# StarsX/FluidX12

Hardware: AMD Instinct MI355X
Metric: voxel-updates/sec (advect+40 Jacobi) at 256^3; achieved HBM GB/s vs peak (higher is better)
Workload: dtype f32

## Files before the change

### fluidx12_amd/capi.py

```python
import ctypes as C
import os

from . import build as _build

FX_OK = 0
FX_E_INVALID, FX_E_DEVICE, FX_E_NOMEM, FX_E_STATE, FX_E_COMM, FX_E_HALO = -1, -2, -3, -4, -5, -6

RAY_MARCH_DIRECT, RAY_MARCH_CUBEMAP, SEPARATE_LIGHT_PASS, OPTIMIZED = 0, 1, 2, 3
FRAME_COUNT = 3
STORAGE_FP32, STORAGE_FP16 = 0, 1
JACOBI_FIXED, JACOBI_FAITHFUL = 0, 1
ADDRESS_CLAMP, ADDRESS_MIRROR = 0, 1
FLAG_JACOBI_FUSE_MASK, FLAG_NO_OVERLAP, FLAG_RENDER_ONLY = 0xF, 0x10, 0x20
OPT_OVERLAP, OPT_JACOBI_ROUND, OPT_ADAPTIVE_HALO, OPT_COUNT_SAMPLES, OPT_RENDER_ACCEL = 1, 2, 3, 4, 5
ABI_VERSION = 7
(FIELD_VELOCITY, FIELD_VELOCITY1, FIELD_COLOR, FIELD_COLOR_PREV, FIELD_PRESSURE, FIELD_DIVERGENCE,
 FIELD_LIGHTMAP, FIELD_CUBEMAP, FIELD_TARGET, FIELD_TARGET_FLOAT, FIELD_CUBE_DEPTH) = range(11)
FIELD_TEMPERATURE = 11
DEPTH_DEVICE = 0x1
LIGHT_DIRECTIONAL, LIGHT_POINT = 0, 1
MAX_EMITTERS = 16
OBSTACLES_DEVICE = 0x1
MAX_OBSTACLE_BODIES = 16
MAX_OBSTACLE_MESHES = 16
# ... 19 lines not shown


class FrameInfo(C.Structure):
    _fields_ = [("cube_lod", C.c_uint32), ("cube_size", C.c_uint32), ("ray_samples", C.c_uint32),
                ("visibility_mask", C.c_uint32), ("frame_parity", C.c_uint32), ("edge_pixels", C.c_float),
                ("time_step", C.c_float), ("world_view_proj_i", C.c_float * 16), ("screen_to_world", C.c_float * 16)]


class Light(C.Structure):
    _fields_ = [("struct_size", C.c_uint32), ("kind", C.c_uint32), ("position", C.c_float * 3), ("color", C.c_float * 4),
                ("ambient", C.c_float * 4)]


class Emitter(C.Structure):
    _fields_ = [("struct_size", C.c_uint32), ("flags", C.c_uint32), ("center", C.c_float * 3), ("radius", C.c_float),
                ("color_rate", C.c_float * 4), ("force", C.c_float * 3), ("swirl", C.c_float)]


class ObstacleBody(C.Structure):
    _fields_ = [("struct_size", C.c_uint32), ("flags", C.c_uint32), ("box_lo", C.c_float * 3), ("box_hi", C.c_float * 3),
                ("linear", C.c_float * 3), ("angular", C.c_float * 3), ("pivot", C.c_float * 3)]


class ObstacleMesh(C.Structure):
    _fields_ = [("struct_size", C.c_uint32), ("flags", C.c_uint32), ("positions", C.c_void_p), ("indices", C.c_void_p),
                ("vertex_count", C.c_uint32), ("triangle_count", C.c_uint32), ("transform", C.c_void_p)]


class MeshReport(C.Structure):
    _fields_ = [("solid_cells", C.c_uint64), ("open_columns", C.c_uint32), ("skipped_triangles", C.c_uint32)]


class Buoyancy(C.Structure):
    _fields_ = [("struct_size", C.c_uint32), ("flags", C.c_uint32), ("ambient", C.c_float), ("density_weight", C.c_float),
                ("lift", C.c_float), ("cooling", C.c_float), ("up", C.c_float * 3)]


class HeatSource(C.Structure):
    _fields_ = [("struct_size", C.c_uint32), ("flags", C.c_uint32), ("center", C.c_float * 3), ("radius", C.c_float), ("rate", C.c_float)]


class PressureSolver(C.Structure):
    _fields_ = [("kind", C.c_uint32), ("flags", C.c_uint32), ("cycles", C.c_uint32), ("pre_sweeps", C.c_uint32), ("post_sweeps", C.c_uint32),
                ("coarse_sweeps", C.c_uint32), ("max_levels", C.c_uint32), ("omega", C.c_float)]


class ParticleParams(C.Structure):
    _fields_ = [("struct_size", C.c_uint32), ("flags", C.c_uint32), ("scheme", C.c_uint32), ("drift", C.c_float * 3), ("lifetime", C.c_float)]


class Timing(C.Structure):
    _fields_ = [("advect_ms", C.c_double), ("divergence_ms", C.c_double), ("jacobi_ms", C.c_double),
                ("project_ms", C.c_double), ("light_ms", C.c_double), ("view_ms", C.c_double),
                ("exchange_ms", C.c_double), ("steps", C.c_uint64), ("jacobi_launches", C.c_uint64),
                ("jacobi_sweeps", C.c_uint64), ("renders", C.c_uint64), ("resolve_ms", C.c_double),
                ("jacobi_main_ms", C.c_double), ("jacobi_main_launches", C.c_uint64), ("jacobi_main_sweeps", C.c_uint64),
                ("exchange_bytes", C.c_uint64), ("advect_halo_planes", C.c_uint64), ("chain_ms", C.c_double),
                ("freeze_solves", C.c_uint64), ("freeze_sweeps", C.c_uint64), ("exchange_calls", C.c_uint64),
                ("view_samples", C.c_uint64), ("light_samples", C.c_uint64), ("lightmap_fetches", C.c_uint64),
                ("freeze_strip_launches", C.c_uint64)]


_vp, _fp = C.c_void_p, C.POINTER(C.c_float)
SYMBOLS = {
    "fx_abi_version": (C.c_int, []),
    "fx_error_string": (C.c_char_p, [C.c_int]),
    "fx_create": (C.c_int, [C.POINTER(_vp), C.POINTER(Desc)]),
    "fx_destroy": (C.c_int, [_vp]),
    "fx_set_max_samples": (C.c_int, [_vp, C.c_uint32, C.c_uint32]),
    "fx_set_sh": (C.c_int, [_vp, _fp]),
    "fx_update_frame": (C.c_int, [_vp, C.c_float, C.c_uint8, _fp, _fp, _fp]),
    "fx_simulate": (C.c_int, [_vp, _vp, C.c_uint8]),
    "fx_render": (C.c_int, [_vp, _vp, C.c_uint8, C.c_uint8]),
    "fx_get_frame_info": (C.c_int, [_vp, C.POINTER(FrameInfo)]),
    "fx_synchronize": (C.c_int, [_vp]),
    "fx_last_error": (C.c_char_p, [_vp]),
    "fx_upload": (C.c_int, [_vp, C.c_int, _vp, C.c_size_t]),
    "fx_download": (C.c_int, [_vp, C.c_int, _vp, C.c_size_t]),
    "fx_field_bytes": (C.c_size_t, [_vp, C.c_int]),
    "fx_field_digest": (C.c_int, [_vp, C.c_int, C.c_uint32, C.c_uint32, C.POINTER(C.c_uint64)]),
    "fx_checkpoint_save": (C.c_int, [_vp, C.c_char_p]),
    "fx_checkpoint_load": (C.c_int, [_vp, C.c_char_p]),
    "fx_advect": (C.c_int, [_vp, _vp]),
    "fx_divergence": (C.c_int, [_vp, _vp]),
    "fx_jacobi": (C.c_int, [_vp, _vp, C.c_uint32]),
    "fx_project": (C.c_int, [_vp, _vp]),
    "fx_set_vorticity_confinement": (C.c_int, [_vp, C.c_float]),
    "fx_confine_vorticity": (C.c_int, [_vp, _vp]),
    "fx_set_emitters": (C.c_int, [_vp, C.POINTER(Emitter), C.c_uint32]),
    "fx_get_emitters": (C.c_int, [_vp, C.POINTER(Emitter), C.c_uint32, C.POINTER(C.c_uint32)]),
    "fx_set_impulse": (C.c_int, [_vp, C.c_int]),
    "fx_emit": (C.c_int, [_vp, _vp]),
    "fx_set_obstacles": (C.c_int, [_vp, _vp, _vp, C.c_size_t, C.c_uint32]),
    "fx_get_obstacles": (C.c_int, [_vp, _vp, C.c_size_t, C.POINTER(C.c_uint64)]),
    "fx_enforce_obstacles": (C.c_int, [_vp, _vp]),
    "fx_set_obstacle_bodies": (C.c_int, [_vp, C.POINTER(ObstacleBody), C.c_uint32]),
    "fx_get_obstacle_bodies": (C.c_int, [_vp, C.POINTER(ObstacleBody), C.c_uint32, C.POINTER(C.c_uint32)]),
    "fx_set_obstacle_meshes": (C.c_int, [_vp, _vp, C.POINTER(ObstacleMesh), C.c_uint32, C.POINTER(MeshReport)]),
    "fx_set_buoyancy": (C.c_int, [_vp, C.POINTER(Buoyancy)]),
    "fx_get_buoyancy": (C.c_int, [_vp, C.POINTER(Buoyancy), C.POINTER(C.c_int)]),
    "fx_set_heat_sources": (C.c_int, [_vp, C.POINTER(HeatSource), C.c_uint32]),
    "fx_get_heat_sources": (C.c_int, [_vp, C.POINTER(HeatSource), C.c_uint32, C.POINTER(C.c_uint32)]),
    "fx_heat": (C.c_int, [_vp, _vp]),
    "fx_set_particles": (C.c_int, [_vp, _vp, _fp, C.c_uint32, C.c_uint32]),
    "fx_get_particles": (C.c_int, [_vp, _fp, C.c_uint32, C.POINTER(C.c_uint32)]),
    "fx_particles_device": (C.c_int, [_vp, C.POINTER(_vp), C.POINTER(C.c_uint32)]),
    "fx_set_particle_params": (C.c_int, [_vp, C.POINTER(ParticleParams)]),
    "fx_get_particle_params": (C.c_int, [_vp, C.POINTER(ParticleParams)]),
    "fx_move_particles": (C.c_int, [_vp, _vp]),
    "fx_sample_velocity": (C.c_int, [_vp, _vp, _fp, C.c_uint32, _fp, C.c_uint32]),
    "fx_set_open_walls": (C.c_int, [_vp, C.c_uint32]),
    "fx_get_open_walls": (C.c_int, [_vp, C.POINTER(C.c_uint32)]),
    "fx_open_inflow": (C.c_int, [_vp, _vp]),
    "fx_set_advection_scheme": (C.c_int, [_vp, C.c_uint32]),
    "fx_get_advection_scheme": (C.c_int, [_vp, C.POINTER(C.c_uint32)]),
    "fx_set_pressure_solver": (C.c_int, [_vp, C.POINTER(PressureSolver)]),
    "fx_get_pressure_solver": (C.c_int, [_vp, C.POINTER(PressureSolver)]),
    "fx_pressure_solve": (C.c_int, [_vp, _vp]),
    "fx_download_pressure_level": (C.c_int, [_vp, C.c_uint32, C.c_int, _vp, C.c_size_t]),
    "fx_sh_transform": (C.c_int, [_vp, _fp, C.c_uint32, _fp]),
    "fx_set_environment": (C.c_int, [_vp, _fp, C.c_uint32]),
    "fx_render_environment": (C.c_int, [_vp, _vp, C.c_uint8]),
    "fx_clear_render_target": (C.c_int, [_vp, _vp, _fp]),
    "fx_render_cube": (C.c_int, [_vp, _vp, C.c_uint8]),
    "fx_set_scene_depth": (C.c_int, [_vp, _vp, _vp, C.c_uint32, C.c_uint32, C.c_float, C.c_float, C.c_uint32]),
    "fx_set_light": (C.c_int, [_vp, C.POINTER(Light)]),
    "fx_get_light": (C.c_int, [_vp, C.POINTER(Light)]),
    "fx_dds_cube_info": (C.c_int, [_vp, C.c_size_t, C.POINTER(C.c_uint32), C.POINTER(C.c_uint32)]),
    "fx_dds_decode_cube": (C.c_int, [_vp, _vp, C.c_size_t, C.c_uint32, _fp, C.c_size_t]),
    "fx_timing_enable": (C.c_int, [_vp, C.c_int]),
    "fx_set_option": (C.c_int, [_vp, C.c_uint32, C.c_uint32]),
    "fx_set_knob": (C.c_int, [C.c_char_p, C.c_char_p]),
    "fx_knob_name": (C.c_char_p, [C.c_uint32]),
    "fx_comm_gather_color": (C.c_int, [_vp, _vp, _vp, C.c_int, C.POINTER(C.c_uint32), C.POINTER(C.c_uint32)]),
    "fx_timing_read": (C.c_int, [_vp, C.POINTER(Timing), C.c_int]),
    "fx_comm_id_bytes": (C.c_size_t, []),
    "fx_comm_get_unique_id": (C.c_int, [_vp, C.c_size_t]),
    "fx_comm_init_rank": (C.c_int, [_vp, _vp, C.c_size_t, C.c_int, C.c_int]),
    "fx_comm_init_local": (C.c_int, [C.POINTER(_vp), C.c_int]),
    "fx_comm_init_peer": (C.c_int, [C.POINTER(_vp), C.c_int]),
}

_lib = None
LAB_KNOBS = {"ADVECT_BLOCK", "ADVECT_FAST", "ADVECT_LDS_HALF", "ADVECT_TILE_ROWS", "ADVECT_ZCHUNK", "BLOCK_REMAP", "BLOCK_SHAPE", "DEBUG_NO_COPY",
             "FREEZE_DENSE_LEVELS", "FREEZE_DENSE_ONE", "FREEZE_FAST", "FREEZE_FUSE_DIV", "FREEZE_NT", "FREEZE_SHRINK", "FREEZE_T", "FREEZE_WGS",
             "JACOBI2D_TILE", "JACOBI_BLOCK", "JACOBI_BLOCKG", "LIGHT_FILL_DIRTY", "LIGHT_RAY_NT", "LIGHT_RAY_WGS", "OBSTACLE_V4", "PROJECT_V4", "ROW_VW",
             "STRIP3H_PAIRS", "STRIP3_COOP", "STRIP3_NO512", "STRIP3_OFF", "STRIP3_ZCHUNK", "STRIP4T", "STRIP4T_256", "STRIP4T_512", "STRIP4T_FROM", "STRIP4T_GRID", "STRIP4T_NARROW", "STRIP4T_NARROW_FROM", "STRIP4T_PIECES", "STRIP4X", "STRIP4X_MINP", "STRIP4X_NT", "STRIP4X_ORDER", "STRIP4X_WGS",
             "STRIP4_OCTET", "STRIP4_ZCHUNK", "STRIP4_ZFLOOR", "STRIP_GENERIC", "STRIP_R", "STRIP_REMAP", "STRIP_WGS", "STRIP_WIDE", "STRIP_ZCHUNK", "VIEW_ORDER", "VIEW_WGS", "VORT_ZCHUNK", "WIDE_OFFSETS", "XCD_REMAP"}


def lib_path():
    return _build.LIB


def load():
    global _lib
    if _lib is not None:
        return _lib
    try:
        import torch
    except Exception:
        pass
    path = _build.ensure_built()
    if os.environ.get("FLUIDX_LIB_PATH"):
        path = os.environ["FLUIDX_LIB_PATH"]
    if not os.path.exists(path):
# ... 48 lines not shown
```

### fluidx12_amd/csrc/fx_advect_lds.hip

```cpp
#include "fx_internal.h"
#include <algorithm>
#include <cstdlib>
#include <cstdio>

namespace fx {

namespace {

constexpr int TX = kAdvectTileX;
constexpr int HX = TX + 2;
constexpr int NSLOT = 4;
template <bool HALF, int TY> struct Lay {
	static constexpr int NCELL = HX * (TY + 2);
	static constexpr int VEL_BYTES = NCELL * 4;
	static constexpr int COL_BYTES = HALF ? 2 * NCELL * 4 : NCELL * 16;
	static constexpr int SLOT_BYTES = COL_BYTES + 3 * VEL_BYTES;
};
typedef _Float16 h16;
typedef _Float16 h16x4 __attribute__((ext_vector_type(4)));
__device__ __forceinline__ h16 to_h16(float v) { asm("" : "+v"(v)); return (h16)v; }
__device__ __forceinline__ float lo_half(uint32_t d) { return (float)__builtin_bit_cast(h16, (uint16_t)(d & 0xffffu)); }
__device__ __forceinline__ float hi_half(uint32_t d) { return (float)__builtin_bit_cast(h16, (uint16_t)(d >> 16)); }

__device__ __forceinline__ float lerpf(float a, float b, float f) { return fmaf(f, b - a, a); }
__device__ __forceinline__ float saturatef(float x) { return fminf(fmaxf(x, 0.0f), 1.0f); }

__device__ __forceinline__ int addr_tap(int i, int n, int mode)
{
	if (mode == FX_ADDRESS_MIRROR) {
		const int period = 2 * n;
		int m = i % period;
		if (m < 0) m += period;
		return m < n ? m : period - 1 - m;
	}
	return min(max(i, 0), n - 1);
}

typedef __attribute__((address_space(3))) void lds_void;
typedef const __attribute__((address_space(1))) void glb_void;

template <int VEL_BYTES>
__device__ __forceinline__ void stage64(const void* col, const void* v0, const void* v1, const void* v2, uint32_t off_col, uint32_t off_vel, uint32_t lds_col, uint32_t lds_vel)
{
	uint32_t keep;
	lds_col = __builtin_amdgcn_readfirstlane(lds_col);
	lds_vel = __builtin_amdgcn_readfirstlane(lds_vel);
	asm volatile(
		"s_mov_b32 %0, m0\n\t"
		"s_mov_b32 m0, %7\n\t"
		"s_nop 0\n\t"
		"global_load_lds_dwordx4 %5, %1\n\t"
		"s_mov_b32 m0, %8\n\t"
		"s_nop 0\n\t"
		"global_load_lds_dword %6, %2\n\t"
		"s_add_u32 m0, m0, %9\n\t"
		"s_nop 0\n\t"
		"global_load_lds_dword %6, %3\n\t"
		"s_add_u32 m0, m0, %9\n\t"
		"s_nop 0\n\t"
		"global_load_lds_dword %6, %4\n\t"
		"s_mov_b32 m0, %0"
		: "=&s"(keep)
		: "s"(col), "s"(v0), "s"(v1), "s"(v2), "v"(off_col), "v"(off_vel), "s"(lds_col), "s"(lds_vel), "n"(VEL_BYTES)
		: "scc");
}

template <int VEL_BYTES>
__device__ __forceinline__ void stage64h(const void* col, const void* v0, const void* v1, const void* v2, uint32_t off_col, uint32_t off_vel, uint32_t lds_col, uint32_t lds_vel)
{
	uint32_t keep;
	lds_col = __builtin_amdgcn_readfirstlane(lds_col);
	lds_vel = __builtin_amdgcn_readfirstlane(lds_vel);
	const uint32_t off_col_hi = off_col + 4u;
	asm volatile(
		"s_mov_b32 %0, m0\n\t"
		"s_mov_b32 m0, %8\n\t"
		"s_nop 0\n\t"
		"global_load_lds_dword %5, %1\n\t"
		"s_add_u32 m0, m0, %10\n\t"
		"s_nop 0\n\t"
		"global_load_lds_dword %6, %1\n\t"
		"s_mov_b32 m0, %9\n\t"
		"s_nop 0\n\t"
		"global_load_lds_ushort %7, %2\n\t"
		"s_add_u32 m0, m0, %10\n\t"
		"s_nop 0\n\t"
		"global_load_lds_ushort %7, %3\n\t"
		"s_add_u32 m0, m0, %10\n\t"
		"s_nop 0\n\t"
		"global_load_lds_ushort %7, %4\n\t"
		"s_mov_b32 m0, %0"
		: "=&s"(keep)
		: "s"(col), "s"(v0), "s"(v1), "s"(v2), "v"(off_col), "v"(off_col_hi), "v"(off_vel), "s"(lds_col), "s"(lds_vel), "n"(VEL_BYTES)
		: "scc");
}

template <typename T>
__device__ __forceinline__ T ldg32(const void* base, uint32_t byte_off)
{
	return *reinterpret_cast<const T*>(static_cast<const char*>(base) + byte_off);
}


template <bool P2> __device__ __forceinline__ uint32_t rows(uint32_t y, int lgX, const Geom& g) { return P2 ? y << lgX : y * (uint32_t)g.X; }
template <bool P2> __device__ __forceinline__ uint32_t planes(uint32_t z, int lgP, const Geom& g) { return P2 ? z << lgP : z * ((uint32_t)g.X * (uint32_t)g.Y); }

template <bool HALF, bool P2>
__device__ __forceinline__ void advect_gather(const Geom& g, const SimParams& sp, int ix, int iy, int z0, int z1, bool z_present, float fx, float fy, float fz,
	const char* v0, const char* v1, const char* v2, const void* __restrict__ col_in, int lgX, int lgP, unsigned* halo_overflow, float (&u)[3], float (&c)[4])
{
	const int xa0 = addr_tap(ix, g.X, sp.address), xa1 = addr_tap(ix + 1, g.X, sp.address);
	const int ya0 = addr_tap(iy, g.Y, sp.address), ya1 = addr_tap(iy + 1, g.Y, sp.address);
	if (!z_present) {
		atomicOr(halo_overflow, 1u);
		z0 = min(max(z0, g.zlo), g.zhi);
		z1 = min(max(z1, g.zlo), g.zhi);
	}
	const uint32_t p0 = planes<P2>((uint32_t)g.lz(z0), lgP, g), p1 = planes<P2>((uint32_t)g.lz(z1), lgP, g);
	const uint32_t ry0 = rows<P2>((uint32_t)ya0, lgX, g), ry1 = rows<P2>((uint32_t)ya1, lgX, g);
	const uint32_t c000 = p0 + ry0 + (uint32_t)xa0, c100 = p0 + ry0 + (uint32_t)xa1;
	const uint32_t c010 = p0 + ry1 + (uint32_t)xa0, c110 = p0 + ry1 + (uint32_t)xa1;
	const uint32_t c001 = p1 + ry0 + (uint32_t)xa0, c101 = p1 + ry0 + (uint32_t)xa1;
	const uint32_t c011 = p1 + ry1 + (uint32_t)xa0, c111 = p1 + ry1 + (uint32_t)xa1;
	const char* vb[3] = { v0, v1, v2 };
	auto gv = [](const char* b, uint32_t cell) -> float { return HALF ? (float)ldg32<h16>(b, cell * 2u) : ldg32<float>(b, cell * 4u); };
	auto gc = [&](uint32_t cell) -> float4 {
		if (HALF) { const h16x4 h = ldg32<h16x4>(col_in, cell * 8u); return make_float4((float)h.x, (float)h.y, (float)h.z, (float)h.w); }
		return ldg32<float4>(col_in, cell * 16u);
	};
#pragma unroll
	for (int a = 0; a < 3; ++a) {
		const float c00 = lerpf(gv(vb[a], c000), gv(vb[a], c100), fx);
		const float c10 = lerpf(gv(vb[a], c010), gv(vb[a], c110), fx);
		const float c01 = lerpf(gv(vb[a], c001), gv(vb[a], c101), fx);
		const float c11 = lerpf(gv(vb[a], c011), gv(vb[a], c111), fx);
		u[a] = lerpf(lerpf(c00, c10, fy), lerpf(c01, c11, fy), fz);
	}
	const float4 t000 = gc(c000), t100 = gc(c100), t010 = gc(c010), t110 = gc(c110);
	const float4 t001 = gc(c001), t101 = gc(c101), t011 = gc(c011), t111 = gc(c111);
#define FX_TRI(m) lerpf(lerpf(lerpf(t000.m, t100.m, fx), lerpf(t010.m, t110.m, fx), fy), \
	lerpf(lerpf(t001.m, t101.m, fx), lerpf(t011.m, t111.m, fx), fy), fz)
	c[0] = FX_TRI(x); c[1] = FX_TRI(y); c[2] = FX_TRI(z); c[3] = FX_TRI(w);
#undef FX_TRI
}

template <bool HALF, bool ALPHA>
__device__ __forceinline__ void advect_finish(const SimParams& sp, float (&u)[3], float (&c)[4], float ex, float dx, float dz, float dt, float atten,
	uint32_t id, uint32_t stride, void* __restrict__ vel_out, void* __restrict__ col_out, float* __restrict__ alpha_out)
{
	if (__builtin_amdgcn_ballot_w64(sp.impulse && ex > -6.5f) != 0) {
		const float basis = exp2f(ex);
		if (basis >= 0.0183156393f) {
			float Fx, Fy, Fz;
			if (sp.is3d) {
				Fx = fmaf(basis, 0.0f, dz * -200.0f);
				Fy = fmaf(basis, 192.0f, 0.0f);
				Fz = fmaf(basis, 0.0f, dx * 200.0f);
			} else {
				Fx = 0.0f; Fy = basis * 48.0f; Fz = 0.0f;
			}
			u[0] = fmaf(Fx, dt, u[0]); u[1] = fmaf(Fy, dt, u[1]); u[2] = fmaf(Fz, dt, u[2]);
			const float bdt = basis * dt;
			c[0] = saturatef(fmaf(bdt, 8.0f, c[0]));
			c[1] = saturatef(fmaf(bdt, 16.0f, c[1]));
			c[2] = saturatef(fmaf(bdt, 40.0f, c[2]));
			c[3] = saturatef(fmaf(bdt, 40.0f, c[3]));
		}
	}
	char* vo = static_cast<char*>(vel_out);
	char* co = static_cast<char*>(col_out);
	if (HALF) {
		*reinterpret_cast<h16*>(vo + id * 2u) = to_h16(u[0] * atten);
		*reinterpret_cast<h16*>(vo + (stride + id) * 2u) = to_h16(u[1] * atten);
		*reinterpret_cast<h16*>(vo + (2u * stride + id) * 2u) = to_h16(u[2] * atten);
		h16x4 hc;
		hc.x = to_h16(c[0] * atten); hc.y = to_h16(c[1] * atten); hc.z = to_h16(c[2] * atten); hc.w = to_h16(c[3] * atten);
		*reinterpret_cast<h16x4*>(co + id * 8u) = hc;
		if (ALPHA) *reinterpret_cast<float*>(reinterpret_cast<char*>(alpha_out) + id * 4u) = (float)hc.w;
	} else {
		*reinterpret_cast<float*>(vo + id * 4u) = u[0] * atten;
		*reinterpret_cast<float*>(vo + (stride + id) * 4u) = u[1] * atten;
		*reinterpret_cast<float*>(vo + (2u * stride + id) * 4u) = u[2] * atten;
		*reinterpret_cast<float4*>(co + id * 16u) = make_float4(c[0] * atten, c[1] * atten, c[2] * atten, c[3] * atten);
		if (ALPHA) *reinterpret_cast<float*>(reinterpret_cast<char*>(alpha_out) + id * 4u) = c[3] * atten;
	}
}

}

template <bool HALF, int TY, bool DEFER, bool P2, bool ALPHA>
__global__ __launch_bounds__(64 * TY) __attribute__((amdgpu_waves_per_eu(4, 4))) void k_advect_lds(const Geom g, const SimParams sp,
	const void* __restrict__ vel_in, const void* __restrict__ col_in, void* __restrict__ vel_out, void* __restrict__ col_out, float* __restrict__ alpha_out,
	int z_begin, int nzp, int zchunk, int nchunks, unsigned* halo_overflow, float rX, float rY, float rZ, float inv_rr,
	int lgX, int lgY, int lg_gx, int lg_gy, uint32_t* __restrict__ far_list, uint32_t* __restrict__ far_flat, uint32_t* __restrict__ far_total, uint32_t far_cap)
{
	__shared__ uint32_t far_n, far_base;
	extern __shared__ __attribute__((aligned(16))) char lds[];

	const int tid = (int)threadIdx.x, lane = tid & 63, wave = __builtin_amdgcn_readfirstlane(tid >> 6);
	const int ntx = P2 ? 1 << lg_gx : lg_gx, nty = P2 ? 1 << lg_gy : lg_gy;
	const int ntiles = ntx * nty * nchunks;
	int tl = (int)blockIdx.x;
	{
		const int q = ntiles >> 3, r = ntiles & 7, xcd = tl & 7, j = tl >> 3;
		tl = xcd * q + min(xcd, r) + j;
	}
	const int tx = P2 ? tl & (ntx - 1) : tl % ntx, ty = P2 ? (tl >> lg_gx) & (nty - 1) : (tl / ntx) % nty, chunk = P2 ? tl >> (lg_gx + lg_gy) : tl / (ntx * nty);
	const int x0t = tx << 6, y0t = ty * TY;
	const int zb = z_begin + chunk * zchunk, ze = min(zb + zchunk, z_begin + nzp);
	if (zb >= ze) return;

	const int lgP = lgX + lgY;
	constexpr int COL_BYTES = Lay<HALF, TY>::COL_BYTES, SLOT_BYTES = Lay<HALF, TY>::SLOT_BYTES;
	constexpr int NCELL = Lay<HALF, TY>::NCELL, VEL_BYTES = Lay<HALF, TY>::VEL_BYTES, NT = 64 * TY;
	constexpr uint32_t ES = HALF ? 2 : 4, CS = HALF ? 8 : 16;
	const uint32_t stride = planes<P2>((uint32_t)g.nzl(), lgP, g);
	const char* v0 = reinterpret_cast<const char*>(vel_in);
	const char* v1 = v0 + (size_t)stride * ES;
	const char* v2 = v1 + (size_t)stride * ES;

	uint32_t src_a, src_b = 0;
	{
		const int c = tid, r = c / HX, cc = c - r * HX;
		src_a = rows<P2>((uint32_t)addr_tap(y0t - 1 + r, g.Y, sp.address), lgX, g) + (uint32_t)addr_tap(x0t - 1 + cc, g.X, sp.address);
	}
	const bool has_b = NT + tid < NCELL;
	if (has_b) {
		const int c = NT + tid, r = c / HX, cc = c - r * HX;
		src_b = rows<P2>((uint32_t)addr_tap(y0t - 1 + r, g.Y, sp.address), lgX, g) + (uint32_t)addr_tap(x0t - 1 + cc, g.X, sp.address);
	}
	const bool wave_has_b = NT + wave * 64 < NCELL;

	const uint32_t lds0 = (uint32_t)(size_t)(__attribute__((address_space(3))) char*)lds;
	auto fill = [&](int zq) {
		const int za = min(max(addr_tap(zq, g.Zg, sp.address), g.zlo), g.zhi);
		const size_t pz = planes<P2>((uint32_t)g.lz(za), lgP, g);
		const uint32_t slot = __builtin_amdgcn_readfirstlane(lds0 + (uint32_t)(((zq + 4) & 3) * SLOT_BYTES));
		const char* bc = reinterpret_cast<const char*>(col_in) + pz * CS;
		const char *b0 = v0 + pz * ES, *b1 = v1 + pz * ES, *b2 = v2 + pz * ES;
		if (HALF) stage64h<VEL_BYTES>(bc, b0, b1, b2, src_a * CS, src_a * ES, slot + (uint32_t)wave * (64 * 4), slot + COL_BYTES + (uint32_t)wave * (64 * 4));
		else stage64<VEL_BYTES>(bc, b0, b1, b2, src_a * CS, src_a * ES, slot + (uint32_t)wave * (64 * 16), slot + COL_BYTES + (uint32_t)wave * (64 * 4));
		if (wave_has_b) {
			if (has_b) {
				if (HALF) stage64h<VEL_BYTES>(bc, b0, b1, b2, src_b * CS, src_b * ES, slot + (NT + (uint32_t)wave * 64) * 4, slot + COL_BYTES + (NT + (uint32_t)wave * 64) * 4);
				else stage64<VEL_BYTES>(bc, b0, b1, b2, src_b * CS, src_b * ES, slot + (NT + (uint32_t)wave * 64) * 16, slot + COL_BYTES + (NT + (uint32_t)wave * 64) * 4);
			}
		}
	};

	if (DEFER && tid == 0) far_n = 0u;
	fill(zb - 1);
	fill(zb);
	fill(zb + 1);
	asm volatile("s_waitcnt vmcnt(0)" ::: "memory");
	__syncthreads();

	const int x = x0t + lane, y = y0t + wave;
	const bool has_voxel = P2 || (x < g.X && y < g.Y);
	const float dt = sp.dt;
	const float px = P2 ? ((float)x + 0.5f) * rX : ((float)x + 0.5f) / (float)g.X;
	const float py = P2 ? ((float)y + 0.5f) * rY : ((float)y + 0.5f) / (float)g.Y;
	const float dx = px + -0.5f, dy = py + -0.100000001f;
	const float dxy2 = fmaf(dy, dy, dx * dx);
	const uint32_t own = (uint32_t)((wave + 1) * HX + lane + 1);
	const float atten = fmaxf(fmaf(-dt, 0.200000003f, 1.0f), 0.0f);

	auto compute = [&](int z) {
		if (!has_voxel) return;
		const float pz = P2 ? ((float)z + 0.5f) * rZ : ((float)z + 0.5f) / (float)g.Zg;
		const float dz = pz + -0.5f;
		const float d2 = fmaf(dz, dz, dxy2);
		const float ex = ((d2 * -4.0f) * inv_rr) * 1.44269502f;

		const char* sc = lds + ((z + 4) & 3) * SLOT_BYTES;
		const uint32_t* vs = reinterpret_cast<const uint32_t*>(sc + COL_BYTES);
		auto vval = [](uint32_t d) -> float { return HALF ? lo_half(d) : __uint_as_float(d); };
		const float u0x = vval(vs[own]), u0y = vval(vs[NCELL + own]), u0z = vval(vs[2 * NCELL + own]);
		const float ax = fmaf(-u0x, dt, px), ay = fmaf(-u0y, dt, py), az = fmaf(-u0z, dt, pz);
		const float tx_ = ax * (float)g.X - 0.5f, ty_ = ay * (float)g.Y - 0.5f, tz_ = az * (float)g.Zg - 0.5f;
		const float flx = floorf(tx_), fly = floorf(ty_), flz = floorf(tz_);
		const float fx = tx_ - flx, fy = ty_ - fly, fz = tz_ - flz;
		const int ix = (int)flx, iy = (int)fly, iz = (int)flz;
		const int jx = ix - x, jy = iy - y, jz = iz - z;
		int z0 = addr_tap(iz, g.Zg, sp.address), z1 = addr_tap(iz + 1, g.Zg, sp.address);
		const bool z_present = z0 >= g.zlo && z0 <= g.zhi && z1 >= g.zlo && z1 <= g.zhi;
		const bool inwin = (unsigned)(jx + 1) <= 1u && (unsigned)(jy + 1) <= 1u && (unsigned)(jz + 1) <= 1u && z_present;

		float u[3], c[4];
		if (DEFER && !inwin) {
			const uint32_t slot = atomicAdd(&far_n, 1u);
			far_list[(size_t)blockIdx.x * far_cap + slot] = P2 ? (uint32_t)x | (uint32_t)y << lgX | (uint32_t)z << lgP
				: ((uint32_t)z * (uint32_t)g.Y + (uint32_t)y) * (uint32_t)g.X + (uint32_t)x;
		}
		if (DEFER || inwin) {
			const int kx = DEFER && !inwin ? 0 : jx, ky = DEFER && !inwin ? 0 : jy, kz = DEFER && !inwin ? z : iz;
			const uint32_t c0 = (uint32_t)((int)own + ky * HX + kx);
			const char* s0 = lds + ((kz + 4) & 3) * SLOT_BYTES;
			const char* s1 = lds + ((kz + 5) & 3) * SLOT_BYTES;
#pragma unroll
			for (int a = 0; a < 3; ++a) {
				const uint32_t* p0 = reinterpret_cast<const uint32_t*>(s0 + COL_BYTES + a * VEL_BYTES) + c0;
				const uint32_t* p1 = reinterpret_cast<const uint32_t*>(s1 + COL_BYTES + a * VEL_BYTES) + c0;
				const float c00 = lerpf(vval(p0[0]), vval(p0[1]), fx);
				const float c10 = lerpf(vval(p0[HX]), vval(p0[HX + 1]), fx);
				const float c01 = lerpf(vval(p1[0]), vval(p1[1]), fx);
				const float c11 = lerpf(vval(p1[HX]), vval(p1[HX + 1]), fx);
				u[a] = lerpf(lerpf(c00, c10, fy), lerpf(c01, c11, fy), fz);
			}
			float4 t000, t100, t010, t110, t001, t101, t011, t111;
			if (HALF) {
				auto tex = [](const char* slot, uint32_t c) -> float4 {
					const uint32_t rg = reinterpret_cast<const uint32_t*>(slot)[c], ba = reinterpret_cast<const uint32_t*>(slot)[NCELL + c];
					return make_float4(lo_half(rg), hi_half(rg), lo_half(ba), hi_half(ba));
				};
				t000 = tex(s0, c0); t100 = tex(s0, c0 + 1); t010 = tex(s0, c0 + HX); t110 = tex(s0, c0 + HX + 1);
				t001 = tex(s1, c0); t101 = tex(s1, c0 + 1); t011 = tex(s1, c0 + HX); t111 = tex(s1, c0 + HX + 1);
			} else {
				const float4* q0 = reinterpret_cast<const float4*>(s0) + c0;
				const float4* q1 = reinterpret_cast<const float4*>(s1) + c0;
				t000 = q0[0]; t100 = q0[1]; t010 = q0[HX]; t110 = q0[HX + 1];
				t001 = q1[0]; t101 = q1[1]; t011 = q1[HX]; t111 = q1[HX + 1];
			}
#define FX_TRI(m) lerpf(lerpf(lerpf(t000.m, t100.m, fx), lerpf(t010.m, t110.m, fx), fy), \
	lerpf(lerpf(t001.m, t101.m, fx), lerpf(t011.m, t111.m, fx), fy), fz)
			c[0] = FX_TRI(x); c[1] = FX_TRI(y); c[2] = FX_TRI(z); c[3] = FX_TRI(w);
#undef FX_TRI
		} else {
			advect_gather<HALF, P2>(g, sp, ix, iy, z0, z1, z_present, fx, fy, fz, v0, v1, v2, col_in, lgX, lgP, halo_overflow, u, c);
		}

		const uint32_t id = planes<P2>((uint32_t)g.lz(z), lgP, g) + rows<P2>((uint32_t)y, lgX, g) + (uint32_t)x;
		advect_finish<HALF, ALPHA>(sp, u, c, ex, dx, dz, dt, atten, id, stride, vel_out, col_out, alpha_out);
	};

	for (int z = zb; z < ze; ++z) {
		if (z + 2 <= ze) fill(z + 2);
		compute(z);
		if (!(P2 || y < g.Y)) asm volatile("s_waitcnt vmcnt(0)" ::: "memory");
		else if (ALPHA) asm volatile("s_waitcnt vmcnt(5)" ::: "memory");
		else asm volatile("s_waitcnt vmcnt(4)" ::: "memory");
		__syncthreads();
	}
	if (DEFER) {
		const uint32_t n = far_n;
		if (n != 0u) {
			if (tid == 0) far_base = atomicAdd(far_total, n);
			__syncthreads();
			const uint32_t base = far_base;
			const uint32_t* seg = far_list + (size_t)blockIdx.x * far_cap;
			for (uint32_t i = (uint32_t)tid; i < n; i += (uint32_t)NT) far_flat[base + i] = seg[i];
		}
	}
}

template <bool HALF, bool P2, bool ALPHA>
__global__ __launch_bounds__(256) void k_advect_far(const Geom g, const SimParams sp,
	const void* __restrict__ vel_in, const void* __restrict__ col_in, void* __restrict__ vel_out, void* __restrict__ col_out, float* __restrict__ alpha_out,
	const uint32_t* __restrict__ far_flat, const uint32_t* __restrict__ far_total, uint32_t* __restrict__ far_total_next, unsigned* halo_overflow,
	float rX, float rY, float rZ, float inv_rr, int lgX, int lgY)
{
	const uint32_t n = *far_total;
	if (blockIdx.x == 0 && threadIdx.x == 0) *far_total_next = 0u;
	const int lgP = lgX + lgY;
	constexpr uint32_t ES = HALF ? 2 : 4;
	const uint32_t stride = planes<P2>((uint32_t)g.nzl(), lgP, g);
	const char* v0 = reinterpret_cast<const char*>(vel_in);
	const char* v1 = v0 + (size_t)stride * ES;
	const char* v2 = v1 + (size_t)stride * ES;
	const float dt = sp.dt;
	const float atten = fmaxf(fmaf(-dt, 0.200000003f, 1.0f), 0.0f);
	for (uint32_t i = blockIdx.x * 256u + threadIdx.x; i < n; i += gridDim.x * 256u) {
		const uint32_t code = far_flat[i];
		int x, y, z;
		if (P2) { x = (int)(code & (uint32_t)(g.X - 1)); y = (int)((code >> lgX) & (uint32_t)(g.Y - 1)); z = (int)(code >> lgP); }
		else { const uint32_t XY = (uint32_t)g.X * (uint32_t)g.Y, rem = code % XY; z = (int)(code / XY); y = (int)(rem / (uint32_t)g.X); x = (int)(rem % (uint32_t)g.X); }
		const float px = P2 ? ((float)x + 0.5f) * rX : ((float)x + 0.5f) / (float)g.X;
		const float py = P2 ? ((float)y + 0.5f) * rY : ((float)y + 0.5f) / (float)g.Y;
		const float pz = P2 ? ((float)z + 0.5f) * rZ : ((float)z + 0.5f) / (float)g.Zg;
		const float dx = px + -0.5f, dy = py + -0.100000001f, dz = pz + -0.5f;
		const float dxy2 = fmaf(dy, dy, dx * dx);
		const float d2 = fmaf(dz, dz, dxy2);
		const float ex = ((d2 * -4.0f) * inv_rr) * 1.44269502f;
		const uint32_t id = planes<P2>((uint32_t)g.lz(z), lgP, g) + rows<P2>((uint32_t)y, lgX, g) + (uint32_t)x;
		auto gv = [](const char* b, uint32_t cell) -> float { return HALF ? (float)ldg32<h16>(b, cell * 2u) : ldg32<float>(b, cell * 4u); };
		const float u0x = gv(v0, id), u0y = gv(v1, id), u0z = gv(v2, id);
		const float ax = fmaf(-u0x, dt, px), ay = fmaf(-u0y, dt, py), az = fmaf(-u0z, dt, pz);
		const float tx_ = ax * (float)g.X - 0.5f, ty_ = ay * (float)g.Y - 0.5f, tz_ = az * (float)g.Zg - 0.5f;
		const float flx = floorf(tx_), fly = floorf(ty_), flz = floorf(tz_);
		const float fx = tx_ - flx, fy = ty_ - fly, fz = tz_ - flz;
		const int ix = (int)flx, iy = (int)fly, iz = (int)flz;
		const int z0 = addr_tap(iz, g.Zg, sp.address), z1 = addr_tap(iz + 1, g.Zg, sp.address);
		const bool z_present = z0 >= g.zlo && z0 <= g.zhi && z1 >= g.zlo && z1 <= g.zhi;
		float u[3], c[4];
		advect_gather<HALF, P2>(g, sp, ix, iy, z0, z1, z_present, fx, fy, fz, v0, v1, v2, col_in, lgX, lgP, halo_overflow, u, c);
		advect_finish<HALF, ALPHA>(sp, u, c, ex, dx, dz, dt, atten, id, stride, vel_out, col_out, alpha_out);
	}
}


hipError_t launch_advect_lds(const Geom& g, const SimParams& sp, int half_store, const void* vel_in, const void* col_in,
	void* vel_out, void* col_out, int z_begin, int z_end, unsigned* halo_overflow, uint32_t* far_scratch, size_t far_words, int far_parity, bool* far_used, hipStream_t s, bool force,
	AdvectAlpha* alpha)
{
	if (far_used) *far_used = false;
	if (alpha) alpha->written = false;
	const int nzp = z_end - z_begin;
	AdvectLdsKnobs kn;
	kn.tile_rows = FX_KNOB_INT("ADVECT_TILE_ROWS", 8);
	kn.lds_half = FX_KNOB_INT("ADVECT_LDS_HALF", 1);
	kn.defer = FX_KNOB_INT("ADVECT_DEFER", 1);
	kn.zchunk = FX_KNOB("ADVECT_ZCHUNK");
	const AdvectLdsPlan pl = advect_lds_plan(g, half_store, z_begin, z_end, force, far_scratch != nullptr, far_words, alpha && alpha->out, kn);
	if (!pl.staged) return hipErrorNotSupported;
	const bool p2 = pl.p2, defer = pl.defer;
	const int TY = pl.tile_rows, ntx = pl.tiles_x, nty = pl.tiles_y, zchunk = pl.zchunk, nchunks = pl.nchunks;
	auto lg = [](int v) { int k = 0; while ((1 << k) < v) ++k; return k; };
	const int lgX = lg(g.X), lgY = lg(g.Y), lg_gx = p2 ? lg(ntx) : ntx, lg_gy = p2 ? lg(nty) : nty;
	const int tiles_xy = ntx * nty;
	const float rX = 1.0f / (float)g.X, rY = 1.0f / (float)g.Y, rZ = 1.0f / (float)g.Zg, inv_rr = sp.is3d ? 256.0f : 1024.0f;
	const uint32_t far_cap = (uint32_t)(TX * TY * zchunk);
	const size_t flat_words = (size_t)g.X * g.Y * (size_t)nzp;
	if (far_used) *far_used = defer;
	uint32_t* far_total = far_scratch ? far_scratch + (far_parity & 1) : nullptr;
	uint32_t* far_total_next = far_scratch ? far_scratch + ((far_parity & 1) ^ 1) : nullptr;
	uint32_t* far_flat = far_scratch ? far_scratch + 2 : nullptr;
	uint32_t* far_list = far_scratch ? far_scratch + 2 + flat_words : nullptr;
#define FX_ADV(H_, TY_, D_, P_, A_) do { \
		static bool attr_set = false; \
		if (!attr_set) { (void)hipFuncSetAttribute(reinterpret_cast<const void*>(k_advect_lds<H_, TY_, D_, P_, A_>), hipFuncAttributeMaxDynamicSharedMemorySize, NSLOT * Lay<H_, TY_>::SLOT_BYTES); attr_set = true; } \
		hipLaunchKernelGGL((k_advect_lds<H_, TY_, D_, P_, A_>), dim3(tiles_xy * nchunks), dim3(64 * TY_), (NSLOT * Lay<H_, TY_>::SLOT_BYTES), s, g, sp, vel_in, col_in, vel_out, col_out, alpha_out, \
			z_begin, nzp, zchunk, nchunks, halo_overflow, rX, rY, rZ, inv_rr, lgX, lgY, lg_gx, lg_gy, far_list, far_flat, far_total, far_cap); } while (0)
#define FX_FAR(H_, P_, A_) hipLaunchKernelGGL((k_advect_far<H_, P_, A_>), dim3(far_wgs), dim3(256), 0, s, g, sp, vel_in, col_in, vel_out, col_out, alpha_out, far_flat, far_total, far_total_next, halo_overflow, rX, rY, rZ, inv_rr, lgX, lgY)
	const int far_wgs = 1024;
	float* alpha_out = pl.alpha ? alpha->out : nullptr;
	if (alpha_out) {
		if (half_store) { if (p2) { FX_ADV(true, 8, true, true, true); FX_FAR(true, true, true); } else { FX_ADV(true, 8, true, false, true); FX_FAR(true, false, true); } }
		else { if (p2) { FX_ADV(false, 8, true, true, true); FX_FAR(false, true, true); } else { FX_ADV(false, 8, true, false, true); FX_FAR(false, false, true); } }
		alpha->written = true;
	} else if (!p2) {
		if (defer) {
			if (half_store) { FX_ADV(true, 8, true, false, false); FX_FAR(true, false, false); } else { FX_ADV(false, 8, true, false, false); FX_FAR(false, false, false); }
		} else { if (half_store) FX_ADV(true, 8, false, false, false); else FX_ADV(false, 8, false, false, false); }
	} else if (defer) {
		if (TY == 16) { if (half_store) FX_ADV(true, 16, true, true, false); else FX_ADV(false, 16, true, true, false); }
		else { if (half_store) FX_ADV(true, 8, true, true, false); else FX_ADV(false, 8, true, true, false); }
		if (half_store) FX_FAR(true, true, false); else FX_FAR(false, true, false);
	} else {
		if (TY == 16) { if (half_store) FX_ADV(true, 16, false, true, false); else FX_ADV(false, 16, false, true, false); }
		else { if (half_store) FX_ADV(true, 8, false, true, false); else FX_ADV(false, 8, false, true, false); }
	}
#undef FX_FAR
#undef FX_ADV
	return hipGetLastError();
}

}
```

### fluidx12_amd/csrc/fx_api.cpp

```cpp
#include "fx_host.h"
#include <cstring>
#include "fx_hostmath.h"
#include "fx_mesh_args.h"

using namespace fx;
using namespace fxh;

extern "C" {

int fx_abi_version(void) { return FX_ABI_VERSION; }

int fx_set_max_samples(fx_ctx* ctx, uint32_t max_ray, uint32_t max_light)
{
	if (!ctx || !max_ray || !max_light) return FX_E_INVALID;
	ctx->max_ray_samples = max_ray;
	ctx->max_light_samples = max_light;
	return FX_OK;
}

int fx_set_sh(fx_ctx* ctx, const float* coeffs27)
{
	if (!ctx) return FX_E_INVALID;
	if (!ctx->sh_dev) return FX_E_STATE;
	if (!coeffs27) { ctx->has_sh = false; return FX_OK; }
// ... 254 lines not shown
		ctx->depth = depth;
	} else {
		const size_t bytes = (size_t)width * height * sizeof(float);
		if (!ctx->depth_own) FX_HIP(hipMalloc((void**)&ctx->depth_own, bytes));
		hipStream_t s = pick_stream(ctx, stream);
		FX_HIP(hipMemcpyAsync(ctx->depth_own, depth, bytes, hipMemcpyHostToDevice, s));
		FX_HIP(hipStreamSynchronize(s));
		ctx->depth = ctx->depth_own;
	}
	ctx->depth_zn = z_near;
	ctx->depth_zf = z_far;
	return FX_OK;
}

int fx_set_light(fx_ctx* ctx, const fx_light* light)
{
	if (!ctx) return FX_E_INVALID;
	if (ctx->g.Zg <= 1 || ctx->g.nz != ctx->g.Zg) return FX_E_INVALID;
	if (!light) { default_light(ctx); return FX_OK; }
	if (light->struct_size != sizeof(fx_light)) return FX_E_INVALID;
	if (light->kind != FX_LIGHT_DIRECTIONAL && light->kind != FX_LIGHT_POINT) return FX_E_INVALID;
	for (int a = 0; a < 3; ++a) if (!std::isfinite(light->position[a])) return FX_E_INVALID;
	for (int a = 0; a < 4; ++a)
		if (!std::isfinite(light->color[a]) || !std::isfinite(light->ambient[a]) || light->color[a] < 0.0f || light->ambient[a] < 0.0f) return FX_E_INVALID;
	if (light->kind == FX_LIGHT_DIRECTIONAL && light->position[0] == 0.0f && light->position[1] == 0.0f && light->position[2] == 0.0f) return FX_E_INVALID;
	std::memcpy(ctx->fc.light_pt, light->position, sizeof ctx->fc.light_pt);
	std::memcpy(ctx->fc.light_color, light->color, sizeof ctx->fc.light_color);
	std::memcpy(ctx->fc.ambient, light->ambient, sizeof ctx->fc.ambient);
	ctx->light_kind = light->kind;
	return FX_OK;
}

int fx_get_light(fx_ctx* ctx, fx_light* out)
{
	if (!ctx || !out) return FX_E_INVALID;
	out->struct_size = sizeof(fx_light);
	out->kind = ctx->light_kind;
	std::memcpy(out->position, ctx->fc.light_pt, sizeof out->position);
	std::memcpy(out->color, ctx->fc.light_color, sizeof out->color);
	std::memcpy(out->ambient, ctx->fc.ambient, sizeof out->ambient);
	return FX_OK;
}

int fx_set_environment(fx_ctx* ctx, const float* cube, uint32_t n)
{
	if (!ctx || (cube && (!n || n > 8192))) return FX_E_INVALID;
	DeviceGuard dg(ctx->device);
	FX_HIP(hipDeviceSynchronize());
	if (ctx->env) { FX_HIP(hipFree(ctx->env)); ctx->env = nullptr; ctx->env_n = 0; }
	if (!cube) return FX_OK;
	const size_t bytes = (size_t)6 * n * n * 3 * sizeof(float);
	FX_HIP(hipMalloc((void**)&ctx->env, bytes));
	FX_HIP(hipMemcpy(ctx->env, cube, bytes, hipMemcpyHostToDevice));
	ctx->env_n = n;
	return FX_OK;
}

int fx_render_environment(fx_ctx* ctx, void* stream, uint8_t frame_index)
{
	if (!ctx || frame_index >= FX_FRAME_COUNT) return FX_E_INVALID;
	if (!ctx->env || !ctx->view_valid) return FX_E_STATE;
	DeviceGuard dg(ctx->device);
	hipStream_t s = pick_stream(ctx, stream);
	int rc = ensure_target(ctx, s);
	if (rc) return rc;
	ScopedMark mk(ctx, s, MK_RESOLVE);
	FX_HIP(launch_environment(ctx->env, (int)ctx->env_n, ctx->fc, (int)ctx->desc.viewport_w, (int)ctx->desc.viewport_h,
		ctx->target, ctx->target_float, s));
	return FX_OK;
}

int fx_get_frame_info(fx_ctx* ctx, fx_frame_info* out)
{
	if (!ctx || !out) return FX_E_INVALID;
	out->cube_lod = ctx->cube_lod;
	out->cube_size = (uint32_t)ctx->g.X >> ctx->cube_lod;
	out->ray_samples = ctx->ray_samples;
	out->visibility_mask = ctx->visibility_mask;
	out->frame_parity = ctx->frame_parity;
	out->edge_pixels = ctx->edge_pixels;
	out->time_step = ctx->time_step;
	std::memcpy(out->world_view_proj_i, ctx->fc.wvp_i, sizeof out->world_view_proj_i);
	std::memcpy(out->screen_to_world, ctx->fc.s2w, sizeof out->screen_to_world);
	return FX_OK;
}

int fx_advect(fx_ctx* ctx, void* stream)
{
	if (!ctx) return FX_E_INVALID;
	if (ctx->desc.flags & FX_FLAG_RENDER_ONLY) return FX_E_STATE;
	if (!ctx->frame_valid) return FX_E_STATE;
	if (ctx->nranks > 1) return FX_E_INVALID;
	hipStream_t s = pick_stream(ctx, stream);
	ScopedMark mk(ctx, s, MK_ADVECT);
	return advect_range(ctx, s, owned(ctx), false);
}

static int sim_guard(const fx_ctx* ctx, bool whole = true)
{
	if (!ctx) return FX_E_INVALID;
	if (ctx->desc.flags & FX_FLAG_RENDER_ONLY) return FX_E_STATE;
	if (whole && (ctx->g.nz != ctx->g.Zg || ctx->nranks > 1)) return FX_E_INVALID;
	return FX_OK;
}

static int run_stage(fx_ctx* ctx, void* stream, int (*phase)(fx_ctx*, hipStream_t))
{
	const int rc = sim_guard(ctx);
	return rc ? rc : phase(ctx, pick_stream(ctx, stream));
}

int fx_set_vorticity_confinement(fx_ctx* ctx, float epsilon)
{
	if (!std::isfinite(epsilon) || epsilon < 0.0f) return FX_E_INVALID;
	if (const int rc = sim_guard(ctx)) return rc;
	ctx->vort_eps = epsilon;
	return FX_OK;
}

int fx_confine_vorticity(fx_ctx* ctx, void* stream) { return run_stage(ctx, stream, confine_phase); }

int fx_set_emitters(fx_ctx* ctx, const fx_emitter* list, uint32_t count)
{
	if (const int rc = sim_guard(ctx)) return rc;
	if (count > FX_MAX_EMITTERS || (count && !list)) return FX_E_INVALID;
	for (uint32_t k = 0; k < count; ++k) {
		const fx_emitter& e = list[k];
		if (e.struct_size != sizeof(fx_emitter) || e.flags != 0) return FX_E_INVALID;
		if (!std::isfinite(e.radius) || !(e.radius > 0.0f) || !std::isfinite(e.swirl)) return FX_E_INVALID;
		for (int a = 0; a < 3; ++a) if (!std::isfinite(e.center[a]) || !std::isfinite(e.force[a])) return FX_E_INVALID;
		for (int a = 0; a < 4; ++a) if (!std::isfinite(e.color_rate[a]) || e.color_rate[a] < 0.0f) return FX_E_INVALID;
	}
	ctx->emitters.assign(list, list + count);
	return FX_OK;
}

int fx_get_emitters(fx_ctx* ctx, fx_emitter* out, uint32_t capacity, uint32_t* count)
{
	if (const int rc = sim_guard(ctx, false)) return rc;
	if (!count || (capacity && !out)) return FX_E_INVALID;
	*count = (uint32_t)ctx->emitters.size();
	for (uint32_t k = 0; k < capacity && k < *count; ++k) out[k] = ctx->emitters[k];
	return FX_OK;
}

int fx_set_impulse(fx_ctx* ctx, int enabled)
{
	if (const int rc = sim_guard(ctx, !enabled)) return rc;
	ctx->impulse_on = enabled != 0;
	return FX_OK;
}

int fx_emit(fx_ctx* ctx, void* stream) { return run_stage(ctx, stream, emit_phase); }

static int install_obstacle_mask(fx_ctx* ctx, const uint8_t* src, hipStream_t s)
{
	FX_HIP(launch_obstacle_codes(ctx->g, src, ctx->obst_spare, ctx->obst_stats, s));
	unsigned st[8];
	FX_HIP(hipMemcpyAsync(st, ctx->obst_stats, sizeof st, hipMemcpyDeviceToHost, s));
	FX_HIP(hipStreamSynchronize(s));
	std::swap(ctx->obst_code, ctx->obst_spare);
	ctx->obst_cells = (uint64_t)st[0] | ((uint64_t)st[1] << 32);
	for (int a = 0; a < 3; ++a) {
		ctx->obst_lo[a] = ctx->obst_cells ? (int)st[2 + a] : 0;
		ctx->obst_hi[a] = ctx->obst_cells ? (int)st[5 + a] + 1 : 0;
	}
// ... 563 lines not shown
	FX_HIP(hipHostMalloc((void**)&ctx->rec_host, 4 * sizeof(int) * (size_t)nrec, hipHostMallocDefault));
	std::memset(ctx->rec_host, 0, 4 * sizeof(int) * (size_t)nrec);
	FX_HIP(hipEventCreateWithFlags(&ctx->rec_ev, hipEventDisableTiming));
	return FX_OK;
}

int fx_comm_init_rank(fx_ctx* ctx, const void* id, size_t bytes, int rank, int nranks)
{
	if (!ctx || !id) return FX_E_INVALID;
	int rc = check_slab_chain(ctx, rank, nranks);
	if (rc) return rc;
	Transport* t = make_rccl_transport(id, bytes, rank, nranks, ctx->device, &ctx->last_error);
	if (!t) { std::fprintf(stderr, "fluidx: %s\n", ctx->last_error.c_str()); return FX_E_COMM; }
	fx_comm_group* g = new fx_comm_group();
	g->members.push_back(ctx);
	g->transport = t;
	g->refs = 1;
	g->per_member = false; g->shared_stream = nullptr; g->broken = false;
	if ((rc = make_lane(g, ctx->device, nullptr))) { destroy_lanes(g); delete t; delete g; return rc; }
	if ((rc = t->min_over_ranks(ctx->g.nz, ctx->stream, &g->min_nz))) { destroy_lanes(g); delete t; delete g; return rc; }
	{
		const fx_desc& d = ctx->desc;
		uint32_t h = 2166136261u;
		for (uint32_t v : { d.grid_x, d.grid_y, d.grid_z, d.halo_advect, d.halo_jacobi, d.jacobi_iters, d.jacobi_mode, d.storage, d.advect_address, (uint32_t)nranks,
				d.flags & (FX_FLAG_NO_OVERLAP | FX_FLAG_JACOBI_FUSE_MASK), (uint32_t)ctx->opt_overlap, (uint32_t)ctx->opt_round, (uint32_t)ctx->opt_adaptive })
			h = (h ^ v) * 16777619u;
		const int digest = (int)(h & 0x3FFFFFFFu);
		int lo = 0, hi = 0;
		if ((rc = t->min_over_ranks(digest, ctx->stream, &lo)) || (rc = t->min_over_ranks(-digest, ctx->stream, &hi))) { destroy_lanes(g); delete t; delete g; return rc; }
		if (lo != digest || -hi != digest) {
			ctx->last_error = "fx_comm_init_rank: the ranks were created with different descriptors";
			std::fprintf(stderr, "fluidx: %s\n", ctx->last_error.c_str());
			destroy_lanes(g); delete t; delete g;
			return FX_E_INVALID;
		}
	}
	if (!ctx->step_rec && (rc = make_step_record(ctx, nranks, true))) { destroy_lanes(g); delete t; delete g; return rc; }
	{
		DeviceGuard dg(ctx->device);
		const int mine[4] = { ctx->g.z0, ctx->g.nz, 0, 0 };
		bool ok = hipMemcpy(ctx->step_rec, mine, sizeof mine, hipMemcpyHostToDevice) == hipSuccess &&
			t->allgather(ctx->step_rec, 4, ctx->gath_dev, ctx->stream) == FX_OK &&
			hipMemcpyAsync(ctx->rec_host, ctx->gath_dev, 4 * sizeof(int) * (size_t)nranks, hipMemcpyDeviceToHost, ctx->stream) == hipSuccess &&
			hipStreamSynchronize(ctx->stream) == hipSuccess;
		bool tiles = ok;
		for (int r = 0; ok && r + 1 < nranks; ++r) tiles = tiles && ctx->rec_host[4 * r] + ctx->rec_host[4 * r + 1] == ctx->rec_host[4 * (r + 1)];
		if (ok) ok = hipMemset(ctx->step_rec, 0, 4 * sizeof(int)) == hipSuccess;
		if (!ok || !tiles) {
			ctx->last_error = ok ? "fx_comm_init_rank: the slabs of the ranks do not tile the grid in rank order" : "fx_comm_init_rank: exchanging the slab ranges failed";
			std::fprintf(stderr, "fluidx: %s\n", ctx->last_error.c_str());
			destroy_lanes(g); delete t; delete g;
			return ok ? FX_E_INVALID : FX_E_COMM;
		}
	}
	ctx->group = g; ctx->rank = rank; ctx->nranks = nranks;
	return FX_OK;
}

int fx_comm_gather_color(fx_ctx* ctx, void* stream, fx_ctx* full, int root, const uint32_t* slab_z0, const uint32_t* slab_nz)
{
	if (!ctx || !ctx->group || root < 0 || root >= ctx->nranks) return FX_E_INVALID;
	if (group_broken(ctx)) return FX_E_STATE;
	if (!is_driver(ctx)) return FX_OK;
	const bool local = ctx->group->transport->is_local();
	const bool am_root = local || ctx->rank == root;
	if (am_root) {
		if (!full || full->g.X != ctx->g.X || full->g.Y != ctx->g.Y || full->g.Zg != ctx->g.Zg || full->g.nz != full->g.Zg ||
			full->half != ctx->half) return FX_E_INVALID;
		if (!local && full->device != ctx->device) return FX_E_INVALID;
		if (local && full->device != ctx->group->members[(size_t)root]->device) return FX_E_INVALID;
	}
	if (!local && (!slab_z0 || !slab_nz)) return FX_E_INVALID;
	const size_t plane_bytes = ctx->g.plane() * 4 * elem_size(ctx);
	std::vector<GatherPart> parts((size_t)ctx->nranks);
	for (int r = 0; r < ctx->nranks; ++r) {
		const fx_ctx* m = local ? ctx->group->members[r] : (r == ctx->rank ? ctx : nullptr);
		const uint32_t z0 = local ? (uint32_t)m->g.z0 : slab_z0[r], nz = local ? (uint32_t)m->g.nz : slab_nz[r];
		if (z0 > (uint32_t)ctx->g.Zg || nz > (uint32_t)ctx->g.Zg - z0) return FX_E_INVALID;
		if (!local && r == ctx->rank && (z0 != (uint32_t)ctx->g.z0 || nz != (uint32_t)ctx->g.nz)) return FX_E_INVALID;
		parts[r].rank = r;
		parts[r].bytes = (size_t)nz * plane_bytes;
		parts[r].src = m ? (const char*)m->col[m->frame_parity] + (size_t)m->g.H * plane_bytes : nullptr;
		parts[r].dst = am_root ? (char*)full->col[full->frame_parity] + (size_t)z0 * plane_bytes : nullptr;
		if (am_root) full->accel_alpha_of = nullptr;
	}
	DeviceGuard dg(ctx->device);
	hipStream_t s = pick_stream(ctx, stream);
	if (ctx->halo_fault) return FX_E_HALO;
	std::vector<hipStream_t> streams;
	if (ctx->group->per_member) for (fx_ctx* m : ctx->group->members) streams.push_back(m->stream);
	else streams.push_back(s);
	hipStream_t done_on = ctx->group->per_member ? streams[(size_t)root] : s;
	ScopedMark mk(ctx, s, MK_EXCH);
	int rc = ctx->group->transport->gather(ctx->group, parts, root, streams);
	if (rc) return rc;
	if (am_root && full->stream != done_on) {
		fx_lane& L = ctx->group->per_member ? ctx->group->lanes[(size_t)root] : ctx->group->lanes[0];
		DeviceGuard dgr(L.device);
		FX_HIP(hipEventRecord(L.ev_done, done_on));
		DeviceGuard dgf(full->device);
		FX_HIP(hipStreamWaitEvent(full->stream, L.ev_done, 0));
	}
	return FX_OK;
}

static int check_local_members(fx_ctx** ctxs, int nranks, bool one_device)
{
	if (!ctxs || nranks < 1) return FX_E_INVALID;
	int zexp = 0;
	for (int r = 0; r < nranks; ++r) {
		if (!ctxs[r]) return FX_E_INVALID;
		int rc = check_slab_chain(ctxs[r], r, nranks);
		if (rc) return rc;
		if (ctxs[r]->g.z0 != zexp || (one_device && ctxs[r]->device != ctxs[0]->device)) return FX_E_INVALID;
		const fx_desc &a = ctxs[r]->desc, &b = ctxs[0]->desc;
		if (a.grid_x != b.grid_x || a.grid_y != b.grid_y || a.grid_z != b.grid_z || a.halo_advect != b.halo_advect ||
			a.halo_jacobi != b.halo_jacobi || a.jacobi_iters != b.jacobi_iters || a.jacobi_mode != b.jacobi_mode ||
			a.storage != b.storage || a.advect_address != b.advect_address)
			return FX_E_INVALID;
		for (int q = 0; q < r; ++q) if (ctxs[q] == ctxs[r]) return FX_E_INVALID;
		zexp += ctxs[r]->g.nz;
	}
	return FX_OK;
}

static int init_in_process_group(fx_ctx** ctxs, int nranks, bool peer)
{
	int rc = check_local_members(ctxs, nranks, !peer);
	if (rc) return rc;
	if (peer) {
		for (int r = 0; r + 1 < nranks; ++r) {
			const int a = ctxs[r]->device, b = ctxs[r + 1]->device;
			if (a == b) continue;
			int ab = 0, ba = 0;
			if (hipDeviceCanAccessPeer(&ab, a, b) != hipSuccess || hipDeviceCanAccessPeer(&ba, b, a) != hipSuccess || !ab || !ba) {
				ctxs[0]->last_error = "fx_comm_init_peer: two neighbouring slabs live on devices without peer access";
				return FX_E_DEVICE;
			}
			for (int k = 0; k < 2; ++k) {
				DeviceGuard dg(k ? b : a);
				const hipError_t e = hipDeviceEnablePeerAccess(k ? a : b, 0);
				if (e != hipSuccess && e != hipErrorPeerAccessAlreadyEnabled) { (void)hipGetLastError(); return FX_E_DEVICE; }
				(void)hipGetLastError();
			}
		}
	}
	for (int r = 0; r < nranks; ++r)
		if (!ctxs[r]->step_rec) { if ((rc = make_step_record(ctxs[r], 1, false))) return rc; }
	fx_comm_group* g = new fx_comm_group();
	g->transport = make_local_transport();
	g->refs = nranks;
	g->per_member = peer; g->shared_stream = nullptr; g->broken = false;
	for (int r = 0; r < (peer ? nranks : 1); ++r)
		if ((rc = make_lane(g, ctxs[r]->device, peer ? ctxs[r]->stream : nullptr))) { destroy_lanes(g); delete g->transport; delete g; return rc; }
	g->min_nz = ctxs[0]->g.nz;
	for (int r = 1; r < nranks; ++r) g->min_nz = std::min(g->min_nz, ctxs[r]->g.nz);
	for (int r = 0; r < nranks; ++r) {
		g->members.push_back(ctxs[r]);
		ctxs[r]->group = g; ctxs[r]->rank = r; ctxs[r]->nranks = nranks;
		if (peer) continue;
		if (r > 0) {
			if (ctxs[r]->owns_stream) (void)hipStreamDestroy(ctxs[r]->stream);
			ctxs[r]->stream = ctxs[0]->stream;
		}
		ctxs[r]->owns_stream = false;
		g->shared_stream = ctxs[0]->stream;
	}
// ... 9 lines not shown
```

### fluidx12_amd/csrc/fx_comm.cpp

```cpp
#include "fx_context.h"
#include <dlfcn.h>
#include <rccl/rccl.h>
#include <cstdio>
#include <cstdlib>
#include <cstring>

namespace fx {

int exchange_items(fx_ctx* c, int which_set, int k, int pidx, ExchItem out[4])
{
	const size_t plane = c->g.plane();
	const size_t es = c->half ? 2 : 4;
	switch (which_set) {
	case EX_ADVECT_IN:
		out[0] = ExchItem{ (char*)c->vel[0], plane * es, 3, k, nullptr, c->adv_w_lo, c->adv_w_hi };
		out[1] = ExchItem{ (char*)c->col[1 - c->frame_parity], plane * es * 4, 1, k, nullptr, c->adv_w_lo, c->adv_w_hi };
		return 2;
	case EX_UZ1:
		out[0] = ExchItem{ (char*)c->vel[1] + 2 * (size_t)c->g.nzl() * plane * es, plane * es, 1, k, nullptr };
		return 1;
	case EX_DIV:
		out[0] = ExchItem{ (char*)c->b, plane * 4, 1, k, nullptr };
		return 1;
	case EX_PRESSURE:
		(void)pidx;
		out[0] = ExchItem{ (char*)c->p[c->p_cur & 1], plane * 4, 1, k, nullptr };
		if (!c->frozen) return 1;
		out[1] = ExchItem{ (char*)c->frozen, plane, 1, k, nullptr };
		return 2;
	case EX_ADVECT_VEL:
		out[0] = ExchItem{ (char*)c->vel[0], plane * es, 3, k, nullptr, c->adv_w_lo, c->adv_w_hi };
		return 1;
	case EX_COLOR_CUR:
		out[0] = ExchItem{ (char*)c->col[c->frame_parity], plane * es * 4, 1, k, nullptr };
		return 1;
	case EX_FREEZE:
		out[0] = ExchItem{ (char*)c->fz_x_p, plane * 4, 1, k, nullptr };
		out[1] = ExchItem{ (char*)c->fz_x_m, (size_t)((c->g.X + 3) / 4) * c->g.Y, 1, k, nullptr };
		return 2;
	case EX_PRESSURE_FACE:
		out[0] = ExchItem{ (char*)c->p_face[(pidx >> 1) & 1], plane * 4, 1, k, (char*)c->p[(c->p_cur ^ pidx) & 1] };
		return 1;
	}
	return 0;
}

void halo_segments(const fx_ctx* c, const ExchItem* items, int n, std::vector<Seg>& out)
{
	const Geom& g = c->g;
	for (int i = 0; i < n; ++i) {
		const ExchItem& it = items[i];
		if (it.k <= 0) continue;
		const size_t pb = it.plane_bytes;
		const int klo = it.k_lo >= 0 ? it.k_lo : it.k, khi = it.k_hi >= 0 ? it.k_hi : it.k;
		for (int cpt = 0; cpt < it.ncomp; ++cpt) {
			char* base = it.base + (size_t)cpt * g.nzl() * pb;
			char* rbase = (it.recv_base ? it.recv_base : it.base) + (size_t)cpt * g.nzl() * pb;
			if (c->rank > 0 && klo > 0)
				out.push_back(Seg{ base + (size_t)g.H * pb, rbase + (size_t)(g.H - klo) * pb, (size_t)klo * pb, -1 });
			if (c->rank + 1 < c->nranks && khi > 0)
				out.push_back(Seg{ base + (size_t)(g.H + g.nz - khi) * pb, rbase + (size_t)(g.H + g.nz) * pb, (size_t)khi * pb, +1 });
		}
	}
}

struct LocalTransport : Transport {
	bool is_local() const override { return true; }
	int min_over_ranks(int v, hipStream_t, int* out) override { *out = v; return FX_OK; }
	int allgather(const int*, int, int*, hipStream_t) override { return FX_OK; }
	int exchange(fx_comm_group* grp, const std::vector<std::vector<Seg>>& segs, const std::vector<hipStream_t>& streams, int channel) override
	{
		(void)channel;
		const int n = (int)grp->members.size();
		if ((int)segs.size() != n || streams.empty()) return FX_E_STATE;
		const bool peer = streams.size() > 1;
		if (peer && ((int)streams.size() != n || (int)grp->lanes.size() != n)) return FX_E_STATE;
#ifdef FX_LAB
		const bool no_copy = [] { const char* e = FX_KNOB("DEBUG_NO_COPY"); return e && e[0] == '1'; }();
		if (no_copy) return FX_OK;
#endif
		int home = -1;
		(void)hipGetDevice(&home);
		int rc = FX_OK;
		if (peer) {
			for (int r = 0; r < n && rc == FX_OK; ++r)
				if (hipSetDevice(grp->lanes[r].device) != hipSuccess || hipEventRecord(grp->lanes[r].x_ready, streams[r]) != hipSuccess) rc = FX_E_DEVICE;
			for (int r = 0; r < n && rc == FX_OK; ++r)
				for (int d = -1; d <= 1; d += 2) {
					const int q = r + d;
					if (q < 0 || q >= n) continue;
					if (hipSetDevice(grp->lanes[r].device) != hipSuccess || hipStreamWaitEvent(streams[r], grp->lanes[q].x_ready, 0) != hipSuccess) rc = FX_E_DEVICE;
				}
		}
		for (int r = 0; r < n && rc == FX_OK; ++r) {
			hipStream_t s = peer ? streams[r] : streams[0];
			if (peer && hipSetDevice(grp->lanes[r].device) != hipSuccess) { rc = FX_E_DEVICE; break; }
			for (int d = -1; d <= 1 && rc == FX_OK; d += 2) {
				const int q = r + d;
				if (q < 0 || q >= n) continue;
				size_t jp = 0;
				for (const Seg& mine : segs[r]) {
					if (mine.dir != d) continue;
					while (jp < segs[q].size() && segs[q][jp].dir != -d) ++jp;
					if (jp == segs[q].size() || segs[q][jp].bytes != mine.bytes) { rc = FX_E_STATE; break; }
					hipError_t e;
					if (peer && grp->lanes[r].device != grp->lanes[q].device)
						e = hipMemcpyPeerAsync(mine.recv, grp->lanes[r].device, segs[q][jp].send, grp->lanes[q].device, mine.bytes, s);
					else e = launch_copy_bytes(mine.recv, segs[q][jp].send, mine.bytes, s);
					if (e != hipSuccess) { rc = FX_E_DEVICE; break; }
					++jp;
				}
			}
		}
		if (peer) {
			for (int r = 0; r < n && rc == FX_OK; ++r)
				if (hipSetDevice(grp->lanes[r].device) != hipSuccess || hipEventRecord(grp->lanes[r].x_done, streams[r]) != hipSuccess) rc = FX_E_DEVICE;
			for (int r = 0; r < n && rc == FX_OK; ++r)
// ... 234 lines not shown
```

### fluidx12_amd/csrc/fx_context.cpp

```cpp
#include "fx_host.h"
#include <time.h>

using namespace fx;
using namespace fxh;

namespace fx {
bool digest_range_ok(const Geom& g, uint32_t z_begin, uint32_t z_count)
{
	if (!z_count) return true;
	if (g.nz < 0 || z_count > (uint32_t)g.nz) return false;
	const int64_t first = (int64_t)z_begin, end = first + (int64_t)z_count;
	return first >= (int64_t)g.z0 && end <= (int64_t)g.z0 + (int64_t)g.nz;
}
}

namespace fxh {

size_t ev_record(fx_ctx* c, hipStream_t s)
{
	if (c->ev_used == c->ev.size()) {
		hipEvent_t e;
		if (hipEventCreate(&e) != hipSuccess) return (size_t)-1;
		c->ev.push_back(e);
	}
	(void)hipEventRecord(c->ev[c->ev_used], s);
	return c->ev_used++;
}

int drain_timing(fx_ctx* c)
{
	for (const auto& m : c->marks) {
		float ms = 0.0f;
		if (hipEventSynchronize(c->ev[m.e1]) != hipSuccess) return FX_E_DEVICE;
		if (hipEventElapsedTime(&ms, c->ev[m.e0], c->ev[m.e1]) != hipSuccess) return FX_E_DEVICE;
		switch (m.kind) {
		case MK_ADVECT: c->acc.advect_ms += ms; break;
		case MK_DIV: c->acc.divergence_ms += ms; break;
		case MK_JACOBI: c->acc.jacobi_ms += ms; c->acc.jacobi_launches += m.launches; c->acc.jacobi_sweeps += m.sweeps;
			c->acc.jacobi_main_ms += ms; c->acc.jacobi_main_launches += m.launches; c->acc.jacobi_main_sweeps += m.sweeps; break;
		case MK_JACOBI_TAIL: c->acc.jacobi_ms += ms; c->acc.jacobi_launches += m.launches; c->acc.jacobi_sweeps += m.sweeps; break;
		case MK_PROJECT: c->acc.project_ms += ms; break;
		case MK_LIGHT: c->acc.light_ms += ms; break;
		case MK_VIEW: c->acc.view_ms += ms; break;
		case MK_EXCH: c->acc.exchange_ms += ms; break;
		case MK_RESOLVE: c->acc.resolve_ms += ms; break;
		case MK_CHAIN: c->acc.chain_ms += ms; break;
		}
	}
	c->marks.clear();
	c->ev_used = 0;
	return FX_OK;
}

int ensure_stage(fx_ctx* ctx, size_t bytes)
{
	if (ctx->stage_bytes >= bytes) return FX_OK;
	if (ctx->stage) { FX_HIP(hipFree(ctx->stage)); ctx->stage = nullptr; ctx->stage_bytes = 0; }
	FX_HIP(hipMalloc((void**)&ctx->stage, bytes));
	ctx->stage_bytes = bytes;
	return FX_OK;
}

void destroy_lanes(fx_comm_group* g)
{
	for (fx_lane& l : g->lanes) {
		DeviceGuard dg(l.device);
		if (l.comm) (void)hipStreamDestroy(l.comm);
		if (l.face) (void)hipStreamDestroy(l.face);
		for (hipEvent_t e : { l.ev_ready, l.ev_done, l.ev_col_ready, l.ev_col_done, l.ev_int, l.ev_face1, l.x_ready, l.x_done }) if (e) (void)hipEventDestroy(e);
	}
	g->lanes.clear();
}

void group_release(fx_comm_group* g)
{
	{
		DeviceGuard dg(g->lanes.empty() ? 0 : g->lanes[0].device);
		if (g->shared_stream) (void)hipStreamDestroy(g->shared_stream);
	}
	destroy_lanes(g);
	delete g->transport;
	delete g;
}

void free_all(fx_ctx* c)
{
	for (int i = 0; i < 2; ++i) {
		if (c->vel[i]) (void)hipFree(c->vel[i]);
		if (c->col[i]) (void)hipFree(c->col[i]);
		if (c->p[i]) (void)hipFree(c->p[i]);
	}
	void* others[] = { c->env, c->cube_depth, c->depth_own, c->accel.occ, c->accel.alpha, c->accel.bits, c->accel.list, c->accel.cells, c->accel.gi, c->accel.ctr, c->target, c->target_float, c->p_face[0], c->p_face[1], c->b, c->frozen, c->frozen_alt, c->lightmap, c->cube, c->sh_dev, c->halo_overflow, c->stage,
		c->sh_scratch[0], c->sh_scratch[1], c->sh_scratch[2], c->sh_scratch[3], c->p_aux, c->fz_mask[0], c->fz_mask[1], c->fz_mask[2], c->fz_tile_next, c->fz_stat, c->fz_list[0], c->fz_list[1], c->fz_counts, c->sample_counters, c->adv_far, c->obst_code, c->obst_spare, c->obst_stats, c->vox_bits, c->vox_report, c->vox_work, c->temp[0], c->temp[1], c->mc_vel, c->mc_col, c->mg_mem, c->part };
	for (void* q : others) if (q) (void)hipFree(q);
	for (hipEvent_t e : c->ev) (void)hipEventDestroy(e);
	if (c->step_rec) (void)hipFree(c->step_rec);
	if (c->gath_dev) (void)hipFree(c->gath_dev);
	if (c->rec_host) (void)hipHostFree(c->rec_host);
	if (c->fz_active_host) (void)hipHostFree(c->fz_active_host);
	if (c->fz_active_ev) (void)hipEventDestroy(c->fz_active_ev);
	if (c->rec_ev) (void)hipEventDestroy(c->rec_ev);
	if (c->owns_stream && c->stream) (void)hipStreamDestroy(c->stream);
}

}

extern "C" {

const char* fx_error_string(int status)
{
	switch (status) {
	case FX_OK: return "ok";
	case FX_E_INVALID: return "invalid argument";
	case FX_E_DEVICE: return "HIP device/runtime error";
	case FX_E_NOMEM: return "out of memory";
	case FX_E_STATE: return "invalid call order";
	case FX_E_COMM: return "RCCL communication error";
	case FX_E_HALO: return "advection back-trace left the exchanged halo";
	default: return "unknown status";
	}
}

int fx_create(fx_ctx** out, const fx_desc* d)
{
	if (!out || !d || d->struct_size != sizeof(fx_desc)) return FX_E_INVALID;
	*out = nullptr;
	if (!d->grid_x || !d->grid_y || !d->grid_z) return FX_E_INVALID;
	if (d->grid_x != d->grid_y) return FX_E_INVALID;
	if (d->grid_x > 65535 || d->grid_z > 65535) return FX_E_INVALID;
	if (d->storage > FX_STORAGE_FP16 || d->jacobi_mode > FX_JACOBI_FAITHFUL || d->advect_address > FX_ADDRESS_MIRROR) return FX_E_INVALID;
	if (!d->jacobi_iters) return FX_E_INVALID;
	uint32_t z0 = d->slab_z0, nz = d->slab_nz ? d->slab_nz : d->grid_z;
	if (z0 + nz > d->grid_z) return FX_E_INVALID;
	const bool slab = nz != d->grid_z;

	int ndev = 0;
	if (hipGetDeviceCount(&ndev) != hipSuccess || ndev <= 0) return FX_E_DEVICE;
	int dev = d->device;
	if (dev < 0 && hipGetDevice(&dev) != hipSuccess) return FX_E_DEVICE;
	if (dev >= ndev) return FX_E_INVALID;

	fx_ctx* ctx = new (std::nothrow) fx_ctx();
	if (!ctx) return FX_E_NOMEM;
	ctx->desc = *d;
	ctx->desc.slab_z0 = z0; ctx->desc.slab_nz = nz;
	default_light(ctx);
	if (!ctx->desc.halo_advect) ctx->desc.halo_advect = kDefaultAdvectHalo;
	if (!ctx->desc.halo_jacobi) ctx->desc.halo_jacobi = kDefaultJacobiHalo;
	if (!slab) { ctx->desc.halo_advect = 0; }
	const int H = slab ? (int)std::max(ctx->desc.halo_advect, ctx->desc.halo_jacobi) : 0;
	if (slab && (int)nz < H) { delete ctx; return FX_E_INVALID; }
	if (slab && (d->flags & FX_FLAG_RENDER_ONLY)) { delete ctx; return FX_E_INVALID; }
	ctx->g = Geom{ (int)d->grid_x, (int)d->grid_y, (int)d->grid_z, (int)z0, (int)nz, H,
		std::max((int)z0 - H, 0), std::min((int)(z0 + nz) + H, (int)d->grid_z) - 1 };
	ctx->half = d->storage == FX_STORAGE_FP16;
	ctx->device = dev;
	ctx->max_ray_samples = 192; ctx->max_light_samples = 64;
	ctx->rank = 0; ctx->nranks = 1;
	ctx->opt_overlap = (d->flags & FX_FLAG_NO_OVERLAP) ? 0 : 2;
	ctx->opt_round = (int)ctx->desc.halo_jacobi;

	DeviceGuard dg(dev);
	if (!dg.ok) { delete ctx; return FX_E_DEVICE; }
	int rc = [&]() -> int {
		FX_HIP(hipStreamCreateWithFlags(&ctx->stream, hipStreamNonBlocking));
		ctx->owns_stream = true;
		const size_t cells = ctx->g.cells_local();
		const size_t es = elem_size(ctx);
		if (d->flags & FX_FLAG_RENDER_ONLY) {
			FX_HIP(hipMalloc(&ctx->col[0], 4 * cells * es));
			FX_HIP(hipMemsetAsync(ctx->col[0], 0, 4 * cells * es, ctx->stream));
		}
		for (int i = 0; i < 2 && !(d->flags & FX_FLAG_RENDER_ONLY); ++i) {
			FX_HIP(hipMalloc(&ctx->vel[i], 3 * cells * es));
			FX_HIP(hipMalloc(&ctx->col[i], 4 * cells * es));
			FX_HIP(hipMalloc((void**)&ctx->p[i], cells * 4));
			FX_HIP(hipMemsetAsync(ctx->vel[i], 0, 3 * cells * es, ctx->stream));
			FX_HIP(hipMemsetAsync(ctx->col[i], 0, 4 * cells * es, ctx->stream));
			FX_HIP(hipMemsetAsync(ctx->p[i], 0, cells * 4, ctx->stream));
		}
		if (slab && !(d->flags & FX_FLAG_RENDER_ONLY))
			for (int i = 0; i < 2; ++i) {
				FX_HIP(hipMalloc((void**)&ctx->p_face[i], cells * 4));
				FX_HIP(hipMemsetAsync(ctx->p_face[i], 0, cells * 4, ctx->stream));
			}
		if (!(d->flags & FX_FLAG_RENDER_ONLY)) {
			FX_HIP(hipMalloc((void**)&ctx->b, cells * 4));
			FX_HIP(hipMemsetAsync(ctx->b, 0, cells * 4, ctx->stream));
		}
		if (d->jacobi_mode == FX_JACOBI_FAITHFUL && !(d->flags & FX_FLAG_RENDER_ONLY)) {
			FX_HIP(hipMalloc((void**)&ctx->frozen, cells));
			FX_HIP(hipMemsetAsync(ctx->frozen, 0, cells, ctx->stream));
			if (ctx->g.Zg == 1) {
				FX_HIP(hipMalloc((void**)&ctx->frozen_alt, cells));
				FX_HIP(hipMemsetAsync(ctx->frozen_alt, 0, cells, ctx->stream));
			}
			if (jacobi_freeze_supported(ctx->g)) {
				const size_t mb = jacobi_freeze_mask_bytes(ctx->g), nt = (size_t)jacobi_freeze_tiles(ctx->g);
				FX_HIP(hipMalloc((void**)&ctx->p_aux, cells * 4));
				FX_HIP(hipMemsetAsync(ctx->p_aux, 0, cells * 4, ctx->stream));
				for (int i = 0; i < 3; ++i) {
					FX_HIP(hipMalloc((void**)&ctx->fz_mask[i], mb));
					FX_HIP(hipMemsetAsync(ctx->fz_mask[i], 0, mb, ctx->stream));
				}
				FX_HIP(hipMalloc((void**)&ctx->fz_tile_next, nt * sizeof(uint32_t)));
				FX_HIP(hipMemsetAsync(ctx->fz_tile_next, 0, nt * sizeof(uint32_t), ctx->stream));
				for (int i = 0; i < 2; ++i) FX_HIP(hipMalloc(&ctx->fz_list[i], jacobi_freeze_list_bytes(ctx->g)));
				FX_HIP(hipMalloc((void**)&ctx->fz_counts, 2 * jacobi_freeze_count_words() * sizeof(uint32_t)));
				FX_HIP(hipMemsetAsync(ctx->fz_counts, 0, 2 * jacobi_freeze_count_words() * sizeof(uint32_t), ctx->stream));
				FX_HIP(hipMalloc((void**)&ctx->fz_stat, kFreezeStatRing * sizeof(uint32_t)));
				FX_HIP(hipMemsetAsync(ctx->fz_stat, 0, kFreezeStatRing * sizeof(uint32_t), ctx->stream));
				ctx->fz_iters.assign(kFreezeStatRing, 0);
				if (jacobi_freeze_strip_supported(ctx->g) && hipHostMalloc((void**)&ctx->fz_active_host, 64, hipHostMallocMapped) == hipSuccess) {
					ctx->fz_active_host[0] = 0u;
					if (hipHostGetDevicePointer((void**)&ctx->fz_active_dev, ctx->fz_active_host, 0) != hipSuccess) ctx->fz_active_dev = nullptr;
				} else (void)hipGetLastError();
			}
		}
		FX_HIP(hipMalloc((void**)&ctx->halo_overflow, sizeof(unsigned)));
		FX_HIP(hipMemsetAsync(ctx->halo_overflow, 0, sizeof(unsigned), ctx->stream));
		if (!(d->flags & FX_FLAG_RENDER_ONLY)) {
			ctx->adv_far_tried = true;
			const size_t words = advect_far_words(ctx->g, ctx->g.nz);
			if (words) {
				if (hipMalloc((void**)&ctx->adv_far, words * sizeof(uint32_t)) == hipSuccess) {
					FX_HIP(hipMemsetAsync(ctx->adv_far, 0, 2 * sizeof(uint32_t), ctx->stream));
					ctx->adv_far_words = words;
				} else { (void)hipGetLastError(); ctx->adv_far = nullptr; }
			}
		}
		if (d->grid_z > 1) {
			FX_HIP(hipMalloc((void**)&ctx->lightmap, ctx->g.cells_owned() * 4));
			FX_HIP(hipMemsetAsync(ctx->lightmap, 0, ctx->g.cells_owned() * 4, ctx->stream));
			size_t off = 0;
			for (uint32_t m = 0; m < kNumMips; ++m) {
				ctx->cube_mip_offset[m] = off;
				const size_t sz = std::max<uint32_t>(d->grid_x >> m, 1);
				off += 6 * sz * sz * 4;
			}
			FX_HIP(hipMalloc((void**)&ctx->cube, off));
			FX_HIP(hipMemsetAsync(ctx->cube, 0, off, ctx->stream));
			if (d->viewport_w && d->viewport_h) {
				FX_HIP(hipMalloc((void**)&ctx->cube_depth, off));
				FX_HIP(hipMemsetD32Async((hipDeviceptr_t)ctx->cube_depth, 0x3f800000, off / 4, ctx->stream));
			}
			if (!slab && ctx->g.cells_owned() <= ((size_t)1 << 28) && ctx->g.X >= 4) {
				RenderAccel& A = ctx->accel;
				render_accel_layout(ctx->g, &A);
				const size_t ncell = (size_t)A.CX * A.CY * A.CZ, vox = ctx->g.cells_owned(), bw = render_accel_bits_words(A);
				FX_HIP(hipMalloc((void**)&A.occ, 2 * ncell * sizeof(float)));
				FX_HIP(hipMalloc((void**)&A.alpha, vox * sizeof(float)));
				FX_HIP(hipMalloc((void**)&A.bits, bw * sizeof(uint32_t)));
				FX_HIP(hipMemsetAsync(A.bits, 0, bw * sizeof(uint32_t), ctx->stream));
				FX_HIP(hipMalloc((void**)&A.list, vox * sizeof(uint32_t)));
				FX_HIP(hipMalloc((void**)&A.cells, ncell * sizeof(uint32_t)));
				FX_HIP(hipMalloc((void**)&A.ctr, render_accel_ctr_words(ctx->g) * sizeof(uint32_t)));
				FX_HIP(hipMemsetAsync(A.ctr, 0, render_accel_ctr_words(ctx->g) * sizeof(uint32_t), ctx->stream));
				ctx->accel_ok = true;
			}
			FX_HIP(hipMalloc((void**)&ctx->sh_dev, 27 * sizeof(float)));
			FX_HIP(hipMemsetAsync(ctx->sh_dev, 0, 27 * sizeof(float), ctx->stream));
		}
		FX_HIP(hipStreamSynchronize(ctx->stream));
		return FX_OK;
	}();
	if (rc != FX_OK) { free_all(ctx); delete ctx; return rc; }
	*out = ctx;
	return FX_OK;
}

int fx_destroy(fx_ctx* ctx)
{
	if (!ctx) return FX_E_INVALID;
	DeviceGuard dg(ctx->device);
	(void)hipDeviceSynchronize();
	if (ctx->group) {
		fx_comm_group* g = ctx->group;
		for (auto& m : g->members) if (m == ctx) m = nullptr;
		g->broken = true;
		if (--g->refs == 0) group_release(g);
	}
	free_all(ctx);
	delete ctx;
	return FX_OK;
}

static int halo_fault_status(fx_ctx* c)
{
	if (!c->halo_overflow) return FX_OK;
	unsigned flag = 0;
	if (hipMemcpy(&flag, c->halo_overflow, sizeof flag, hipMemcpyDeviceToHost) != hipSuccess) return FX_E_DEVICE;
	if (flag) c->halo_fault = true;
	return c->halo_fault ? FX_E_HALO : FX_OK;
}

static int wait_for_device(fx_ctx* c)
{
	Transport* t = c->group && c->group->transport && !c->group->transport->is_local() ? c->group->transport : nullptr;
	if (!t || !t->can_poll()) return hipDeviceSynchronize() == hipSuccess ? FX_OK : FX_E_DEVICE;
	std::vector<hipStream_t> streams{ c->stream, c->last_step_stream };
	for (const fx_lane& L : c->group->lanes) { streams.push_back(L.comm); streams.push_back(L.face); }
	std::vector<hipEvent_t> evs;
	int rc = FX_OK;
	for (hipStream_t s : streams) {
		if (!s) continue;
		hipEvent_t e;
		if (hipEventCreateWithFlags(&e, hipEventDisableTiming) != hipSuccess) { rc = FX_E_DEVICE; break; }
		evs.push_back(e);
		if (hipEventRecord(e, s) != hipSuccess) { rc = FX_E_DEVICE; break; }
	}
	for (size_t i = 0; i < evs.size() && rc == FX_OK;) {
// ... 67 lines not shown
		return FX_OK;
	}
	return FX_E_INVALID;
}

size_t fx_field_bytes(fx_ctx* ctx, int field)
{
	size_t b = 0;
	if (!ctx || field_info(ctx, field, &b) != FX_OK) return 0;
	return b;
}

int fx_field_digest(fx_ctx* ctx, int field, uint32_t z_begin, uint32_t z_count, uint64_t out[2])
{
	if (!ctx || !out) return FX_E_INVALID;
	size_t need = 0;
	int rc = field_info(ctx, field, &need);
	if (rc) return rc;
	if (field > FX_FIELD_DIVERGENCE) return FX_E_INVALID;
	const Geom& g = ctx->g;
	if (!digest_range_ok(g, z_begin, z_count)) return FX_E_INVALID;
	if (!z_count) { z_begin = (uint32_t)g.z0; z_count = (uint32_t)g.nz; }
	DeviceGuard dg(ctx->device);
	FX_HIP(hipDeviceSynchronize());
	if ((rc = halo_fault_status(ctx))) return rc;
	if ((rc = ensure_stage(ctx, 16))) return rc;
	unsigned long long* acc = reinterpret_cast<unsigned long long*>(ctx->stage);
	FX_HIP(hipMemsetAsync(acc, 0, 16, ctx->stream));
	const size_t plane = g.plane(), cl = g.cells_local(), first = (size_t)g.lz((int)z_begin) * plane, n = (size_t)z_count * plane;
	const size_t es = elem_size(ctx);
	const unsigned long long gfirst = (unsigned long long)z_begin * plane, gcells = (unsigned long long)g.Zg * plane;
	switch (field) {
	case FX_FIELD_VELOCITY: case FX_FIELD_VELOCITY1: {
		const char* src = (const char*)ctx->vel[field == FX_FIELD_VELOCITY1];
		for (int a = 0; a < 3; ++a) FX_HIP(launch_digest(src + (a * cl + first) * es, n, (int)es, a * gcells + gfirst, acc, ctx->stream));
		break;
	}
	case FX_FIELD_COLOR: case FX_FIELD_COLOR_PREV: {
		const char* src = (const char*)ctx->col[field == FX_FIELD_COLOR ? ctx->frame_parity : 1 - ctx->frame_parity];
		FX_HIP(launch_digest(src + first * 4 * es, 4 * n, (int)es, 4 * gfirst, acc, ctx->stream));
		break;
	}
	case FX_FIELD_PRESSURE: FX_HIP(launch_digest(ctx->p[ctx->p_cur] + first, n, 4, gfirst, acc, ctx->stream)); break;
	default: FX_HIP(launch_digest(ctx->b + first, n, 4, gfirst, acc, ctx->stream)); break;
	}
	FX_HIP(hipStreamSynchronize(ctx->stream));
	FX_HIP(hipMemcpy(out, acc, 16, hipMemcpyDeviceToHost));
	return FX_OK;
}

int fx_upload(fx_ctx* ctx, int field, const void* host, size_t bytes)
{
	if (!ctx || !host) return FX_E_INVALID;
	size_t need = 0;
	int rc = field_info(ctx, field, &need);
	if (rc) return rc;
	if (bytes != need) return FX_E_INVALID;
	DeviceGuard dg(ctx->device);
	FX_HIP(hipDeviceSynchronize());
	if (field <= FX_FIELD_DIVERGENCE || field == FX_FIELD_TEMPERATURE) { ctx->fz_dense_n = 0; ctx->fz_active_pending = false; }
	const size_t n = ctx->g.cells_owned(), off = (size_t)ctx->g.H * ctx->g.plane(), cl = ctx->g.cells_local();
	const size_t es = elem_size(ctx);
	switch (field) {
	case FX_FIELD_VELOCITY: case FX_FIELD_VELOCITY1: {
		if (field == FX_FIELD_VELOCITY && ctx->group) {
			if (!ctx->group->transport->is_local() && ctx->opt_adaptive && ctx->rec_pending && !ctx->collective_upload) return FX_E_STATE;
			ctx->need_valid = false;
		}
		char* dst = (char*)ctx->vel[field == FX_FIELD_VELOCITY1];
		if ((rc = ensure_stage(ctx, need))) return rc;
		FX_HIP(hipMemcpy(ctx->stage, host, need, hipMemcpyHostToDevice));
		for (int a = 0; a < 3; ++a)
			FX_HIP(launch_to_storage(ctx->stage + a * n, dst + (a * cl + off) * es, n, ctx->half, ctx->stream));
		break;
	}
	case FX_FIELD_COLOR: case FX_FIELD_COLOR_PREV: {
		if (ctx->col_halo_buf >= 0 && ctx->group) {
			if (!ctx->group->transport->is_local() && !ctx->collective_upload) return FX_E_STATE;
			if (ctx->group->transport->is_local()) { for (fx_ctx* m : ctx->group->members) if (m) m->col_halo_buf = -1; }
			else ctx->col_halo_buf = -1;
		}
		char* dst = (char*)ctx->col[field == FX_FIELD_COLOR ? ctx->frame_parity : 1 - ctx->frame_parity];
		if (ctx->accel_alpha_of == dst) ctx->accel_alpha_of = nullptr;
		if ((rc = ensure_stage(ctx, need))) return rc;
		FX_HIP(hipMemcpy(ctx->stage, host, need, hipMemcpyHostToDevice));
		FX_HIP(launch_to_storage(ctx->stage, dst + off * 4 * es, 4 * n, ctx->half, ctx->stream));
		break;
	}
	case FX_FIELD_PRESSURE:
		FX_HIP(hipMemcpy(ctx->p[ctx->p_cur] + off, host, need, hipMemcpyHostToDevice));
		break;
	case FX_FIELD_DIVERGENCE:
		FX_HIP(hipMemcpy(ctx->b + off, host, need, hipMemcpyHostToDevice));
		break;
	case FX_FIELD_TEMPERATURE:
		FX_HIP(hipMemcpy(ctx->temp[ctx->temp_cur], host, need, hipMemcpyHostToDevice));
		break;
	case FX_FIELD_CUBEMAP:
		FX_HIP(hipMemcpy(ctx->cube + ctx->cube_mip_offset[ctx->cube_lod], host, need, hipMemcpyHostToDevice));
		ctx->cube_depth_on[ctx->cube_lod] = false;
		break;
	default:
		return FX_E_INVALID;
	}
	FX_HIP(hipStreamSynchronize(ctx->stream));
	return FX_OK;
}

int fx_download(fx_ctx* ctx, int field, void* host, size_t bytes)
{
	if (!ctx || !host) return FX_E_INVALID;
	size_t need = 0;
	int rc = field_info(ctx, field, &need);
	if (rc) return rc;
	if (bytes != need) return FX_E_INVALID;
	DeviceGuard dg(ctx->device);
	FX_HIP(hipDeviceSynchronize());
	if (field <= FX_FIELD_DIVERGENCE && (rc = halo_fault_status(ctx))) return rc;
	const size_t n = ctx->g.cells_owned(), off = (size_t)ctx->g.H * ctx->g.plane(), cl = ctx->g.cells_local();
	const size_t es = elem_size(ctx);
	switch (field) {
	case FX_FIELD_VELOCITY: case FX_FIELD_VELOCITY1: {
		const char* src = (const char*)ctx->vel[field == FX_FIELD_VELOCITY1];
		if ((rc = ensure_stage(ctx, need))) return rc;
		for (int a = 0; a < 3; ++a)
			FX_HIP(launch_from_storage(src + (a * cl + off) * es, ctx->stage + a * n, n, ctx->half, ctx->stream));
		FX_HIP(hipStreamSynchronize(ctx->stream));
		FX_HIP(hipMemcpy(host, ctx->stage, need, hipMemcpyDeviceToHost));
		break;
	}
	case FX_FIELD_COLOR: case FX_FIELD_COLOR_PREV: {
		const char* src = (const char*)ctx->col[field == FX_FIELD_COLOR ? ctx->frame_parity : 1 - ctx->frame_parity];
		if ((rc = ensure_stage(ctx, need))) return rc;
		FX_HIP(launch_from_storage(src + off * 4 * es, ctx->stage, 4 * n, ctx->half, ctx->stream));
		FX_HIP(hipStreamSynchronize(ctx->stream));
		FX_HIP(hipMemcpy(host, ctx->stage, need, hipMemcpyDeviceToHost));
		break;
	}
	case FX_FIELD_PRESSURE:
		FX_HIP(hipMemcpy(host, ctx->p[ctx->p_cur] + off, need, hipMemcpyDeviceToHost));
		break;
	case FX_FIELD_DIVERGENCE:
		FX_HIP(hipMemcpy(host, ctx->b + off, need, hipMemcpyDeviceToHost));
		break;
	case FX_FIELD_TEMPERATURE:
		FX_HIP(hipMemcpy(host, ctx->temp[ctx->temp_cur], need, hipMemcpyDeviceToHost));
		break;
	case FX_FIELD_LIGHTMAP:
		if ((rc = ensure_stage(ctx, need))) return rc;
		FX_HIP(launch_lightmap_decode(ctx->lightmap, ctx->stage, n, ctx->stream));
		FX_HIP(hipStreamSynchronize(ctx->stream));
		FX_HIP(hipMemcpy(host, ctx->stage, need, hipMemcpyDeviceToHost));
		break;
	case FX_FIELD_CUBEMAP:
		FX_HIP(hipMemcpy(host, ctx->cube + ctx->cube_mip_offset[ctx->cube_lod], need, hipMemcpyDeviceToHost));
		break;
	case FX_FIELD_CUBE_DEPTH:
		FX_HIP(hipMemcpy(host, (const char*)ctx->cube_depth + ctx->cube_mip_offset[ctx->cube_lod], need, hipMemcpyDeviceToHost));
		break;
	case FX_FIELD_TARGET:
		FX_HIP(hipMemcpy(host, ctx->target, need, hipMemcpyDeviceToHost));
		break;
	case FX_FIELD_TARGET_FLOAT:
		FX_HIP(hipMemcpy(host, ctx->target_float, need, hipMemcpyDeviceToHost));
		break;
	default:
// ... 98 lines not shown
```

### fluidx12_amd/csrc/fx_context.h

```cpp
#pragma once
#include "fx_internal.h"
#include <vector>
#include <string>

struct fx_comm_group;
struct fx_lane;

struct fx_ctx {
	fx_desc desc;
	fx::Geom g;
	int half;
	int device;
	hipStream_t stream;
	bool owns_stream;

	void* vel[2];
	void* col[2];
	float* p[2];
	int p_cur;
	float* p_face[2];
	float* b;
	uint8_t* frozen;
	uint8_t* frozen_alt = nullptr;
	float* p_aux = nullptr;
	uint32_t* fz_active_host = nullptr;
	uint32_t* fz_active_dev = nullptr;
	hipEvent_t fz_active_ev = nullptr;
	bool fz_active_pending = false;
	int fz_dense_n = 0;
	uint8_t* fz_mask[3] = { nullptr, nullptr, nullptr };
	uint32_t* fz_tile_next = nullptr;
	void* fz_list[2] = { nullptr, nullptr };
	uint32_t* fz_counts = nullptr;
	uint32_t* fz_stat = nullptr;
	float* fz_x_p = nullptr;
	uint8_t* fz_x_m = nullptr;
	bool fz_fuse_div = false;
	uint32_t* adv_far = nullptr;
	bool adv_far_tried = false;
	size_t adv_far_words = 0;
	uint32_t adv_far_turn = 0;
	uint32_t fz_gen = 0;
	uint32_t fz_gen_mark = 0;
	std::vector<uint32_t> fz_iters;
	uint32_t* lightmap;
	uint8_t* cube;
	size_t cube_mip_offset[5];
	float* cube_depth;
	bool cube_depth_on[5];
	const float* depth;
	float* depth_own;
	float depth_zn, depth_zf;
	float vort_eps = 0.0f;
	std::vector<fx_emitter> emitters;
	bool impulse_on = true;
	uint8_t* obst_code = nullptr;
	uint8_t* obst_spare = nullptr;
	unsigned* obst_stats = nullptr;
	uint64_t obst_cells = 0;
	int obst_lo[3] = { 0, 0, 0 }, obst_hi[3] = { 0, 0, 0 };
	std::vector<fx_obstacle_body> obst_bodies;
	unsigned* vox_bits = nullptr;
	unsigned* vox_report = nullptr;
	void* vox_work = nullptr;
	size_t vox_work_bytes = 0;
	uint32_t open_faces = 0;
	bool buoy_on = false;
	fx_buoyancy buoy = { (uint32_t)sizeof(fx_buoyancy), 0u, 0.0f, 0.0f, 0.0f, 0.0f, { 0.0f, 1.0f, 0.0f } };
	float* temp[2] = { nullptr, nullptr };
	int temp_cur = 0;
	std::vector<fx_heat_source> heat_sources;
	uint32_t adv_scheme = FX_ADVECT_SEMI_LAGRANGIAN;
	float* mc_vel = nullptr;
	float* mc_col = nullptr;
	fx_pressure_solver solver = { FX_PRESSURE_JACOBI, 0u, 0u, 0u, 0u, 0u, 0u, 0.0f };
	fx::MgPlan mg = {};
	float* mg_mem = nullptr;
	float* mg_e[fx::kMgMaxLevels][2] = {};
	float* mg_b[fx::kMgMaxLevels] = {};
	int mg_cur[fx::kMgMaxLevels] = {};
	float* part = nullptr;
	uint32_t part_count = 0;
	fx_particle_params part_prm = { (uint32_t)sizeof(fx_particle_params), 0u, FX_PARTICLE_MIDPOINT, { 0.0f, 0.0f, 0.0f }, 0.0f };
	uint32_t light_kind = 0;
	float wvp[16];
	float* env;
	uint32_t env_n;
	fx::RenderAccel accel = {};
	bool accel_ok = false;
	const void* accel_alpha_of = nullptr;
	bool rendered_since_step = false;
	bool lightmap_filled = false;
	float lightmap_key[9] = {};
	hipStream_t last_step_stream = nullptr;
	hipStream_t rendered_on = nullptr;
	int opt_render_accel = 1;
	uint8_t* target;
	float* target_float;
	float* sh_dev;
	bool has_sh;
	unsigned* halo_overflow;
	float* stage;
	size_t stage_bytes;
	float* sh_scratch[4];
	size_t sh_scratch_n;

	uint32_t max_ray_samples, max_light_samples;
	uint32_t ray_samples, cube_lod, visibility_mask;
	uint8_t frame_parity;
	float time_step;
	float edge_pixels;
	bool frame_valid, view_valid;
	fx::FrameConsts fc;

	bool timing_on;
	std::vector<hipEvent_t> ev;
	size_t ev_used;
	struct Mark { int kind; size_t e0, e1; uint64_t launches, sweeps; };
	std::vector<Mark> marks;
	fx_timing acc;

	fx_comm_group* group;
	int rank, nranks;
	int opt_overlap;
	int opt_round;
	int opt_count_samples = 0;
	unsigned long long* sample_counters = nullptr;
	std::string last_error;
	int col_halo_buf = -1;
	uint64_t steps_simulated = 0;
	int* step_rec = nullptr;
	int* gath_dev = nullptr;
	int* rec_host = nullptr;
	hipEvent_t rec_ev = nullptr;
	bool rec_pending = false;
	bool need_valid = false;
	float rec_dt = 0.0f;
	int opt_adaptive = 1;
	int adv_w_lo = 0, adv_w_hi = 0;
	bool halo_fault = false;
	bool collective_upload = false;
	bool rec_in_project = false;
};

namespace fx {

struct ExchItem { char* base; size_t plane_bytes; int ncomp; int k; char* recv_base; int k_lo = -1, k_hi = -1; };

struct Seg { char* send; char* recv; size_t bytes; int dir; };

struct GatherPart { int rank; const char* src; char* dst; size_t bytes; };

struct Transport {
	virtual ~Transport() {}
	virtual int exchange(fx_comm_group* grp, const std::vector<std::vector<Seg>>& segs, const std::vector<hipStream_t>& streams, int channel = 0) = 0;
	virtual int gather(fx_comm_group* grp, const std::vector<GatherPart>& parts, int root, const std::vector<hipStream_t>& streams) = 0;
	virtual bool is_local() const = 0;
	virtual int min_over_ranks(int v, hipStream_t s, int* out) = 0;
	virtual int allgather(const int* send_dev, int count, int* recv_dev, hipStream_t s) = 0;
	virtual int poll_error(std::string* err) { (void)err; return FX_OK; }
	virtual bool can_poll() const { return false; }
};

}

struct fx_lane {
	int device;
	hipStream_t compute;
	hipStream_t comm;
	hipEvent_t ev_ready, ev_done;
	hipStream_t face;
	hipEvent_t ev_col_ready, ev_col_done;
	hipEvent_t ev_int, ev_face1;
	hipEvent_t x_ready, x_done;
};

struct fx_comm_group {
	std::vector<fx_ctx*> members;
	fx::Transport* transport;
	int refs;
	std::vector<fx_lane> lanes;
	bool per_member;
	int min_nz;
	hipStream_t shared_stream;
	bool broken;
	fx_lane& lane_of(const fx_ctx* m);
};

inline fx_lane& fx_comm_group::lane_of(const fx_ctx* m) { return per_member ? lanes[(size_t)m->rank] : lanes[0]; }

namespace fx {
enum ExchSet {
	EX_ADVECT_IN = 0,
	EX_UZ1 = 1,
	EX_DIV = 2,
	EX_PRESSURE = 3,
	EX_PRESSURE_FACE = 4,
	EX_ADVECT_VEL = 5,
	EX_COLOR_CUR = 6,
	EX_FREEZE = 7
};
int exchange_items(fx_ctx* c, int which_set, int k, int pidx, ExchItem out[4]);
void halo_segments(const fx_ctx* c, const ExchItem* items, int n, std::vector<Seg>& out);
Transport* make_local_transport();
Transport* make_rccl_transport(const void* id, size_t bytes, int rank, int nranks, int device, std::string* err);
size_t rccl_id_bytes();
int rccl_get_unique_id(void* out, size_t bytes, std::string* err);
}
```

### fluidx12_amd/csrc/fx_internal.h

```cpp
#pragma once
#include <hip/hip_runtime.h>
#include <stdint.h>
#include <stddef.h>
#include "../../include/fluidx_hip.h"
#include "fx_knobs.h"

namespace fx {

struct Geom {
	int X, Y;
	int Zg;
	int z0;
	int nz;
	int H;
	int zlo, zhi;
	__host__ __device__ size_t plane() const { return (size_t)X * Y; }
	__host__ __device__ int nzl() const { return nz + 2 * H; }
	__host__ __device__ size_t cells_local() const { return plane() * (size_t)nzl(); }
	__host__ __device__ size_t cells_owned() const { return plane() * (size_t)nz; }
	__host__ __device__ int lz(int z) const { return z - z0 + H; }
};
inline bool whole_grid(const Geom& g) { return g.nz == g.Zg && g.H == 0; }
inline bool open_faces_ok(const Geom& g, unsigned faces) { return !(faces & ~0x3Fu) && !(g.Zg <= 1 && (faces & (FX_WALL_Z_LO | FX_WALL_Z_HI))); }
inline bool lab_wide_offsets() { return FX_KNOB_INT("WIDE_OFFSETS", 0) != 0; }
inline bool colour_wants_wide_offsets(const Geom& g) { return g.cells_local() * 16 >= ((size_t)1 << 32) || lab_wide_offsets(); }

struct FrameConsts {
	float world_i[12];
	float world[12];
	float eye_pt[3];
	float light_pt[3];
	float light_color[4];
	float ambient[4];
	float wvp_i[16];
	float s2w[16];
};

struct DepthArgs {
	const float* depth;
	int W, H;
	float wvp[16];
	float z_near, z_far;
	float* cube_depth;
};

struct SimParams {
	float dt;
	int address;
	int is3d;
	int impulse = 1;
};

struct AdvectAlpha { float* out; bool written; };
hipError_t launch_advect(const Geom& g, const SimParams& sp, int half_store, const void* vel_in, const void* col_in,
	void* vel_out, void* col_out, int z_begin, int z_end, unsigned* halo_overflow, hipStream_t s, uint32_t* far_scratch = nullptr, size_t far_words = 0, int far_parity = 0, bool* far_used = nullptr,
	AdvectAlpha* alpha = nullptr);
hipError_t launch_advect_lds(const Geom& g, const SimParams& sp, int half_store, const void* vel_in, const void* col_in,
	void* vel_out, void* col_out, int z_begin, int z_end, unsigned* halo_overflow, uint32_t* far_scratch, size_t far_words, int far_parity, bool* far_used, hipStream_t s, bool force,
	AdvectAlpha* alpha = nullptr);
size_t advect_far_words(const Geom& g, int nzp);
const int kAdvectTileX = 64;
struct AdvectLdsKnobs { int tile_rows = 8, lds_half = 1, defer = 1; const char* zchunk = nullptr; };
struct AdvectLdsPlan { bool staged, p2; int tile_rows, tiles_x, tiles_y, zchunk, nchunks; bool defer, alpha; };
AdvectLdsPlan advect_lds_plan(const Geom& g, int half_store, int z_begin, int z_end, bool force, bool has_scratch, size_t far_words, bool alpha_offered,
	const AdvectLdsKnobs& k);
hipError_t launch_confine_vorticity(const Geom& g, int half_store, const void* vel_in, void* vel_out, float eps, float dt, hipStream_t s);
const int kEmitTileX = 64, kEmitTileY = 4;
struct EmitBall { float c[3], rr, rate[4], force[3], swirl; int lo[3], hi[3]; };
struct EmitArgs { int n, x0, y0, z0, tiles_x, tiles_y, tiles_z; EmitBall e[FX_MAX_EMITTERS]; };
int emit_plan(const Geom& g, const fx_emitter* list, int count, EmitArgs* out);
hipError_t launch_emit(const Geom& g, int half_store, void* vel, void* col, float* alpha, const fx_emitter* list, int count, float dt, hipStream_t s);
const int kHeatTileX = 64, kHeatTileY = 4;
struct HeatBall { float c[3], rr, rate; int lo[3], hi[3]; };
struct HeatArgs { float ambient, weight, lift, cooling, up[3]; int axes, n, tiles_x, tiles_y; HeatBall s[FX_MAX_HEAT_SOURCES]; };
int heat_plan(const Geom& g, const fx_buoyancy& b, const fx_heat_source* list, int count, HeatArgs* out);
hipError_t launch_heat(const Geom& g, int half_store, const fx_buoyancy& b, const fx_heat_source* list, int count, const void* vel0, void* vel1,
	const void* col, const float* t_in, float* t_out, const uint8_t* code, float dt, int address, hipStream_t s, unsigned faces = 0);
const int kMcTileX = 64, kMcTileY = 4;
hipError_t launch_maccormack(const Geom& g, const SimParams& sp, int half_store, const void* vel_in, const void* col_in, void* vel_out, void* col_out,
	float* hat_vel, float* hat_col, float* alpha_out, hipStream_t s);
const int kMgMaxLevels = (int)FX_MG_MAX_LEVELS, kMgTailCells = 4096, kMgTailLdsBytes = 64 * 1024;
struct MgDims { int X, Y, Z; __host__ __device__ size_t cells() const { return (size_t)X * Y * Z; } };
struct MgPlan { int levels, tail, tail_floats; MgDims lv[kMgMaxLevels]; };
int mg_plan(const Geom& g, unsigned max_levels, MgPlan* out);
hipError_t launch_mg_smooth(const MgDims& d, int is3d, const float* e_in, const float* b, float* e_out, float omega, hipStream_t s);
hipError_t launch_mg_residual_restrict(const MgDims& fine, int is3d, const float* p, const float* b, float* b_coarse, hipStream_t s);
hipError_t launch_mg_prolong_correct(const MgDims& fine, int is3d, float* p, const float* e_coarse, hipStream_t s);
struct MgTailArgs { int first, levels, is3d, pre, post, coarse; float omega; MgDims lv[kMgMaxLevels]; float* e[kMgMaxLevels]; float* b[kMgMaxLevels]; };
hipError_t launch_mg_tail(const MgTailArgs& a, int lds_floats, hipStream_t s);
__host__ __device__ inline float open_wall_weight(float fl, float f, int n, unsigned lo_open, unsigned hi_open)
{
	float w = 1.0f;
	if (lo_open && fl < 0.0f) w = fl == -1.0f ? f : 0.0f;
	if (hi_open && fl >= (float)(n - 1)) w = fl == (float)(n - 1) ? 1.0f - f : 0.0f;
	return w;
}
__host__ __device__ inline float open_wall_trace(float u0, float dt, int i, int n, unsigned lo_open, unsigned hi_open)
{
	const float p = ((float)i + 0.5f) / (float)n;
	const float a = fmaf(-u0, dt, p);
	const float t = a * (float)n - 0.5f;
	const float fl = floorf(t);
	return open_wall_weight(fl, t - fl, n, lo_open, hi_open);
}
const int kOpenTileX = 64, kOpenTileY = 4;
hipError_t launch_open_inflow(const Geom& g, int half_store, const void* vel0, void* col, float* alpha, unsigned faces, float dt, hipStream_t s);
hipError_t launch_divergence(const Geom& g, int half_store, const void* vel, float* b, int z_begin, int z_end, hipStream_t s);
hipError_t launch_obstacle_codes(const Geom& g, const uint8_t* solid_dev, uint8_t* code, unsigned* stats_dev, hipStream_t s);
hipError_t launch_obstacle_mask(const uint8_t* code, uint8_t* solid_dev, size_t n, hipStream_t s);
long long obstacle_enforce_tiles(const int lo[3], const int hi[3], int* x0, int* y0, int* tiles_x, int* tiles_y);
hipError_t launch_obstacle_enforce(const Geom& g, int half_store, const uint8_t* code, const int lo[3], const int hi[3], void* vel, void* col,
	float* alpha, hipStream_t s);
hipError_t launch_divergence_obs(const Geom& g, int half_store, const void* vel, const uint8_t* code, float* b, int z_begin, int z_end, hipStream_t s);
hipError_t launch_jacobi_bnd(const Geom& g, const float* p_in, const float* b, const uint8_t* code, float* p_out, unsigned faces,
	int z_begin, int z_end, hipStream_t s);
hipError_t launch_project_bnd(const Geom& g, const SimParams& sp, int half_store, const void* vel_in, const float* p, const uint8_t* code,
	void* vel_out, unsigned faces, int z_begin, int z_end, hipStream_t s);
struct BodyArg { float lo[3], hi[3], lin[3], ang[3], piv[3]; };
struct BodyArgs { int n, is3d; BodyArg b[FX_MAX_OBSTACLE_BODIES]; };
hipError_t launch_obstacle_enforce_mov(const Geom& g, int half_store, const uint8_t* code, const int lo[3], const int hi[3],
	const fx_obstacle_body* list, int count, void* vel, void* col, float* alpha, hipStream_t s);
hipError_t launch_divergence_obs_mov(const Geom& g, int half_store, const void* vel, const uint8_t* code, const fx_obstacle_body* list, int count,
	float* b, int z_begin, int z_end, hipStream_t s);
hipError_t launch_project_bnd_mov(const Geom& g, const SimParams& sp, int half_store, const void* vel_in, const float* p, const uint8_t* code,
	const fx_obstacle_body* list, int count, void* vel_out, unsigned faces, int z_begin, int z_end, hipStream_t s);
struct VoxMesh { const float* pos; const uint32_t* idx; const float* xf; uint32_t nv, nt; };
enum { kVoxReportWords = 2 + FX_MAX_OBSTACLE_MESHES };
inline int voxel_row_words(const Geom& g) { return g.X / 32 + 1; }
hipError_t launch_voxel_scatter(const Geom& g, const VoxMesh& m, unsigned* bits, unsigned* report, unsigned* nbig, uint4* list, hipStream_t s);
hipError_t launch_voxel_fill(const Geom& g, unsigned* bits, uint8_t* mask, bool first, unsigned* report, hipStream_t s);
hipError_t launch_move_particles(const Geom& g, int half_store, const fx_particle_params& prm, const void* vel0, const uint8_t* code, unsigned faces,
	float dt, float* records, uint32_t count, hipStream_t s);
hipError_t launch_sample_velocity(const Geom& g, int half_store, const void* vel0, const float* points, float* out, uint32_t count, hipStream_t s);
enum SimStage { SIM_DIVERGENCE = 0, SIM_PROJECT = 1 };
enum SimRowKernel { ROW_SCALAR = 0, ROW_V4 = 4, ROW_VW2 = 2, ROW_VW3 = 3 };
int sim_row_kernel(const Geom& g, int half_store, int stage, int is3d);
bool digest_range_ok(const Geom& g, uint32_t z_begin, uint32_t z_count);
hipError_t launch_jacobi_sweep(const Geom& g, const float* p_in, const float* b, float* p_out, uint8_t* frozen,
	int z_begin, int z_end, hipStream_t s);
hipError_t launch_jacobi_sweep2(const Geom& g, const float* p_in, const float* b, float* p_out, uint8_t* frozen,
	int z_begin, int z_end, int z_begin2, int z_end2, hipStream_t s);
bool jacobi_strip_supported(const Geom& g);
// ... 121 lines not shown
```

### fluidx12_amd/csrc/fx_schedule.cpp

```cpp
#include "fx_host.h"
#include <memory>

using namespace fx;

namespace fxh {

int for_members(fx_ctx* ctx, std::vector<fx_ctx*>& out)
{
	out.clear();
	if (ctx->group && ctx->group->transport->is_local() && !ctx->group->broken) out = ctx->group->members;
	else out.push_back(ctx);
	return FX_OK;
}


static inline bool peer_group(const fx_ctx* c) { return c->group && c->group->per_member; }
static inline hipStream_t CS(const fx_ctx* m, hipStream_t s) { return peer_group(m) ? m->group->lane_of(m).compute : s; }
struct LaneRef { fx_lane* lane; hipStream_t compute; };
static std::vector<LaneRef> lanes_of(fx_ctx* lead, const std::vector<fx_ctx*>& M, hipStream_t s)
{
	std::vector<LaneRef> out;
	if (!lead->group) return out;
	if (lead->group->per_member) for (fx_ctx* m : M) out.push_back(LaneRef{ &lead->group->lane_of(m), lead->group->lane_of(m).compute });
	else out.push_back(LaneRef{ &lead->group->lanes[0], s });
	return out;
}
enum StreamKind { ON_COMPUTE = 0, ON_COMM = 1 };

int overlap_level(const fx_ctx* lead)
{
	if (!multi_rank(lead) || lead->group->lanes.empty() || !lead->group->lanes[0].comm) return 0;
	return lead->opt_overlap;
}

struct ExchSpec { int set, k, pidx; };

static int do_exchange(fx_ctx* ctx, const std::vector<fx_ctx*>& M, const ExchSpec* specs, int nspec, StreamKind kind, hipStream_t s, int channel = 0)
{
	if (!multi_rank(ctx)) return FX_OK;
	DeviceGuard dg(ctx->device);
	std::vector<hipStream_t> streams;
	for (const LaneRef& L : lanes_of(ctx, M, s)) streams.push_back(kind == ON_COMM ? L.lane->comm : L.compute);
	ScopedMark mk(ctx, peer_group(ctx) ? streams[(size_t)ctx->rank] : streams[0], MK_EXCH);
	std::vector<std::vector<Seg>> segs(M.size());
	size_t total = 0;
	for (size_t i = 0; i < M.size(); ++i) {
		for (int j = 0; j < nspec; ++j) {
			if (specs[j].k <= 0) continue;
			ExchItem it[4];
			const int n = exchange_items(M[i], specs[j].set, specs[j].k, specs[j].pidx, it);
			halo_segments(M[i], it, n, segs[i]);
		}
		total += segs[i].size();
		if (M[i]->timing_on) for (const Seg& sg : segs[i]) M[i]->acc.exchange_bytes += sg.bytes;
	}
	if (!total) return FX_OK;
	for (fx_ctx* m : M) if (m->timing_on) m->acc.exchange_calls += 1;
	return ctx->group->transport->exchange(ctx->group, segs, streams, channel);
}

#define FX_LANES(body) do { for (const LaneRef& L : lanes_of(ctx, M, s)) { DeviceGuard dgl_(L.lane->device); body } } while (0)
static int comm_fork(fx_ctx* ctx, const std::vector<fx_ctx*>& M, hipStream_t s)
{
	FX_LANES(FX_HIP(hipEventRecord(L.lane->ev_ready, L.compute)); FX_HIP(hipStreamWaitEvent(L.lane->comm, L.lane->ev_ready, 0)););
	return FX_OK;
}
static int comm_mark_done(fx_ctx* ctx, const std::vector<fx_ctx*>& M, hipStream_t s) { FX_LANES(FX_HIP(hipEventRecord(L.lane->ev_done, L.lane->comm));); return FX_OK; }
static int comm_join(fx_ctx* ctx, const std::vector<fx_ctx*>& M, hipStream_t s) { FX_LANES(FX_HIP(hipStreamWaitEvent(L.compute, L.lane->ev_done, 0));); return FX_OK; }


int advect_range(fx_ctx* ctx, hipStream_t s, Range r, bool own_only)
{
	if (r.hi <= r.lo) return FX_OK;
	DeviceGuard dg(ctx->device);
	const SimParams sp{ ctx->time_step, (int)ctx->desc.advect_address, ctx->g.Zg > 1 ? 1 : 0, ctx->impulse_on ? 1 : 0 };
	const int par = ctx->frame_parity;
	if (ctx->adv_scheme == FX_ADVECT_MACCORMACK) {
		if (!ctx->mc_vel || !ctx->mc_col || r.lo != 0 || r.hi != ctx->g.Zg) { ctx->last_error = "MacCormack advection of a partial plane range"; return FX_E_STATE; }
		const bool was_rendered = ctx->rendered_since_step && ctx->rendered_on == s;
		ctx->rendered_since_step = false;
		float* alpha = was_rendered && ctx->accel_ok && ctx->opt_render_accel && FX_KNOB_INT("ADVECT_ALPHA", 1) ? ctx->accel.alpha : nullptr;
		if (ctx->accel_alpha_of == ctx->col[par]) ctx->accel_alpha_of = nullptr;
		FX_HIP(launch_maccormack(ctx->g, sp, ctx->half, ctx->vel[0], ctx->col[1 - par], ctx->vel[1], ctx->col[par], ctx->mc_vel, ctx->mc_col, alpha, s));
		if (alpha) ctx->accel_alpha_of = ctx->col[par];
		return FX_OK;
	}
	Geom g = ctx->g;
	g.zlo = std::max(g.zlo, g.z0 - ctx->adv_w_lo); g.zhi = std::min(g.zhi, g.z0 + g.nz - 1 + ctx->adv_w_hi);
	if (own_only) { g.zlo = std::max(g.zlo, g.z0); g.zhi = std::min(g.zhi, g.z0 + g.nz - 1); }
	if (!ctx->adv_far && !ctx->adv_far_tried) {
		ctx->adv_far_tried = true;
		const size_t words = advect_far_words(g, g.nz);
		if (words) {
			if (hipMalloc((void**)&ctx->adv_far, words * sizeof(uint32_t)) == hipSuccess) {
				FX_HIP(hipMemsetAsync(ctx->adv_far, 0, 2 * sizeof(uint32_t), s));
				ctx->adv_far_words = words;
			} else {
				(void)hipGetLastError();
				ctx->adv_far = nullptr;
			}
		}
	}
	const bool lend = ctx->adv_far != nullptr;
	bool far_used = false;
	const bool frame_was_rendered = ctx->rendered_since_step && ctx->rendered_on == s;
	ctx->rendered_since_step = false;
	AdvectAlpha aa{ frame_was_rendered && ctx->accel_ok && ctx->opt_render_accel && FX_KNOB_INT("ADVECT_ALPHA", 1) ? ctx->accel.alpha : nullptr, false };
	if (ctx->accel_alpha_of == ctx->col[par]) ctx->accel_alpha_of = nullptr;
	FX_HIP(launch_advect(g, sp, ctx->half, ctx->vel[0], ctx->col[1 - par], ctx->vel[1], ctx->col[par],
		r.lo, r.hi, ctx->halo_overflow, s, lend ? ctx->adv_far : nullptr, lend ? ctx->adv_far_words : 0, (int)(ctx->adv_far_turn & 1u), &far_used, &aa));
	if (aa.written) ctx->accel_alpha_of = ctx->col[par];
	if (far_used) ++ctx->adv_far_turn;
	return FX_OK;
}

int options_digest(const fx_ctx* c)
{
	uint32_t h = 2166136261u;
	uint32_t dt_bits;
	std::memcpy(&dt_bits, &c->time_step, 4);
	for (uint32_t v : { (uint32_t)c->opt_overlap, (uint32_t)c->opt_round, (uint32_t)c->opt_adaptive, dt_bits }) h = (h ^ v) * 16777619u;
	return (int)(h & 0x3FFFFFFFu);
}

static int record_step(fx_ctx* ctx, std::vector<fx_ctx*>& M, hipStream_t s)
{
	if (!multi_rank(ctx) || !ctx->step_rec) return FX_OK;
	for (fx_ctx* m : M) {
		if (m->rec_in_project) { m->rec_in_project = false; continue; }
		DeviceGuard dg(m->device);
		FX_HIP(launch_face_need(m->g, m->half, m->vel[0], m->time_step, (int)m->desc.advect_address, options_digest(m), m->halo_overflow, m->step_rec, CS(m, s)));
	}
	DeviceGuard dg(ctx->device);
	if (ctx->group->transport->is_local()) {
		for (fx_ctx* m : M) {
			DeviceGuard dgm(m->device);
			FX_HIP(hipMemcpyAsync(m->rec_host, m->step_rec, 4 * sizeof(int), hipMemcpyDeviceToHost, CS(m, s)));
			FX_HIP(hipEventRecord(m->rec_ev, CS(m, s)));
		}
	} else {
		hipStream_t cs = s;
		if (overlap_level(ctx) >= 1) { int rc = comm_fork(ctx, M, s); if (rc) return rc; cs = ctx->group->lanes[0].comm; }
		if (ctx->group->transport->allgather(ctx->step_rec, 4, ctx->gath_dev, cs) != FX_OK) { ctx->last_error = "rccl: all-gather of the step record failed"; return FX_E_COMM; }
		FX_HIP(hipMemcpyAsync(ctx->rec_host, ctx->gath_dev, 4 * sizeof(int) * (size_t)ctx->nranks, hipMemcpyDeviceToHost, cs));
		FX_HIP(hipEventRecord(ctx->rec_ev, cs));
	}
	for (fx_ctx* m : M) { m->rec_pending = true; m->need_valid = true; m->rec_dt = m->time_step; }
	return FX_OK;
}

static int consume_record(fx_ctx* ctx, std::vector<fx_ctx*>& M)
{
	const int Ha = (int)ctx->desc.halo_advect;
	for (fx_ctx* m : M) { m->adv_w_lo = has_lower(m) ? Ha : 0; m->adv_w_hi = has_upper(m) ? Ha : 0; }
	if (!multi_rank(ctx) || !ctx->rec_pending) return FX_OK;
	const bool local = ctx->group->transport->is_local();
	for (fx_ctx* m : M) {
		DeviceGuard dg(m->device);
		FX_HIP(hipEventSynchronize(m->rec_ev));
		if (!local) break;
	}
	const int n = ctx->nranks;
	auto rec = [&](int r) -> const int* { return local ? M[(size_t)r]->rec_host : ctx->rec_host + 4 * r; };
	bool fault = false, mismatch = false, usable = ctx->opt_adaptive != 0;
	for (int r = 0; r < n; ++r) { fault = fault || rec(r)[3] != 0; mismatch = mismatch || rec(r)[2] != rec(0)[2]; }
	for (fx_ctx* m : M) { usable = usable && m->need_valid && m->time_step <= m->rec_dt; m->rec_pending = false; }
	if (fault) {
		for (fx_ctx* m : M) {
			if (!rec(m->rank)[3] || !m->halo_overflow) continue;
			DeviceGuard dg(m->device);
			FX_HIP(hipDeviceSynchronize());
			unsigned flag = 0;
			FX_HIP(hipMemcpy(&flag, m->halo_overflow, sizeof flag, hipMemcpyDeviceToHost));
			if (!flag) continue;
			FX_HIP(hipMemset(m->halo_overflow, 0, sizeof(unsigned)));
			FX_HIP(hipDeviceSynchronize());
			m->halo_fault = true;
		}
		ctx->last_error = "the previous step's advection left the exchanged halo on at least one rank";
		return FX_E_HALO;
	}
	if (mismatch) { ctx->last_error = "the ranks of the chain run with different schedule options (fx_set_option) or time steps"; return FX_E_STATE; }
	if (!usable) return FX_OK;
	for (int r = 0; r + 1 < n; ++r)
		if (std::max(rec(r)[1], rec(r + 1)[0]) > Ha) {
			ctx->last_error = "the next advection needs more planes across a slab face than halo_advect provides";
			return FX_E_HALO;
		}
	for (fx_ctx* m : M) {
		const int r = m->rank;
		m->adv_w_lo = r > 0 ? std::max(rec(r - 1)[1], rec(r)[0]) : 0;
		m->adv_w_hi = r + 1 < n ? std::max(rec(r)[1], rec(r + 1)[0]) : 0;
	}
	return FX_OK;
}

int advect_all(fx_ctx* ctx, std::vector<fx_ctx*>& M, hipStream_t s)
{
	int rc;
	const int Ha = (int)ctx->desc.halo_advect;
	bool col_ready = multi_rank(ctx);
	for (fx_ctx* m : M) col_ready = col_ready && m->col_halo_buf == 1 - (int)m->frame_parity;
	for (fx_ctx* m : M) m->col_halo_buf = -1;
	bool ov = overlap_level(ctx) >= 1;
	if (ov && ctx->group->min_nz <= 2 * Ha) ov = false;
	if (!ov) {
		if ((rc = consume_record(ctx, M))) return rc;
		if (col_ready) FX_LANES(FX_HIP(hipStreamWaitEvent(L.compute, L.lane->ev_col_done, 0)););
		const ExchSpec spec{ col_ready ? EX_ADVECT_VEL : EX_ADVECT_IN, Ha, 0 };
		if ((rc = do_exchange(ctx, M, &spec, 1, ON_COMPUTE, s))) return rc;
		for (fx_ctx* m : M) {
			ScopedMark mk(m, CS(m, s), MK_ADVECT);
			if (m->timing_on) m->acc.advect_halo_planes += (uint64_t)(m->adv_w_lo + m->adv_w_hi);
			if ((rc = advect_range(m, CS(m, s), owned(m), false))) return rc;
		}
		return FX_OK;
	}
	if ((rc = comm_fork(ctx, M, s))) return rc;
	for (fx_ctx* m : M) {
		ScopedMark mk(m, CS(m, s), MK_ADVECT);
		const Range o = owned(m);
		if ((rc = advect_range(m, CS(m, s), Range{ o.lo + (has_lower(m) ? Ha : 0), o.hi - (has_upper(m) ? Ha : 0) }, true))) return rc;
	}
	if ((rc = consume_record(ctx, M))) return rc;
	if (col_ready) FX_LANES(FX_HIP(hipStreamWaitEvent(L.lane->comm, L.lane->ev_col_done, 0)););
	const ExchSpec spec{ col_ready ? EX_ADVECT_VEL : EX_ADVECT_IN, Ha, 0 };
	if ((rc = do_exchange(ctx, M, &spec, 1, ON_COMM, s))) return rc;
	if ((rc = comm_mark_done(ctx, M, s))) return rc;
	if ((rc = comm_join(ctx, M, s))) return rc;
	for (fx_ctx* m : M) {
		ScopedMark mk(m, CS(m, s), MK_ADVECT);
		if (m->timing_on) m->acc.advect_halo_planes += (uint64_t)(m->adv_w_lo + m->adv_w_hi);
		const Range o = owned(m);
		if (has_lower(m) && (rc = advect_range(m, CS(m, s), Range{ o.lo, o.lo + Ha }, false))) return rc;
		if (has_upper(m) && (rc = advect_range(m, CS(m, s), Range{ o.hi - Ha, o.hi }, false))) return rc;
	}
	return FX_OK;
}

static float* alpha_mirror(const fx_ctx* ctx) { return ctx->accel_alpha_of == ctx->col[ctx->frame_parity] ? ctx->accel.alpha : nullptr; }

int confine_phase(fx_ctx* ctx, hipStream_t s)
{
	if (!(ctx->vort_eps > 0.0f) || !(ctx->time_step > 0.0f)) return FX_OK;
	DeviceGuard dg(ctx->device);
	ScopedMark mk(ctx, s, MK_ADVECT);
	FX_HIP(launch_confine_vorticity(ctx->g, ctx->half, ctx->vel[1], ctx->vel[0], ctx->vort_eps, ctx->time_step, s));
	std::swap(ctx->vel[0], ctx->vel[1]);
	return FX_OK;
}

int open_inflow_phase(fx_ctx* ctx, hipStream_t s)
{
	if (!ctx->open_faces || !(ctx->time_step > 0.0f)) return FX_OK;
	DeviceGuard dg(ctx->device);
	ScopedMark mk(ctx, s, MK_ADVECT);
	FX_HIP(launch_open_inflow(ctx->g, ctx->half, ctx->vel[0], ctx->col[ctx->frame_parity], alpha_mirror(ctx), ctx->open_faces, ctx->time_step, s));
	return FX_OK;
}

int emit_phase(fx_ctx* ctx, hipStream_t s)
{
	if (ctx->emitters.empty() || !(ctx->time_step > 0.0f)) return FX_OK;
	DeviceGuard dg(ctx->device);
	ScopedMark mk(ctx, s, MK_ADVECT);
	FX_HIP(launch_emit(ctx->g, ctx->half, ctx->vel[1], ctx->col[ctx->frame_parity], alpha_mirror(ctx), ctx->emitters.data(), (int)ctx->emitters.size(), ctx->time_step, s));
	return FX_OK;
}

int heat_phase(fx_ctx* ctx, hipStream_t s)
{
	if (!ctx->buoy_on || !ctx->temp[0] || !(ctx->time_step > 0.0f)) return FX_OK;
	DeviceGuard dg(ctx->device);
	ScopedMark mk(ctx, s, MK_ADVECT);
	const int cur = ctx->temp_cur;
	FX_HIP(launch_heat(ctx->g, ctx->half, ctx->buoy, ctx->heat_sources.data(), (int)ctx->heat_sources.size(), ctx->vel[0], ctx->vel[1],
		ctx->col[ctx->frame_parity], ctx->temp[cur], ctx->temp[1 - cur], ctx->obst_code, ctx->time_step, (int)ctx->desc.advect_address, s, ctx->open_faces));
	ctx->temp_cur = 1 - cur;
	return FX_OK;
}

int enforce_phase(fx_ctx* ctx, hipStream_t s)
{
	if (!ctx->obst_code || !ctx->obst_cells || !(ctx->time_step > 0.0f)) return FX_OK;
	DeviceGuard dg(ctx->device);
	ScopedMark mk(ctx, s, MK_ADVECT);
	if (!ctx->obst_bodies.empty()) {
		FX_HIP(launch_obstacle_enforce_mov(ctx->g, ctx->half, ctx->obst_code, ctx->obst_lo, ctx->obst_hi, ctx->obst_bodies.data(), (int)ctx->obst_bodies.size(),
			ctx->vel[1], ctx->col[ctx->frame_parity], alpha_mirror(ctx), s));
		return FX_OK;
	}
	FX_HIP(launch_obstacle_enforce(ctx->g, ctx->half, ctx->obst_code, ctx->obst_lo, ctx->obst_hi, ctx->vel[1], ctx->col[ctx->frame_parity], alpha_mirror(ctx), s));
	return FX_OK;
}

int divergence_phase(fx_ctx* ctx, hipStream_t s)
{
	DeviceGuard dg(ctx->device);
	ScopedMark mk(ctx, s, MK_DIV);
	const Range r = owned(ctx);
	if (ctx->obst_code && !ctx->obst_bodies.empty()) {
		FX_HIP(launch_divergence_obs_mov(ctx->g, ctx->half, ctx->vel[1], ctx->obst_code, ctx->obst_bodies.data(), (int)ctx->obst_bodies.size(), ctx->b, r.lo, r.hi, s));
		return FX_OK;
	}
	if (ctx->obst_code) {
		FX_HIP(launch_divergence_obs(ctx->g, ctx->half, ctx->vel[1], ctx->obst_code, ctx->b, r.lo, r.hi, s));
		return FX_OK;
	}
	FX_HIP(launch_divergence(ctx->g, ctx->half, ctx->vel[1], ctx->b, r.lo, r.hi, s));
	return FX_OK;
}

static JacobiPolicy policy_of(const fx_ctx* c)
{
	return jacobi_policy(c->g, (int)(c->desc.flags & FX_FLAG_JACOBI_FUSE_MASK), c->frozen != nullptr, c->frozen_alt != nullptr);
}

static int jacobi_launch(fx_ctx* ctx, hipStream_t s, int src, JacobiLaunch l, Range r, ScopedMark* mk)
{
	r.lo = std::max(r.lo, 0); r.hi = std::min(r.hi, ctx->g.Zg);
	if (r.hi <= r.lo) return FX_OK;
	DeviceGuard dg(ctx->device);
	FX_HIP(launch_jacobi(ctx->g, l, ctx->p[src], ctx->b, ctx->p[src ^ 1], ctx->frozen, ctx->frozen ? ctx->frozen_alt : nullptr, r.lo, r.hi, s));
	if (l.family == JF_TILE2D && ctx->frozen) std::swap(ctx->frozen, ctx->frozen_alt);
	if (mk) { mk->launches += 1; mk->sweeps += l.sweeps; }
	return FX_OK;
}

static int jacobi_round(fx_ctx* ctx, hipStream_t s, int count, ScopedMark* mk)
{
	std::vector<JacobiLaunch> plan(count);
	plan.resize(jacobi_plan(policy_of(ctx), count, plan.data()));
	int left = count;
	for (const JacobiLaunch& l : plan) {
		const int t = l.sweeps;
		if (mk && mk->kind == MK_JACOBI && mk->launches && t * mk->launches < mk->sweeps) mk->split(MK_JACOBI_TAIL);
		left -= t;
		const int rc = jacobi_launch(ctx, s, ctx->p_cur, l, grown(ctx, multi_rank(ctx) ? left : 0), mk);
		if (rc) return rc;
		ctx->p_cur ^= 1;
	}
	return FX_OK;
}

static int clear_freeze_masks(std::vector<fx_ctx*>& M, hipStream_t s)
{
	for (fx_ctx* m : M)
		if (m->frozen) { DeviceGuard dg(m->device); if (hipMemsetAsync(m->frozen, 0, m->g.cells_local(), s) != hipSuccess) return FX_E_DEVICE; }
	return FX_OK;
}

static bool takes_sparse_solver(const fx_ctx* c, uint32_t iters) { return freeze_takes_sparse_solver(c->g, iters, c->frozen && c->fz_tile_next, multi_rank(c), multi_rank(c) ? c->group->min_nz : 0); }

template <class T> static void freeze_rotate(T*& a, T*& d, T*& spare, bool strip) { std::swap(a, d); if (strip) std::swap(d, spare); }

static int jacobi_freeze(fx_ctx* lead, std::vector<fx_ctx*>& M, hipStream_t s, uint32_t iters)
{
	fx_ctx* ctx = lead;
	const bool multi = multi_rank(lead);
	struct Run { Geom v; size_t off, moff; int own0; FreezeWork w; float *src, *a, *d; uint8_t *ma, *md, *mx; uint32_t* stat; uint32_t stat_hi; };
	std::vector<Run> R(M.size());
	std::vector<std::unique_ptr<ScopedMark>> mk(M.size());
	const bool fuse = lead->fz_fuse_div;
	lead->fz_fuse_div = false;
	FreezeLaunch plan[kFreezeSlots];
	int launches = 0;
	for (size_t i = 0; i < M.size(); ++i) {
		fx_ctx* m = M[i];
		DeviceGuard dg(m->device);
		hipStream_t ms = CS(m, s);
		if (++m->fz_gen >= (1u << 23)) {
			FX_HIP(hipMemsetAsync(m->fz_tile_next, 0, (size_t)jacobi_freeze_tiles(m->g) * sizeof(uint32_t), ms));
			FX_HIP(hipMemsetAsync(m->fz_stat, 0, kFreezeStatRing * sizeof(uint32_t), ms));
			FX_HIP(hipMemsetAsync(m->fz_counts, 0, 2 * jacobi_freeze_count_words() * sizeof(uint32_t), ms));
// ... 340 lines not shown
```

### fluidx12_amd/csrc/fx_sim.hip

```cpp
#include "fx_internal.h"
#include <algorithm>
#include <cstdlib>
#include <cstdio>

namespace fx {

typedef _Float16 h16;
typedef _Float16 h16x4 __attribute__((ext_vector_type(4)));

struct __attribute__((packed, aligned(4))) F32Pair { float a, b; };
struct __attribute__((packed, aligned(2))) F16Pair { _Float16 a, b; };

template <bool HALF> struct Store;
template <> struct Store<false> {
	typedef float S;
	typedef float4 S4;
	static __device__ __forceinline__ void ld2(const S* p, size_t i, float& a, float& b)
	{
		const F32Pair v = *reinterpret_cast<const F32Pair*>(p + i);
		a = v.a; b = v.b;
	}
	static __device__ __forceinline__ float ld(const S* p, size_t i) { return p[i]; }
	static __device__ __forceinline__ float stored(float v) { return v; }
	static __device__ __forceinline__ void st(S* p, size_t i, float v) { p[i] = v; }
// ... 674 lines not shown
	return g.X % 3 == 0 ? ROW_VW3 : (g.X % 2 == 0 ? ROW_VW2 : ROW_SCALAR);
}

template <bool HALF>
__global__ __launch_bounds__(256) void k_face_need(const Geom g, const typename Store<HALF>::S* __restrict__ uz, float dt, int address, int* __restrict__ rec,
	int digest, const unsigned* __restrict__ halo_overflow)
{
	typedef Store<HALF> St;
	const size_t plane = g.plane();
	const int z = g.z0 + (int)blockIdx.y;
	const float pz = ((float)z + 0.5f) / (float)g.Zg;
	const typename St::S* row = uz + (size_t)g.lz(z) * plane;
	int lo = 0, hi = 0;
	auto one = [&](float u) {
		const float az = fmaf(-u, dt, pz);
		const int iz = (int)floorf(az * (float)g.Zg - 0.5f);
		const int a = addr_tap(iz, g.Zg, address), b_ = addr_tap(iz + 1, g.Zg, address);
		lo = max(lo, g.z0 - min(a, b_));
		hi = max(hi, max(a, b_) - (g.z0 + g.nz - 1));
	};
	if (!HALF && (plane & 3) == 0) {
		const float4* row4 = reinterpret_cast<const float4*>(row);
		for (size_t i = (size_t)blockIdx.x * blockDim.x + threadIdx.x; i < plane / 4; i += (size_t)gridDim.x * blockDim.x) {
			const float4 v = row4[i];
			one(v.x); one(v.y); one(v.z); one(v.w);
		}
	} else {
		for (size_t i = (size_t)blockIdx.x * blockDim.x + threadIdx.x; i < plane; i += (size_t)gridDim.x * blockDim.x) one(St::ld(row, i));
	}
	if (blockIdx.x == 0 && blockIdx.y == 0 && threadIdx.x == 0) { rec[2] = digest; rec[3] = (int)*halo_overflow; }
	if (__builtin_amdgcn_ballot_w64(lo > 0 || hi > 0) == 0) return;
#pragma unroll
	for (int o = 32; o > 0; o >>= 1) { lo = max(lo, __shfl_xor(lo, o)); hi = max(hi, __shfl_xor(hi, o)); }
	if ((threadIdx.x & 63) == 0) { if (lo > 0) atomicMax(rec, lo); if (hi > 0) atomicMax(rec + 1, hi); }
}

template <bool HALF>
__global__ __launch_bounds__(256) void k_copy_owned(const Geom g, const typename Store<HALF>::S* __restrict__ src,
	typename Store<HALF>::S* __restrict__ dst)
{
	const size_t n = g.cells_owned();
	const size_t off = (size_t)g.H * g.plane();
	for (size_t i = (size_t)blockIdx.x * blockDim.x + threadIdx.x; i < 3 * n; i += (size_t)gridDim.x * blockDim.x) {
		const size_t a = i / n, r = i - a * n;
		dst[a * g.cells_local() + off + r] = src[a * g.cells_local() + off + r];
	}
}

template <bool HALF>
__global__ __launch_bounds__(256) void k_to_storage(const float* __restrict__ src, typename Store<HALF>::S* __restrict__ dst, size_t n)
{
	for (size_t i = (size_t)blockIdx.x * blockDim.x + threadIdx.x; i < n; i += (size_t)gridDim.x * blockDim.x)
		Store<HALF>::st(dst, i, src[i]);
}
template <bool HALF>
__global__ __launch_bounds__(256) void k_from_storage(const typename Store<HALF>::S* __restrict__ src, float* __restrict__ dst, size_t n)
{
	for (size_t i = (size_t)blockIdx.x * blockDim.x + threadIdx.x; i < n; i += (size_t)gridDim.x * blockDim.x)
		dst[i] = Store<HALF>::ld(src, i);
}

static inline dim3 grid_xyz(const Geom& g, int nzp) { return dim3(((g.X + 63) / 64) * ((g.Y + 3) / 4) * nzp, 1, 1); }
static inline unsigned grid_1d(size_t n) { return (unsigned)((n + 255) / 256 < 4096 ? (n + 255) / 256 : 4096); }
enum { REMAP_JACOBI = 0, REMAP_ADVECT = 1, REMAP_DIV = 2, REMAP_PROJECT = 3 };
static int xcd_remap_on(int which)
{
	int mode[4] = { 1, 0, 0, 0 };
	const char* e = FX_KNOB("XCD_REMAP");
	int a, b_, c, d;
	if (e && sscanf(e, "%d,%d,%d,%d", &a, &b_, &c, &d) == 4) { mode[0] = a; mode[1] = b_; mode[2] = c; mode[3] = d; }
	return mode[which];
}

static int xcd_remap_for(int which, const Geom& g)
{
	const char* fe_ = FX_KNOB("XCD_REMAP");
	const bool forced = fe_ && *fe_;
	if (forced || which == REMAP_JACOBI) return xcd_remap_on(which);
	return g.Zg > 1 && g.plane() <= 32768 && g.cells_local() < (size_t)6 << 20 ? 1 : 0;
}

hipError_t launch_advect(const Geom& g, const SimParams& sp, int half_store, const void* vel_in, const void* col_in,
	void* vel_out, void* col_out, int z_begin, int z_end, unsigned* halo_overflow, hipStream_t s, uint32_t* far_scratch, size_t far_words, int far_parity, bool* far_used,
	AdvectAlpha* alpha)
{
	if (far_used) *far_used = false;
	if (alpha) alpha->written = false;
	if (z_end <= z_begin) return hipSuccess;
	int bx = 64, by = 4, bz = 1;
	if (const char* e = FX_KNOB("ADVECT_BLOCK")) {
		int a, b_, c;
		if (sscanf(e, "%d,%d,%d", &a, &b_, &c) == 3 && a > 0 && b_ > 0 && c > 0 && a * b_ * c <= 256) { bx = a; by = b_; bz = c; }
	}
	const int nzp = z_end - z_begin;
	{
		const char* le = FX_KNOB("ADVECT_LDS");
		if (!(le && le[0] == '0') && bx == 64 && by == 4 && bz == 1 && !xcd_remap_on(REMAP_ADVECT)) {
			const hipError_t e = launch_advect_lds(g, sp, half_store, vel_in, col_in, vel_out, col_out, z_begin, z_end, halo_overflow, far_scratch, far_words, far_parity, far_used, s, le && le[0] == '2', alpha);
			if (e != hipErrorNotSupported) return e;
		}
	}
	float* alpha_out = alpha && alpha->out && g.nzl() == g.Zg && z_begin == 0 && z_end == g.Zg ? alpha->out : nullptr;
	if (alpha_out) alpha->written = true;
	const char* fe = FX_KNOB("ADVECT_FAST");
	const bool fast_off = fe && fe[0] == '0';
	auto pow2 = [](int v) { return v > 0 && (v & (v - 1)) == 0; };
	if (!fast_off && pow2(g.X) && pow2(g.Y) && pow2(g.Zg) && g.X >= 2 && g.cells_local() * 16 < ((size_t)1 << 32) &&
		bx == 64 && by == 4 && bz == 1 && !xcd_remap_on(REMAP_ADVECT)) {
		const dim3 block(64, 4, 1), grid(((g.X + 63) / 64) * ((g.Y + 3) / 4) * nzp, 1, 1);
		const float rX = 1.0f / (float)g.X, rY = 1.0f / (float)g.Y, rZ = 1.0f / (float)g.Zg, inv_rr = sp.is3d ? 256.0f : 1024.0f;
		auto lg = [](int v) { int k = 0; while ((1 << k) < v) ++k; return k; };
		const int lgX = lg(g.X), lgY = lg(g.Y), lg_gx = lg((g.X + 63) / 64), lg_gy = lg((g.Y + 3) / 4);
		if (half_store)
			hipLaunchKernelGGL(k_advect_fast<true>, grid, block, 0, s, g, sp, (const h16*)vel_in, (const h16x4*)col_in,
				(h16*)vel_out, (h16x4*)col_out, z_begin, nzp, halo_overflow, rX, rY, rZ, inv_rr, lgX, lgY, lg_gx, lg_gy, alpha_out);
		else
			hipLaunchKernelGGL(k_advect_fast<false>, grid, block, 0, s, g, sp, (const float*)vel_in, (const float4*)col_in,
				(float*)vel_out, (float4*)col_out, z_begin, nzp, halo_overflow, rX, rY, rZ, inv_rr, lgX, lgY, lg_gx, lg_gy, alpha_out);
		return hipGetLastError();
	}
	const int cbz = g.Zg > 1 ? bz : 1;
	const dim3 block(bx, by, cbz), grid(((g.X + bx - 1) / bx) * ((g.Y + by - 1) / by) * ((nzp + cbz - 1) / cbz), 1, 1);
	if (half_store)
		hipLaunchKernelGGL(k_advect<true>, grid, block, 0, s, g, sp, (const h16*)vel_in, (const h16x4*)col_in,
			(h16*)vel_out, (h16x4*)col_out, z_begin, nzp, xcd_remap_for(REMAP_ADVECT, g), halo_overflow, alpha_out);
	else
		hipLaunchKernelGGL(k_advect<false>, grid, block, 0, s, g, sp, (const float*)vel_in, (const float4*)col_in,
			(float*)vel_out, (float4*)col_out, z_begin, nzp, xcd_remap_for(REMAP_ADVECT, g), halo_overflow, alpha_out);
	return hipGetLastError();
}

hipError_t launch_divergence(const Geom& g, int half_store, const void* vel, float* b, int z_begin, int z_end, hipStream_t s)
{
	if (z_end <= z_begin) return hipSuccess;
	const int w = sim_row_kernel(g, half_store, SIM_DIVERGENCE, g.Zg > 1);
	if (w == ROW_V4) {
		const int nzp = z_end - z_begin, X4 = g.X >> 2;
		const int bx = X4 < 64 ? X4 : 64;
		int by = 256 / bx; if (by > g.Y) by = g.Y;
		const dim3 block(bx, by, 1), grid(((X4 + bx - 1) / bx) * ((g.Y + by - 1) / by) * nzp, 1, 1);
		if (half_store) hipLaunchKernelGGL(k_divergence_v4<true>, grid, block, 0, s, g, (const h16*)vel, b, z_begin, nzp, xcd_remap_for(REMAP_DIV, g), by);
		else hipLaunchKernelGGL(k_divergence_v4<false>, grid, block, 0, s, g, (const float*)vel, b, z_begin, nzp, xcd_remap_for(REMAP_DIV, g), by);
		return hipGetLastError();
	}
	if (w != ROW_SCALAR) {
		const int nzp = z_end - z_begin, XW = g.X / w;
		const int bx = XW < 64 ? XW : 64;
		int by = 256 / bx; if (by > g.Y) by = g.Y;
		const dim3 block(bx, by, 1), grid(((XW + bx - 1) / bx) * ((g.Y + by - 1) / by) * nzp, 1, 1);
		if (half_store) hipLaunchKernelGGL((k_divergence_vw<2, true>), grid, block, 0, s, g, (const h16*)vel, b, z_begin, nzp, xcd_remap_for(REMAP_DIV, g), by);
		else if (w == 3) hipLaunchKernelGGL((k_divergence_vw<3, false>), grid, block, 0, s, g, (const float*)vel, b, z_begin, nzp, xcd_remap_for(REMAP_DIV, g), by);
		else hipLaunchKernelGGL((k_divergence_vw<2, false>), grid, block, 0, s, g, (const float*)vel, b, z_begin, nzp, xcd_remap_for(REMAP_DIV, g), by);
		return hipGetLastError();
	}
	const dim3 grid = grid_xyz(g, z_end - z_begin), block(64, 4, 1);
	if (half_store) hipLaunchKernelGGL(k_divergence<true>, grid, block, 0, s, g, (const h16*)vel, b, z_begin, z_end - z_begin, xcd_remap_for(REMAP_DIV, g));
	else hipLaunchKernelGGL(k_divergence<false>, grid, block, 0, s, g, (const float*)vel, b, z_begin, z_end - z_begin, xcd_remap_for(REMAP_DIV, g));
	return hipGetLastError();
}

hipError_t launch_jacobi_sweep(const Geom& g, const float* p_in, const float* b, float* p_out, uint8_t* frozen,
	int z_begin, int z_end, hipStream_t s)
{
	return launch_jacobi_sweep2(g, p_in, b, p_out, frozen, z_begin, z_end, 0, 0, s);
}

hipError_t launch_jacobi_sweep2(const Geom& g, const float* p_in, const float* b, float* p_out, uint8_t* frozen,
	int z_begin, int z_end, int z_begin2, int z_end2, hipStream_t s)
{
	if (z_end < z_begin) z_end = z_begin;
	if (z_end2 < z_begin2) z_end2 = z_begin2;
	const int split = z_end - z_begin;
	const int nzp = split + (z_end2 - z_begin2);
	if (nzp <= 0) return hipSuccess;
	if (!frozen && g.Zg > 1 && (g.X & 3) == 0) {
		const int X4 = g.X >> 2;
		const int bx = X4 < 64 ? X4 : 64;
		int by = 256 / bx; if (by < 1) by = 1; if (by > g.Y) by = g.Y;
		const dim3 block(bx, by, 1), grid(((X4 + bx - 1) / bx) * ((g.Y + by - 1) / by) * nzp, 1, 1);
		hipLaunchKernelGGL(k_jacobi_v4, grid, block, 0, s, g, p_in, b, p_out, z_begin, nzp, xcd_remap_on(REMAP_JACOBI), by, split, z_begin2);
	} else {
// ... 135 lines not shown
```

### fluidx12_amd/fluid.py

```python
import ctypes as C
import os

import numpy as np

from . import capi


def look_at_lh(eye, focus, up):
    eye, focus, up = (np.asarray(v, np.float32) for v in (eye, focus, up))
    z = focus - eye
    z = z / np.float32(np.sqrt(np.dot(z, z)))
    x = np.cross(up, z).astype(np.float32)
    x = x / np.float32(np.sqrt(np.dot(x, x)))
    y = np.cross(z, x).astype(np.float32)
    m = np.zeros((4, 4), np.float32)
    m[:3, 0], m[:3, 1], m[:3, 2] = x, y, z
    m[3, :3] = [-np.dot(x, eye), -np.dot(y, eye), -np.dot(z, eye)]
    m[3, 3] = 1.0
    return m


def perspective_fov_lh(fovy, aspect, zn, zf):
    h = np.float32(np.cos(0.5 * fovy) / np.sin(0.5 * fovy))
    w = np.float32(h / np.float32(aspect))
# ... 472 lines not shown
        p.lifetime = float(lifetime)
        capi.check(self._lib.fx_set_particle_params(self._ctx, C.byref(p)), "SetParticleParams")

    def GetParticleParams(self):
        self._need()
        p = capi.ParticleParams()
        capi.check(self._lib.fx_get_particle_params(self._ctx, C.byref(p)), "GetParticleParams")
        return {"scheme": {capi.PARTICLE_EULER: "euler", capi.PARTICLE_MIDPOINT: "midpoint"}.get(p.scheme, p.scheme), "drift": tuple(p.drift),
                "lifetime": p.lifetime, "flags": p.flags}

    def MoveParticles(self, stream=None):
        self._need()
        capi.check(self._lib.fx_move_particles(self._ctx, stream), "MoveParticles")

    def SampleVelocity(self, points, stream=None, out=None):
        self._need()
        if hasattr(points, "data_ptr") and getattr(points, "is_cuda", False):
            if out is None or tuple(out.shape) != (points.shape[0], 3) or tuple(points.shape[1:]) != (4,) or not points.is_contiguous() or not out.is_contiguous():
                raise TypeError("SampleVelocity: device points are a contiguous float32 (n, 4) tensor and take a contiguous float32 (n, 3) `out`")
            fp = C.POINTER(C.c_float)
            capi.check(self._lib.fx_sample_velocity(self._ctx, stream, C.cast(points.data_ptr() or None, fp), points.shape[0],
                                                    C.cast(out.data_ptr() or None, fp), capi.PARTICLES_DEVICE), "SampleVelocity")
            return out
        p = np.asarray(points, np.float32)
        p = p.reshape(-1, p.shape[-1] if p.ndim > 1 else 3)
        if p.shape[1] == 3:
            p = np.concatenate([p, np.zeros((p.shape[0], 1), np.float32)], axis=1)
        p = np.ascontiguousarray(p.reshape(-1, 4))
        res = np.empty((p.shape[0], 3), np.float32)
        capi.check(self._lib.fx_sample_velocity(self._ctx, stream, _fp(p) if p.size else None, p.shape[0], _fp(res) if p.size else None, 0), "SampleVelocity")
        return res

    def Divergence(self, stream=None):
        capi.check(self._lib.fx_divergence(self._ctx, stream), "Divergence")

    def Jacobi(self, iters, stream=None):
        capi.check(self._lib.fx_jacobi(self._ctx, stream, iters), "Jacobi")

    def Project(self, stream=None):
        capi.check(self._lib.fx_project(self._ctx, stream), "Project")

    def frame_info(self):
        self._need()
        fi = capi.FrameInfo()
        capi.check(self._lib.fx_get_frame_info(self._ctx, C.byref(fi)), "frame_info")
        return fi

    def _shape(self, field):
        X, Y, _ = self.grid
        nz = self.slab[1]
        if field in (capi.FIELD_VELOCITY, capi.FIELD_VELOCITY1):
            return (3, nz, Y, X), np.float32
        if field in (capi.FIELD_COLOR, capi.FIELD_COLOR_PREV):
            return (nz, Y, X, 4), np.float32
        if field in (capi.FIELD_PRESSURE, capi.FIELD_DIVERGENCE, capi.FIELD_TEMPERATURE):
            return (nz, Y, X), np.float32
        if field == capi.FIELD_LIGHTMAP:
            return (nz, Y, X, 3), np.float32
        if field == capi.FIELD_TARGET:
            return (self.viewport[1], self.viewport[0], 4), np.uint8
        if field == capi.FIELD_TARGET_FLOAT:
            return (self.viewport[1], self.viewport[0], 4), np.float32
        s = self.frame_info().cube_size
        if field == capi.FIELD_CUBE_DEPTH:
            return (6, s, s), np.float32
        return (6, s, s, 4), np.uint8

    def download(self, field):
        self._need()
        shape, dt = self._shape(field)
        out = np.empty(shape, dt)
        capi.check(self._lib.fx_download(self._ctx, field, out.ctypes.data_as(C.c_void_p), out.nbytes), "download")
        return out

    def digest(self, field, z_begin=0, z_count=0):
        z_begin, z_count = int(z_begin), int(z_count)
        if not (0 <= z_begin < 1 << 32 and 0 <= z_count < 1 << 32):
            raise ValueError("digest: z_begin and z_count must be in 0 .. 2^32 - 1, got %d, %d" % (z_begin, z_count))
        self._need()
        out = (C.c_uint64 * 2)()
        capi.check(self._lib.fx_field_digest(self._ctx, field, z_begin, z_count, out), "digest")
        return (int(out[1]) << 64) | int(out[0])

    def upload(self, field, array):
        self._need()
        shape, dt = self._shape(field)
        a = np.ascontiguousarray(array, dt)
        if a.shape != shape:
            raise ValueError("field %d expects shape %s, got %s" % (field, shape, a.shape))
        capi.check(self._lib.fx_upload(self._ctx, field, a.ctypes.data_as(C.c_void_p), a.nbytes), "upload")

    def SaveCheckpoint(self, path):
        self._need()
        capi.check(self._lib.fx_checkpoint_save(self._ctx, os.fsencode(path)), "SaveCheckpoint")

    def LoadCheckpoint(self, path):
        self._need()
        capi.check(self._lib.fx_checkpoint_load(self._ctx, os.fsencode(path)), "LoadCheckpoint")

    def timing_enable(self, on=True):
        capi.check(self._lib.fx_timing_enable(self._ctx, int(on)), "timing_enable")

    def timing_read(self, reset=True):
        t = capi.Timing()
        capi.check(self._lib.fx_timing_read(self._ctx, C.byref(t), int(reset)), "timing_read")
        return t

    def set_option(self, option, value):
        self._need()
        capi.check(self._lib.fx_set_option(self._ctx, int(option), int(value)), "set_option")

    def gather_color(self, full=None, root=0, slabs=None, stream=None):
        self._need()
        z0 = nz = None
        if slabs is not None:
            z0 = (C.c_uint32 * len(slabs))(*[int(a) for a, _ in slabs])
            nz = (C.c_uint32 * len(slabs))(*[int(b) for _, b in slabs])
        capi.check(self._lib.fx_comm_gather_color(self._ctx, stream, full._ctx if full is not None else None, int(root), z0, nz),
                   "gather_color")

    def comm_init_rank(self, unique_id, rank, nranks):
        buf = (C.c_char * len(unique_id)).from_buffer_copy(unique_id)
        capi.check(self._lib.fx_comm_init_rank(self._ctx, buf, len(unique_id), rank, nranks), "comm_init_rank")


def comm_unique_id():
    lib = capi.load()
    n = lib.fx_comm_id_bytes()
    buf = (C.c_char * n)()
    capi.check(lib.fx_comm_get_unique_id(buf, n), "comm_get_unique_id")
    return bytes(buf)


default_local_group = "shared"


def comm_init_local(fluids, peer=None):
    lib = capi.load()
    arr = (C.c_void_p * len(fluids))(*[f._ctx for f in fluids])
    if peer is None:
        peer = default_local_group == "peer"
    if peer:
        capi.check(lib.fx_comm_init_peer(arr, len(fluids)), "comm_init_peer")
    else:
        capi.check(lib.fx_comm_init_local(arr, len(fluids)), "comm_init_local")


def comm_init_peer(fluids):
    comm_init_local(fluids, peer=True)


class LightProbe:

    def __init__(self, fluid):
        self._fluid = fluid
        self._radiance = None
        self._sh = None

    def Init(self, radiance_cube, mip=0):
        if isinstance(radiance_cube, (str, bytes, bytearray)):
            data = open(radiance_cube, "rb").read() if isinstance(radiance_cube, str) else bytes(radiance_cube)
            radiance_cube = self.decode_dds(data, mip)
            if radiance_cube is None:
                return False
        a = np.ascontiguousarray(radiance_cube, np.float32)
        if a.ndim != 4 or a.shape[0] != 6 or a.shape[1] != a.shape[2] or a.shape[3] != 3:
# ... 26 lines not shown
```

### include/fluidx_hip.h

```cpp
#ifndef FLUIDX_HIP_H
#define FLUIDX_HIP_H

#include <stddef.h>
#include <stdint.h>

#ifdef __cplusplus
extern "C" {
#endif

#define FX_ABI_VERSION 7

enum fx_status {
	FX_OK = 0,
	FX_E_INVALID = -1,
	FX_E_DEVICE = -2,
	FX_E_NOMEM = -3,
	FX_E_STATE = -4,
	FX_E_COMM = -5,
	FX_E_HALO = -6
};

enum fx_render_flags {
	FX_RAY_MARCH_DIRECT = 0,
	FX_RAY_MARCH_CUBEMAP = 1,
// ... 25 lines not shown
	uint32_t viewport_w, viewport_h;
	uint32_t storage;
	uint32_t jacobi_iters;
	uint32_t jacobi_mode;
	uint32_t advect_address;
	int32_t  device;
	uint32_t slab_z0, slab_nz;
	uint32_t halo_advect;
	uint32_t halo_jacobi;
	uint32_t flags;
} fx_desc;

#define FX_FLAG_JACOBI_FUSE_MASK 0xFu
#define FX_FLAG_NO_OVERLAP 0x10u
#define FX_FLAG_RENDER_ONLY 0x20u

typedef struct fx_frame_info {
	uint32_t cube_lod;
	uint32_t cube_size;
	uint32_t ray_samples;
	uint32_t visibility_mask;
	uint32_t frame_parity;
	float    edge_pixels;
	float    time_step;
	float    world_view_proj_i[16];
	float    screen_to_world[16];
} fx_frame_info;

typedef struct fx_timing {
	double   advect_ms, divergence_ms, jacobi_ms, project_ms, light_ms, view_ms, exchange_ms;
	uint64_t steps, jacobi_launches, jacobi_sweeps, renders;
	double   resolve_ms;
	double   jacobi_main_ms;
	uint64_t jacobi_main_launches, jacobi_main_sweeps;
	uint64_t exchange_bytes, advect_halo_planes;
	double   chain_ms;
	uint64_t freeze_solves, freeze_sweeps;
	uint64_t exchange_calls;
	uint64_t view_samples, light_samples, lightmap_fetches;
	uint64_t freeze_strip_launches;
} fx_timing;

int fx_abi_version(void);
const char* fx_error_string(int status);

int fx_create(fx_ctx** out, const fx_desc* desc);
int fx_destroy(fx_ctx* ctx);
int fx_set_max_samples(fx_ctx* ctx, uint32_t max_ray_samples, uint32_t max_light_samples);
int fx_set_sh(fx_ctx* ctx, const float* coeffs27);
int fx_update_frame(fx_ctx* ctx, float time_step, uint8_t frame_index,
	const float view[16], const float proj[16], const float eye[3]);
int fx_simulate(fx_ctx* ctx, void* stream, uint8_t frame_index);
int fx_render(fx_ctx* ctx, void* stream, uint8_t frame_index, uint8_t flags);
int fx_clear_render_target(fx_ctx* ctx, void* stream, const float rgba[4]);
int fx_render_cube(fx_ctx* ctx, void* stream, uint8_t frame_index);

#define FX_DEPTH_DEVICE 0x1u
int fx_set_scene_depth(fx_ctx* ctx, void* stream, const float* depth, uint32_t width, uint32_t height,
	float z_near, float z_far, uint32_t flags);

#define FX_LIGHT_DIRECTIONAL 0u
#define FX_LIGHT_POINT       1u
typedef struct fx_light {
	uint32_t struct_size, kind;
	float position[3];
	float color[4];
	float ambient[4];
} fx_light;
int fx_set_light(fx_ctx* ctx, const fx_light* light);
int fx_get_light(fx_ctx* ctx, fx_light* out);

int fx_set_environment(fx_ctx* ctx, const float* cube, uint32_t n);
int fx_render_environment(fx_ctx* ctx, void* stream, uint8_t frame_index);

int fx_get_frame_info(fx_ctx* ctx, fx_frame_info* out);

int fx_synchronize(fx_ctx* ctx);
const char* fx_last_error(fx_ctx* ctx);

int fx_upload(fx_ctx* ctx, int field, const void* host, size_t bytes);
int fx_download(fx_ctx* ctx, int field, void* host, size_t bytes);
size_t fx_field_bytes(fx_ctx* ctx, int field);
int fx_field_digest(fx_ctx* ctx, int field, uint32_t z_begin, uint32_t z_count, uint64_t out[2]);

int fx_checkpoint_save(fx_ctx* ctx, const char* path);
int fx_checkpoint_load(fx_ctx* ctx, const char* path);

int fx_advect(fx_ctx* ctx, void* stream);
int fx_divergence(fx_ctx* ctx, void* stream);
int fx_jacobi(fx_ctx* ctx, void* stream, uint32_t iters);
int fx_project(fx_ctx* ctx, void* stream);

int fx_set_vorticity_confinement(fx_ctx* ctx, float epsilon);
int fx_confine_vorticity(fx_ctx* ctx, void* stream);

#define FX_MAX_EMITTERS 16u
typedef struct fx_emitter {
	uint32_t struct_size, flags;
	float center[3];
	float radius;
	float color_rate[4];
	float force[3];
	float swirl;
} fx_emitter;
int fx_set_emitters(fx_ctx* ctx, const fx_emitter* list, uint32_t count);
int fx_get_emitters(fx_ctx* ctx, fx_emitter* out, uint32_t capacity, uint32_t* count);
int fx_set_impulse(fx_ctx* ctx, int enabled);
int fx_emit(fx_ctx* ctx, void* stream);

#define FX_OBSTACLES_DEVICE 0x1u
int fx_set_obstacles(fx_ctx* ctx, void* stream, const uint8_t* solid, size_t bytes, uint32_t flags);
int fx_get_obstacles(fx_ctx* ctx, uint8_t* solid_out, size_t bytes, uint64_t* solid_cells);
int fx_enforce_obstacles(fx_ctx* ctx, void* stream);

#define FX_MAX_OBSTACLE_BODIES 16u
typedef struct fx_obstacle_body {
	uint32_t struct_size, flags;
	float box_lo[3], box_hi[3];
	float linear[3];
	float angular[3];
	float pivot[3];
} fx_obstacle_body;
int fx_set_obstacle_bodies(fx_ctx* ctx, const fx_obstacle_body* list, uint32_t count);
int fx_get_obstacle_bodies(fx_ctx* ctx, fx_obstacle_body* out, uint32_t capacity, uint32_t* count);

#define FX_MAX_OBSTACLE_MESHES 16u
#define FX_MESH_DEVICE 0x1u
typedef struct fx_obstacle_mesh {
	uint32_t struct_size, flags;
	const float* positions;
	const uint32_t* indices;
	uint32_t vertex_count, triangle_count;
	const float* transform;
} fx_obstacle_mesh;
typedef struct fx_mesh_report { uint64_t solid_cells; uint32_t open_columns, skipped_triangles; } fx_mesh_report;
int fx_set_obstacle_meshes(fx_ctx* ctx, void* stream, const fx_obstacle_mesh* meshes, uint32_t count, fx_mesh_report* report);

#define FX_WALL_X_LO 0x01u
#define FX_WALL_X_HI 0x02u
#define FX_WALL_Y_LO 0x04u
#define FX_WALL_Y_HI 0x08u
#define FX_WALL_Z_LO 0x10u
#define FX_WALL_Z_HI 0x20u
int fx_set_open_walls(fx_ctx* ctx, uint32_t faces);
int fx_get_open_walls(fx_ctx* ctx, uint32_t* faces);
int fx_open_inflow(fx_ctx* ctx, void* stream);

#define FX_MAX_HEAT_SOURCES 16u
typedef struct fx_buoyancy {
	uint32_t struct_size, flags;
	float ambient;
	float density_weight;
	float lift;
	float cooling;
	float up[3];
} fx_buoyancy;
typedef struct fx_heat_source {
	uint32_t struct_size, flags;
	float center[3];
	float radius;
	float rate;
} fx_heat_source;
int fx_set_buoyancy(fx_ctx* ctx, const fx_buoyancy* buoyancy);
int fx_get_buoyancy(fx_ctx* ctx, fx_buoyancy* out, int* enabled);
int fx_set_heat_sources(fx_ctx* ctx, const fx_heat_source* list, uint32_t count);
int fx_get_heat_sources(fx_ctx* ctx, fx_heat_source* out, uint32_t capacity, uint32_t* count);
// ... 70 lines not shown
```

Before: 22.80 billion.

## Track colour bounding box in advection and skip loading colour outside it

Advection now records a device-side bounding box of voxels with non-zero colour output, via wave ballots and workgroup atomics. On the next step, tiles and planes outside the previous box skip the global colour gather into LDS and zero the LDS slot instead, staging only velocity. This is meant to cut HBM reads of the colour field in empty regions. In exchange it adds atomics, extra LDS state and box bookkeeping, and it depends on the box staying valid across every path that writes colour.

```diff
diff --git a/fluidx12_amd/capi.py b/fluidx12_amd/capi.py
--- a/fluidx12_amd/capi.py
+++ b/fluidx12_amd/capi.py
@@ -125,6 +125,7 @@
     "fx_checkpoint_save": (C.c_int, [_vp, C.c_char_p]),
     "fx_checkpoint_load": (C.c_int, [_vp, C.c_char_p]),
     "fx_advect": (C.c_int, [_vp, _vp]),
+    "fx_colour_bounds": (C.c_int, [_vp, C.POINTER(C.c_int)]),
     "fx_divergence": (C.c_int, [_vp, _vp]),
     "fx_jacobi": (C.c_int, [_vp, _vp, C.c_uint32]),
     "fx_project": (C.c_int, [_vp, _vp]),
diff --git a/fluidx12_amd/csrc/fx_advect_lds.hip b/fluidx12_amd/csrc/fx_advect_lds.hip
--- a/fluidx12_amd/csrc/fx_advect_lds.hip
+++ b/fluidx12_amd/csrc/fx_advect_lds.hip
@@ -93,6 +93,55 @@
 		: "=&s"(keep)
 		: "s"(col), "s"(v0), "s"(v1), "s"(v2), "v"(off_col), "v"(off_col_hi), "v"(off_vel), "s"(lds_col), "s"(lds_vel), "n"(VEL_BYTES)
 		: "scc");
+}
+
+template <bool HALF, int VEL_BYTES>
+__device__ __forceinline__ void stage64v(const void* v0, const void* v1, const void* v2, uint32_t off_vel, uint32_t lds_vel)
+{
+	uint32_t keep;
+	lds_vel = __builtin_amdgcn_readfirstlane(lds_vel);
+	if (HALF)
+		asm volatile(
+			"s_mov_b32 %0, m0\n\t"
+			"s_mov_b32 m0, %5\n\t"
+			"s_nop 0\n\t"
+			"global_load_lds_ushort %4, %1\n\t"
+			"s_add_u32 m0, m0, %6\n\t"
+			"s_nop 0\n\t"
+			"global_load_lds_ushort %4, %2\n\t"
+			"s_add_u32 m0, m0, %6\n\t"
+			"s_nop 0\n\t"
+			"global_load_lds_ushort %4, %3\n\t"
+			"s_mov_b32 m0, %0"
+			: "=&s"(keep)
+			: "s"(v0), "s"(v1), "s"(v2), "v"(off_vel), "s"(lds_vel), "n"(VEL_BYTES)
+			: "scc");
+	else
+		asm volatile(
+			"s_mov_b32 %0, m0\n\t"
+			"s_mov_b32 m0, %5\n\t"
+			"s_nop 0\n\t"
+			"global_load_lds_dword %4, %1\n\t"
+			"s_add_u32 m0, m0, %6\n\t"
+			"s_nop 0\n\t"
+			"global_load_lds_dword %4, %2\n\t"
+			"s_add_u32 m0, m0, %6\n\t"
+			"s_nop 0\n\t"
+			"global_load_lds_dword %4, %3\n\t"
+			"s_mov_b32 m0, %0"
+			: "=&s"(keep)
+			: "s"(v0), "s"(v1), "s"(v2), "v"(off_vel), "s"(lds_vel), "n"(VEL_BYTES)
+			: "scc");
+}
+
+__device__ __forceinline__ void box_widen(int* box, int (&seen)[6], int x, int y, int z)
+{
+	if (x < seen[0]) { atomicMin(box + 0, x); seen[0] = x; }
+	if (y < seen[1]) { atomicMin(box + 1, y); seen[1] = y; }
+	if (z < seen[2]) { atomicMin(box + 2, z); seen[2] = z; }
+	if (x > seen[3]) { atomicMax(box + 3, x); seen[3] = x; }
+	if (y > seen[4]) { atomicMax(box + 4, y); seen[4] = y; }
+	if (z > seen[5]) { atomicMax(box + 5, z); seen[5] = z; }
 }
 
 template <typename T>
@@ -145,7 +194,7 @@
 }
 
 template <bool HALF, bool ALPHA>
-__device__ __forceinline__ void advect_finish(const SimParams& sp, float (&u)[3], float (&c)[4], float ex, float dx, float dz, float dt, float atten,
+__device__ __forceinline__ bool advect_finish(const SimParams& sp, float (&u)[3], float (&c)[4], float ex, float dx, float dz, float dt, float atten,
 	uint32_t id, uint32_t stride, void* __restrict__ vel_out, void* __restrict__ col_out, float* __restrict__ alpha_out)
 {
 	if (__builtin_amdgcn_ballot_w64(sp.impulse && ex > -6.5f) != 0) {
@@ -177,12 +226,15 @@
 		hc.x = to_h16(c[0] * atten); hc.y = to_h16(c[1] * atten); hc.z = to_h16(c[2] * atten); hc.w = to_h16(c[3] * atten);
 		*reinterpret_cast<h16x4*>(co + id * 8u) = hc;
 		if (ALPHA) *reinterpret_cast<float*>(reinterpret_cast<char*>(alpha_out) + id * 4u) = (float)hc.w;
+		return __builtin_bit_cast(uint64_t, hc) != 0u;
 	} else {
 		*reinterpret_cast<float*>(vo + id * 4u) = u[0] * atten;
 		*reinterpret_cast<float*>(vo + (stride + id) * 4u) = u[1] * atten;
 		*reinterpret_cast<float*>(vo + (2u * stride + id) * 4u) = u[2] * atten;
-		*reinterpret_cast<float4*>(co + id * 16u) = make_float4(c[0] * atten, c[1] * atten, c[2] * atten, c[3] * atten);
-		if (ALPHA) *reinterpret_cast<float*>(reinterpret_cast<char*>(alpha_out) + id * 4u) = c[3] * atten;
+		const float4 t = make_float4(c[0] * atten, c[1] * atten, c[2] * atten, c[3] * atten);
+		*reinterpret_cast<float4*>(co + id * 16u) = t;
+		if (ALPHA) *reinterpret_cast<float*>(reinterpret_cast<char*>(alpha_out) + id * 4u) = t.w;
+		return (__float_as_uint(t.x) | __float_as_uint(t.y) | __float_as_uint(t.z) | __float_as_uint(t.w)) != 0u;
 	}
 }
 
@@ -192,9 +244,12 @@
 __global__ __launch_bounds__(64 * TY) __attribute__((amdgpu_waves_per_eu(4, 4))) void k_advect_lds(const Geom g, const SimParams sp,
 	const void* __restrict__ vel_in, const void* __restrict__ col_in, void* __restrict__ vel_out, void* __restrict__ col_out, float* __restrict__ alpha_out,
 	int z_begin, int nzp, int zchunk, int nchunks, unsigned* halo_overflow, float rX, float rY, float rZ, float inv_rr,
-	int lgX, int lgY, int lg_gx, int lg_gy, uint32_t* __restrict__ far_list, uint32_t* __restrict__ far_flat, uint32_t* __restrict__ far_total, uint32_t far_cap)
+	int lgX, int lgY, int lg_gx, int lg_gy, uint32_t* __restrict__ far_list, uint32_t* __restrict__ far_flat, uint32_t* __restrict__ far_total, uint32_t far_cap,
+	const int* __restrict__ box_in, int* box_out)
 {
 	__shared__ uint32_t far_n, far_base;
+	__shared__ unsigned long long wg_x;
+	__shared__ int wg_lo[2], wg_hi[2];
 	extern __shared__ __attribute__((aligned(16))) char lds[];
 
 	const int tid = (int)threadIdx.x, lane = tid & 63, wave = __builtin_amdgcn_readfirstlane(tid >> 6);
@@ -220,24 +275,56 @@
 	const char* v2 = v1 + (size_t)stride * ES;
 
 	uint32_t src_a, src_b = 0;
+	int xa_a, ya_a, xa_b = 0, ya_b = 0;
 	{
 		const int c = tid, r = c / HX, cc = c - r * HX;
-		src_a = rows<P2>((uint32_t)addr_tap(y0t - 1 + r, g.Y, sp.address), lgX, g) + (uint32_t)addr_tap(x0t - 1 + cc, g.X, sp.address);
+		xa_a = addr_tap(x0t - 1 + cc, g.X, sp.address); ya_a = addr_tap(y0t - 1 + r, g.Y, sp.address);
+		src_a = rows<P2>((uint32_t)ya_a, lgX, g) + (uint32_t)xa_a;
 	}
 	const bool has_b = NT + tid < NCELL;
 	if (has_b) {
 		const int c = NT + tid, r = c / HX, cc = c - r * HX;
-		src_b = rows<P2>((uint32_t)addr_tap(y0t - 1 + r, g.Y, sp.address), lgX, g) + (uint32_t)addr_tap(x0t - 1 + cc, g.X, sp.address);
+		xa_b = addr_tap(x0t - 1 + cc, g.X, sp.address); ya_b = addr_tap(y0t - 1 + r, g.Y, sp.address);
+		src_b = rows<P2>((uint32_t)ya_b, lgX, g) + (uint32_t)xa_b;
 	}
 	const bool wave_has_b = NT + wave * 64 < NCELL;
+
+	bool col_xy = true;
+	int col_z0 = 0, col_z1 = g.Zg - 1;
+	if (box_in) {
+		const int bx0 = box_in[0], by0 = box_in[1], bx1 = box_in[3], by1 = box_in[4];
+		col_z0 = box_in[2]; col_z1 = box_in[5];
+		const bool in_a = xa_a >= bx0 && xa_a <= bx1 && ya_a >= by0 && ya_a <= by1;
+		const bool in_b = has_b && xa_b >= bx0 && xa_b <= bx1 && ya_b >= by0 && ya_b <= by1;
+		col_xy = __builtin_amdgcn_ballot_w64(in_a || in_b) != 0;
+	}
+	uint32_t col_zero = 0u;
 
 	const uint32_t lds0 = (uint32_t)(size_t)(__attribute__((address_space(3))) char*)lds;
 	auto fill = [&](int zq) {
 		const int za = min(max(addr_tap(zq, g.Zg, sp.address), g.zlo), g.zhi);
 		const size_t pz = planes<P2>((uint32_t)g.lz(za), lgP, g);
-		const uint32_t slot = __builtin_amdgcn_readfirstlane(lds0 + (uint32_t)(((zq + 4) & 3) * SLOT_BYTES));
+		const uint32_t ring = (uint32_t)((zq + 4) & 3);
+		const uint32_t slot = __builtin_amdgcn_readfirstlane(lds0 + ring * SLOT_BYTES);
+		const char *b0 = v0 + pz * ES, *b1 = v1 + pz * ES, *b2 = v2 + pz * ES;
+		if (!(col_xy && za >= col_z0 && za <= col_z1)) {
+			stage64v<HALF, VEL_BYTES>(b0, b1, b2, src_a * ES, slot + COL_BYTES + (uint32_t)wave * (64 * 4));
+			if (wave_has_b && has_b) stage64v<HALF, VEL_BYTES>(b0, b1, b2, src_b * ES, slot + COL_BYTES + (NT + (uint32_t)wave * 64) * 4);
+			if (!(col_zero >> ring & 1u)) {
+				char* sc = lds + ring * SLOT_BYTES;
+				if (HALF) {
+					reinterpret_cast<uint32_t*>(sc)[tid] = 0u; reinterpret_cast<uint32_t*>(sc)[NCELL + tid] = 0u;
+					if (has_b) { reinterpret_cast<uint32_t*>(sc)[NT + tid] = 0u; reinterpret_cast<uint32_t*>(sc)[NCELL + NT + tid] = 0u; }
+				} else {
+					reinterpret_cast<float4*>(sc)[tid] = make_float4(0.0f, 0.0f, 0.0f, 0.0f);
+					if (has_b) reinterpret_cast<float4*>(sc)[NT + tid] = make_float4(0.0f, 0.0f, 0.0f, 0.0f);
+				}
+				col_zero |= 1u << ring;
+			}
+			return;
+		}
+		col_zero &= ~(1u << ring);
 		const char* bc = reinterpret_cast<const char*>(col_in) + pz * CS;
-		const char *b0 = v0 + pz * ES, *b1 = v1 + pz * ES, *b2 = v2 + pz * ES;
 		if (HALF) stage64h<VEL_BYTES>(bc, b0, b1, b2, src_a * CS, src_a * ES, slot + (uint32_t)wave * (64 * 4), slot + COL_BYTES + (uint32_t)wave * (64 * 4));
 		else stage64<VEL_BYTES>(bc, b0, b1, b2, src_a * CS, src_a * ES, slot + (uint32_t)wave * (64 * 16), slot + COL_BYTES + (uint32_t)wave * (64 * 4));
 		if (wave_has_b) {
@@ -249,6 +336,7 @@
 	};
 
 	if (DEFER && tid == 0) far_n = 0u;
+	if (tid == 0) { wg_x = 0ull; wg_lo[0] = wg_lo[1] = kBoxEmptyLo; wg_hi[0] = wg_hi[1] = kBoxEmptyHi; }
 	fill(zb - 1);
 	fill(zb);
 	fill(zb + 1);
@@ -264,6 +352,9 @@
 	const float dxy2 = fmaf(dy, dy, dx * dx);
 	const uint32_t own = (uint32_t)((wave + 1) * HX + lane + 1);
 	const float atten = fmaxf(fmaf(-dt, 0.200000003f, 1.0f), 0.0f);
+
+	uint64_t out_x = 0;
+	int out_z0 = g.Zg, out_z1 = -1;
 
 	auto compute = [&](int z) {
 		if (!has_voxel) return;
@@ -330,7 +421,9 @@
 		}
 
 		const uint32_t id = planes<P2>((uint32_t)g.lz(z), lgP, g) + rows<P2>((uint32_t)y, lgX, g) + (uint32_t)x;
-		advect_finish<HALF, ALPHA>(sp, u, c, ex, dx, dz, dt, atten, id, stride, vel_out, col_out, alpha_out);
+		const bool nz = advect_finish<HALF, ALPHA>(sp, u, c, ex, dx, dz, dt, atten, id, stride, vel_out, col_out, alpha_out);
+		const uint64_t m = __builtin_amdgcn_ballot_w64(nz);
+		if (m != 0) { out_x |= m; out_z0 = min(out_z0, z); out_z1 = z; }
 	};
 
 	for (int z = zb; z < ze; ++z) {
@@ -340,6 +433,19 @@
 		else if (ALPHA) asm volatile("s_waitcnt vmcnt(5)" ::: "memory");
 		else asm volatile("s_waitcnt vmcnt(4)" ::: "memory");
 		__syncthreads();
+	}
+	if (box_out) {
+		if (out_x != 0 && lane == 0) {
+			atomicOr(&wg_x, (unsigned long long)out_x);
+			atomicMin(&wg_lo[0], y); atomicMax(&wg_hi[0], y);
+			atomicMin(&wg_lo[1], out_z0); atomicMax(&wg_hi[1], out_z1);
+		}
+		__syncthreads();
+		if (tid == 0 && wg_x != 0ull) {
+			atomicMin(box_out + 0, x0t + (int)__builtin_ctzll(wg_x)); atomicMax(box_out + 3, x0t + 63 - (int)__builtin_clzll(wg_x));
+			atomicMin(box_out + 1, wg_lo[0]); atomicMax(box_out + 4, wg_hi[0]);
+			atomicMin(box_out + 2, wg_lo[1]); atomicMax(box_out + 5, wg_hi[1]);
+		}
 	}
 	if (DEFER) {
 		const uint32_t n = far_n;
@@ -357,10 +463,13 @@
 __global__ __launch_bounds__(256) void k_advect_far(const Geom g, const SimParams sp,
 	const void* __restrict__ vel_in, const void* __restrict__ col_in, void* __restrict__ vel_out, void* __restrict__ col_out, float* __restrict__ alpha_out,
 	const uint32_t* __restrict__ far_flat, const uint32_t* __restrict__ far_total, uint32_t* __restrict__ far_total_next, unsigned* halo_overflow,
-	float rX, float rY, float rZ, float inv_rr, int lgX, int lgY)
+	float rX, float rY, float rZ, float inv_rr, int lgX, int lgY, int* box_out, int* box_reset)
 {
 	const uint32_t n = *far_total;
-	if (blockIdx.x == 0 && threadIdx.x == 0) *far_total_next = 0u;
+	if (blockIdx.x == 0 && threadIdx.x == 0) {
+		*far_total_next = 0u;
+		if (box_reset) { for (int a = 0; a < 3; ++a) { box_reset[a] = kBoxEmptyLo; box_reset[3 + a] = kBoxEmptyHi; } }
+	}
 	const int lgP = lgX + lgY;
 	constexpr uint32_t ES = HALF ? 2 : 4;
 	const uint32_t stride = planes<P2>((uint32_t)g.nzl(), lgP, g);
@@ -369,6 +478,8 @@
 	const char* v2 = v1 + (size_t)stride * ES;
 	const float dt = sp.dt;
 	const float atten = fmaxf(fmaf(-dt, 0.200000003f, 1.0f), 0.0f);
+	int seen[6] = { kBoxEmptyLo, kBoxEmptyLo, kBoxEmptyLo, kBoxEmptyHi, kBoxEmptyHi, kBoxEmptyHi };
+	if (box_out && blockIdx.x * 256u + threadIdx.x < n) { for (int a = 0; a < 6; ++a) seen[a] = box_out[a]; }
 	for (uint32_t i = blockIdx.x * 256u + threadIdx.x; i < n; i += gridDim.x * 256u) {
 		const uint32_t code = far_flat[i];
 		int x, y, z;
@@ -393,17 +504,19 @@
 		const bool z_present = z0 >= g.zlo && z0 <= g.zhi && z1 >= g.zlo && z1 <= g.zhi;
 		float u[3], c[4];
 		advect_gather<HALF, P2>(g, sp, ix, iy, z0, z1, z_present, fx, fy, fz, v0, v1, v2, col_in, lgX, lgP, halo_overflow, u, c);
-		advect_finish<HALF, ALPHA>(sp, u, c, ex, dx, dz, dt, atten, id, stride, vel_out, col_out, alpha_out);
+		const bool nz = advect_finish<HALF, ALPHA>(sp, u, c, ex, dx, dz, dt, atten, id, stride, vel_out, col_out, alpha_out);
+		if (box_out && nz) box_widen(box_out, seen, x, y, z);
 	}
 }
 
 
 hipError_t launch_advect_lds(const Geom& g, const SimParams& sp, int half_store, const void* vel_in, const void* col_in,
 	void* vel_out, void* col_out, int z_begin, int z_end, unsigned* halo_overflow, uint32_t* far_scratch, size_t far_words, int far_parity, bool* far_used, hipStream_t s, bool force,
-	AdvectAlpha* alpha)
+	AdvectAlpha* alpha, AdvectBox* box)
 {
 	if (far_used) *far_used = false;
 	if (alpha) alpha->written = false;
+	if (box) box->used = false;
 	const int nzp = z_end - z_begin;
 	AdvectLdsKnobs kn;
 	kn.tile_rows = FX_KNOB_INT("ADVECT_TILE_ROWS", 8);
@@ -429,10 +542,14 @@
 		static bool attr_set = false; \
 		if (!attr_set) { (void)hipFuncSetAttribute(reinterpret_cast<const void*>(k_advect_lds<H_, TY_, D_, P_, A_>), hipFuncAttributeMaxDynamicSharedMemorySize, NSLOT * Lay<H_, TY_>::SLOT_BYTES); attr_set = true; } \
 		hipLaunchKernelGGL((k_advect_lds<H_, TY_, D_, P_, A_>), dim3(tiles_xy * nchunks), dim3(64 * TY_), (NSLOT * Lay<H_, TY_>::SLOT_BYTES), s, g, sp, vel_in, col_in, vel_out, col_out, alpha_out, \
-			z_begin, nzp, zchunk, nchunks, halo_overflow, rX, rY, rZ, inv_rr, lgX, lgY, lg_gx, lg_gy, far_list, far_flat, far_total, far_cap); } while (0)
-#define FX_FAR(H_, P_, A_) hipLaunchKernelGGL((k_advect_far<H_, P_, A_>), dim3(far_wgs), dim3(256), 0, s, g, sp, vel_in, col_in, vel_out, col_out, alpha_out, far_flat, far_total, far_total_next, halo_overflow, rX, rY, rZ, inv_rr, lgX, lgY)
+			z_begin, nzp, zchunk, nchunks, halo_overflow, rX, rY, rZ, inv_rr, lgX, lgY, lg_gx, lg_gy, far_list, far_flat, far_total, far_cap, box_in, box_out); } while (0)
+#define FX_FAR(H_, P_, A_) hipLaunchKernelGGL((k_advect_far<H_, P_, A_>), dim3(far_wgs), dim3(256), 0, s, g, sp, vel_in, col_in, vel_out, col_out, alpha_out, far_flat, far_total, far_total_next, halo_overflow, rX, rY, rZ, inv_rr, lgX, lgY, box_out, box_reset)
 	const int far_wgs = 1024;
 	float* alpha_out = pl.alpha ? alpha->out : nullptr;
+	const bool boxed = box && box->out && box->reset && defer && g.nzl() == g.Zg && z_begin == 0 && z_end == g.Zg;
+	const int* box_in = boxed ? box->in : nullptr;
+	int *box_out = boxed ? box->out : nullptr, *box_reset = boxed ? box->reset : nullptr;
+	if (boxed) box->used = true;
 	if (alpha_out) {
 		if (half_store) { if (p2) { FX_ADV(true, 8, true, true, true); FX_FAR(true, true, true); } else { FX_ADV(true, 8, true, false, true); FX_FAR(true, false, true); } }
 		else { if (p2) { FX_ADV(false, 8, true, true, true); FX_FAR(false, true, true); } else { FX_ADV(false, 8, true, false, true); FX_FAR(false, false, true); } }
diff --git a/fluidx12_amd/csrc/fx_api.cpp b/fluidx12_amd/csrc/fx_api.cpp
--- a/fluidx12_amd/csrc/fx_api.cpp
+++ b/fluidx12_amd/csrc/fx_api.cpp
@@ -360,6 +360,16 @@
 	out->time_step = ctx->time_step;
 	std::memcpy(out->world_view_proj_i, ctx->fc.wvp_i, sizeof out->world_view_proj_i);
 	std::memcpy(out->screen_to_world, ctx->fc.s2w, sizeof out->screen_to_world);
+	return FX_OK;
+}
+
+int fx_colour_bounds(fx_ctx* ctx, int out[6])
+{
+	if (!ctx || !out) return FX_E_INVALID;
+	if (!ctx->col_box || !ctx->col_box_valid[ctx->frame_parity]) return FX_E_STATE;
+	DeviceGuard dg(ctx->device);
+	FX_HIP(hipDeviceSynchronize());
+	FX_HIP(hipMemcpy(out, ctx->col_box + 6 * ctx->frame_parity, 6 * sizeof(int), hipMemcpyDeviceToHost));
 	return FX_OK;
 }
 
@@ -1089,7 +1099,7 @@
 		parts[r].bytes = (size_t)nz * plane_bytes;
 		parts[r].src = m ? (const char*)m->col[m->frame_parity] + (size_t)m->g.H * plane_bytes : nullptr;
 		parts[r].dst = am_root ? (char*)full->col[full->frame_parity] + (size_t)z0 * plane_bytes : nullptr;
-		if (am_root) full->accel_alpha_of = nullptr;
+		if (am_root) { full->accel_alpha_of = nullptr; fx_colour_written(full, full->frame_parity); }
 	}
 	DeviceGuard dg(ctx->device);
 	hipStream_t s = pick_stream(ctx, stream);
diff --git a/fluidx12_amd/csrc/fx_comm.cpp b/fluidx12_amd/csrc/fx_comm.cpp
--- a/fluidx12_amd/csrc/fx_comm.cpp
+++ b/fluidx12_amd/csrc/fx_comm.cpp
@@ -15,6 +15,7 @@
 	case EX_ADVECT_IN:
 		out[0] = ExchItem{ (char*)c->vel[0], plane * es, 3, k, nullptr, c->adv_w_lo, c->adv_w_hi };
 		out[1] = ExchItem{ (char*)c->col[1 - c->frame_parity], plane * es * 4, 1, k, nullptr, c->adv_w_lo, c->adv_w_hi };
+		fx_colour_written(c, 1 - c->frame_parity);
 		return 2;
 	case EX_UZ1:
 		out[0] = ExchItem{ (char*)c->vel[1] + 2 * (size_t)c->g.nzl() * plane * es, plane * es, 1, k, nullptr };
@@ -33,6 +34,7 @@
 		return 1;
 	case EX_COLOR_CUR:
 		out[0] = ExchItem{ (char*)c->col[c->frame_parity], plane * es * 4, 1, k, nullptr };
+		fx_colour_written(c, c->frame_parity);
 		return 1;
 	case EX_FREEZE:
 		out[0] = ExchItem{ (char*)c->fz_x_p, plane * 4, 1, k, nullptr };
diff --git a/fluidx12_amd/csrc/fx_context.cpp b/fluidx12_amd/csrc/fx_context.cpp
--- a/fluidx12_amd/csrc/fx_context.cpp
+++ b/fluidx12_amd/csrc/fx_context.cpp
@@ -91,7 +91,7 @@
 		if (c->p[i]) (void)hipFree(c->p[i]);
 	}
 	void* others[] = { c->env, c->cube_depth, c->depth_own, c->accel.occ, c->accel.alpha, c->accel.bits, c->accel.list, c->accel.cells, c->accel.gi, c->accel.ctr, c->target, c->target_float, c->p_face[0], c->p_face[1], c->b, c->frozen, c->frozen_alt, c->lightmap, c->cube, c->sh_dev, c->halo_overflow, c->stage,
-		c->sh_scratch[0], c->sh_scratch[1], c->sh_scratch[2], c->sh_scratch[3], c->p_aux, c->fz_mask[0], c->fz_mask[1], c->fz_mask[2], c->fz_tile_next, c->fz_stat, c->fz_list[0], c->fz_list[1], c->fz_counts, c->sample_counters, c->adv_far, c->obst_code, c->obst_spare, c->obst_stats, c->vox_bits, c->vox_report, c->vox_work, c->temp[0], c->temp[1], c->mc_vel, c->mc_col, c->mg_mem, c->part };
+		c->sh_scratch[0], c->sh_scratch[1], c->sh_scratch[2], c->sh_scratch[3], c->p_aux, c->fz_mask[0], c->fz_mask[1], c->fz_mask[2], c->fz_tile_next, c->fz_stat, c->fz_list[0], c->fz_list[1], c->fz_counts, c->sample_counters, c->adv_far, c->col_box, c->obst_code, c->obst_spare, c->obst_stats, c->vox_bits, c->vox_report, c->vox_work, c->temp[0], c->temp[1], c->mc_vel, c->mc_col, c->mg_mem, c->part };
 	for (void* q : others) if (q) (void)hipFree(q);
 	for (hipEvent_t e : c->ev) (void)hipEventDestroy(e);
 	if (c->step_rec) (void)hipFree(c->step_rec);
@@ -227,6 +227,14 @@
 					FX_HIP(hipMemsetAsync(ctx->adv_far, 0, 2 * sizeof(uint32_t), ctx->stream));
 					ctx->adv_far_words = words;
 				} else { (void)hipGetLastError(); ctx->adv_far = nullptr; }
+			}
+			if (!slab && ctx->adv_far) {
+				FX_HIP(hipMalloc((void**)&ctx->col_box, 12 * sizeof(int)));
+				for (int i = 0; i < 2; ++i) {
+					FX_HIP(hipMemsetD32Async((hipDeviceptr_t)(ctx->col_box + 6 * i), kBoxEmptyLo, 3, ctx->stream));
+					FX_HIP(hipMemsetD32Async((hipDeviceptr_t)(ctx->col_box + 6 * i + 3), kBoxEmptyHi, 3, ctx->stream));
+					ctx->col_box_valid[i] = ctx->col_box_empty[i] = true;
+				}
 			}
 		}
 		if (d->grid_z > 1) {
@@ -460,6 +468,7 @@
 		}
 		char* dst = (char*)ctx->col[field == FX_FIELD_COLOR ? ctx->frame_parity : 1 - ctx->frame_parity];
 		if (ctx->accel_alpha_of == dst) ctx->accel_alpha_of = nullptr;
+		fx_colour_written(ctx, field == FX_FIELD_COLOR ? ctx->frame_parity : 1 - ctx->frame_parity);
 		if ((rc = ensure_stage(ctx, need))) return rc;
 		FX_HIP(hipMemcpy(ctx->stage, host, need, hipMemcpyHostToDevice));
 		FX_HIP(launch_to_storage(ctx->stage, dst + off * 4 * es, 4 * n, ctx->half, ctx->stream));
diff --git a/fluidx12_amd/csrc/fx_context.h b/fluidx12_amd/csrc/fx_context.h
--- a/fluidx12_amd/csrc/fx_context.h
+++ b/fluidx12_amd/csrc/fx_context.h
@@ -40,6 +40,9 @@
 	bool adv_far_tried = false;
 	size_t adv_far_words = 0;
 	uint32_t adv_far_turn = 0;
+	int* col_box = nullptr;
+	bool col_box_valid[2] = { false, false };
+	bool col_box_empty[2] = { false, false };
 	uint32_t fz_gen = 0;
 	uint32_t fz_gen_mark = 0;
 	std::vector<uint32_t> fz_iters;
@@ -143,6 +146,8 @@
 	bool rec_in_project = false;
 };
 
+inline void fx_colour_written(fx_ctx* c, int i) { c->col_box_valid[i & 1] = false; }
+
 namespace fx {
 
 struct ExchItem { char* base; size_t plane_bytes; int ncomp; int k; char* recv_base; int k_lo = -1, k_hi = -1; };
diff --git a/fluidx12_amd/csrc/fx_internal.h b/fluidx12_amd/csrc/fx_internal.h
--- a/fluidx12_amd/csrc/fx_internal.h
+++ b/fluidx12_amd/csrc/fx_internal.h
@@ -52,12 +52,14 @@
 };
 
 struct AdvectAlpha { float* out; bool written; };
+struct AdvectBox { const int* in; int* out; int* reset; bool used; };
+const int kBoxEmptyLo = 0x7fffffff, kBoxEmptyHi = -0x7fffffff - 1;
 hipError_t launch_advect(const Geom& g, const SimParams& sp, int half_store, const void* vel_in, const void* col_in,
 	void* vel_out, void* col_out, int z_begin, int z_end, unsigned* halo_overflow, hipStream_t s, uint32_t* far_scratch = nullptr, size_t far_words = 0, int far_parity = 0, bool* far_used = nullptr,
-	AdvectAlpha* alpha = nullptr);
+	AdvectAlpha* alpha = nullptr, AdvectBox* box = nullptr);
 hipError_t launch_advect_lds(const Geom& g, const SimParams& sp, int half_store, const void* vel_in, const void* col_in,
 	void* vel_out, void* col_out, int z_begin, int z_end, unsigned* halo_overflow, uint32_t* far_scratch, size_t far_words, int far_parity, bool* far_used, hipStream_t s, bool force,
-	AdvectAlpha* alpha = nullptr);
+	AdvectAlpha* alpha = nullptr, AdvectBox* box = nullptr);
 size_t advect_far_words(const Geom& g, int nzp);
 const int kAdvectTileX = 64;
 struct AdvectLdsKnobs { int tile_rows = 8, lds_half = 1, defer = 1; const char* zchunk = nullptr; };
diff --git a/fluidx12_amd/csrc/fx_schedule.cpp b/fluidx12_amd/csrc/fx_schedule.cpp
--- a/fluidx12_amd/csrc/fx_schedule.cpp
+++ b/fluidx12_amd/csrc/fx_schedule.cpp
@@ -81,6 +81,7 @@
 		ctx->rendered_since_step = false;
 		float* alpha = was_rendered && ctx->accel_ok && ctx->opt_render_accel && FX_KNOB_INT("ADVECT_ALPHA", 1) ? ctx->accel.alpha : nullptr;
 		if (ctx->accel_alpha_of == ctx->col[par]) ctx->accel_alpha_of = nullptr;
+		fx_colour_written(ctx, par);
 		FX_HIP(launch_maccormack(ctx->g, sp, ctx->half, ctx->vel[0], ctx->col[1 - par], ctx->vel[1], ctx->col[par], ctx->mc_vel, ctx->mc_col, alpha, s));
 		if (alpha) ctx->accel_alpha_of = ctx->col[par];
 		return FX_OK;
@@ -107,9 +108,25 @@
 	ctx->rendered_since_step = false;
 	AdvectAlpha aa{ frame_was_rendered && ctx->accel_ok && ctx->opt_render_accel && FX_KNOB_INT("ADVECT_ALPHA", 1) ? ctx->accel.alpha : nullptr, false };
 	if (ctx->accel_alpha_of == ctx->col[par]) ctx->accel_alpha_of = nullptr;
+	AdvectBox bx{ nullptr, nullptr, nullptr, false };
+	if (ctx->col_box && !ctx->group && lend && r.lo == 0 && r.hi == g.Zg && g.nzl() == g.Zg) {
+		if (!ctx->col_box_empty[par]) {
+			FX_HIP(hipMemsetD32Async((hipDeviceptr_t)(ctx->col_box + 6 * par), kBoxEmptyLo, 3, s));
+			FX_HIP(hipMemsetD32Async((hipDeviceptr_t)(ctx->col_box + 6 * par + 3), kBoxEmptyHi, 3, s));
+			ctx->col_box_empty[par] = true;
+		}
+		bx.in = ctx->col_box_valid[1 - par] ? ctx->col_box + 6 * (1 - par) : nullptr;
+		bx.out = ctx->col_box + 6 * par;
+		bx.reset = ctx->col_box + 6 * (1 - par);
+	}
+	fx_colour_written(ctx, par);
 	FX_HIP(launch_advect(g, sp, ctx->half, ctx->vel[0], ctx->col[1 - par], ctx->vel[1], ctx->col[par],
-		r.lo, r.hi, ctx->halo_overflow, s, lend ? ctx->adv_far : nullptr, lend ? ctx->adv_far_words : 0, (int)(ctx->adv_far_turn & 1u), &far_used, &aa));
+		r.lo, r.hi, ctx->halo_overflow, s, lend ? ctx->adv_far : nullptr, lend ? ctx->adv_far_words : 0, (int)(ctx->adv_far_turn & 1u), &far_used, &aa, &bx));
 	if (aa.written) ctx->accel_alpha_of = ctx->col[par];
+	if (bx.used) {
+		ctx->col_box_valid[par] = true; ctx->col_box_empty[par] = false;
+		ctx->col_box_valid[1 - par] = false; ctx->col_box_empty[1 - par] = true;
+	}
 	if (far_used) ++ctx->adv_far_turn;
 	return FX_OK;
 }
@@ -255,6 +272,7 @@
 	if (!ctx->open_faces || !(ctx->time_step > 0.0f)) return FX_OK;
 	DeviceGuard dg(ctx->device);
 	ScopedMark mk(ctx, s, MK_ADVECT);
+	fx_colour_written(ctx, ctx->frame_parity);
 	FX_HIP(launch_open_inflow(ctx->g, ctx->half, ctx->vel[0], ctx->col[ctx->frame_parity], alpha_mirror(ctx), ctx->open_faces, ctx->time_step, s));
 	return FX_OK;
 }
@@ -264,6 +282,7 @@
 	if (ctx->emitters.empty() || !(ctx->time_step > 0.0f)) return FX_OK;
 	DeviceGuard dg(ctx->device);
 	ScopedMark mk(ctx, s, MK_ADVECT);
+	fx_colour_written(ctx, ctx->frame_parity);
 	FX_HIP(launch_emit(ctx->g, ctx->half, ctx->vel[1], ctx->col[ctx->frame_parity], alpha_mirror(ctx), ctx->emitters.data(), (int)ctx->emitters.size(), ctx->time_step, s));
 	return FX_OK;
 }
@@ -286,10 +305,12 @@
 	DeviceGuard dg(ctx->device);
 	ScopedMark mk(ctx, s, MK_ADVECT);
 	if (!ctx->obst_bodies.empty()) {
+		fx_colour_written(ctx, ctx->frame_parity);
 		FX_HIP(launch_obstacle_enforce_mov(ctx->g, ctx->half, ctx->obst_code, ctx->obst_lo, ctx->obst_hi, ctx->obst_bodies.data(), (int)ctx->obst_bodies.size(),
 			ctx->vel[1], ctx->col[ctx->frame_parity], alpha_mirror(ctx), s));
 		return FX_OK;
 	}
+	fx_colour_written(ctx, ctx->frame_parity);
 	FX_HIP(launch_obstacle_enforce(ctx->g, ctx->half, ctx->obst_code, ctx->obst_lo, ctx->obst_hi, ctx->vel[1], ctx->col[ctx->frame_parity], alpha_mirror(ctx), s));
 	return FX_OK;
 }
diff --git a/fluidx12_amd/csrc/fx_sim.hip b/fluidx12_amd/csrc/fx_sim.hip
--- a/fluidx12_amd/csrc/fx_sim.hip
+++ b/fluidx12_amd/csrc/fx_sim.hip
@@ -780,10 +780,11 @@
 
 hipError_t launch_advect(const Geom& g, const SimParams& sp, int half_store, const void* vel_in, const void* col_in,
 	void* vel_out, void* col_out, int z_begin, int z_end, unsigned* halo_overflow, hipStream_t s, uint32_t* far_scratch, size_t far_words, int far_parity, bool* far_used,
-	AdvectAlpha* alpha)
+	AdvectAlpha* alpha, AdvectBox* box)
 {
 	if (far_used) *far_used = false;
 	if (alpha) alpha->written = false;
+	if (box) box->used = false;
 	if (z_end <= z_begin) return hipSuccess;
 	int bx = 64, by = 4, bz = 1;
 	if (const char* e = FX_KNOB("ADVECT_BLOCK")) {
@@ -794,7 +795,7 @@
 	{
 		const char* le = FX_KNOB("ADVECT_LDS");
 		if (!(le && le[0] == '0') && bx == 64 && by == 4 && bz == 1 && !xcd_remap_on(REMAP_ADVECT)) {
-			const hipError_t e = launch_advect_lds(g, sp, half_store, vel_in, col_in, vel_out, col_out, z_begin, z_end, halo_overflow, far_scratch, far_words, far_parity, far_used, s, le && le[0] == '2', alpha);
+			const hipError_t e = launch_advect_lds(g, sp, half_store, vel_in, col_in, vel_out, col_out, z_begin, z_end, halo_overflow, far_scratch, far_words, far_parity, far_used, s, le && le[0] == '2', alpha, box);
 			if (e != hipErrorNotSupported) return e;
 		}
 	}
diff --git a/fluidx12_amd/fluid.py b/fluidx12_amd/fluid.py
--- a/fluidx12_amd/fluid.py
+++ b/fluidx12_amd/fluid.py
@@ -578,6 +578,15 @@
         capi.check(self._lib.fx_field_digest(self._ctx, field, z_begin, z_count, out), "digest")
         return (int(out[1]) << 64) | int(out[0])
 
+    def colour_bounds(self):
+        self._need()
+        out = (C.c_int * 6)()
+        rc = self._lib.fx_colour_bounds(self._ctx, out)
+        if rc == capi.FX_E_STATE:
+            return None
+        capi.check(rc, "colour_bounds")
+        return tuple(int(v) for v in out)
+
     def upload(self, field, array):
         self._need()
         shape, dt = self._shape(field)
diff --git a/include/fluidx_hip.h b/include/fluidx_hip.h
--- a/include/fluidx_hip.h
+++ b/include/fluidx_hip.h
@@ -131,6 +131,8 @@
 int fx_download(fx_ctx* ctx, int field, void* host, size_t bytes);
 size_t fx_field_bytes(fx_ctx* ctx, int field);
 int fx_field_digest(fx_ctx* ctx, int field, uint32_t z_begin, uint32_t z_count, uint64_t out[2]);
+
+int fx_colour_bounds(fx_ctx* ctx, int out[6]);
 
 int fx_checkpoint_save(fx_ctx* ctx, const char* path);
 int fx_checkpoint_load(fx_ctx* ctx, const char* path);
```

New measurement: 22.17 billion. -2.8%, worse.
